# LoveDaisy/ice_halo_sim

Measured on AMD Instinct MI355X. Metric: rays/sec (whole node) at 9 wavelengths, single-scatter hex column, higher is better.
Workload: dtype f32

## Files before the change

### ice_halo_sim_amd/csrc/halo_backend.cpp

```cpp
#include <cstdlib>
#include <dlfcn.h>
#include <hip/hip_runtime.h>

#include <algorithm>
#include <cmath>
#include <cstdio>
#include <cstring>
#include <map>
#include <memory>
#include <mutex>
#include <string>
#include <vector>

#include "halo_device.h"
#include "halo_host.hpp"
#include "halo_launch.h"

#ifndef HALO_XYZ_LOG_MIN_PIX
#define HALO_XYZ_LOG_MIN_PIX (1u << 19)
#endif

using namespace halo;

namespace {

template <typename T>
struct DevBuf {
  T* ptr = nullptr;
  size_t cap = 0;
  hipError_t reserve(size_t n) {
    if (n <= cap) return hipSuccess;
    if (ptr) (void)hipFree(ptr);
    ptr = nullptr;
    cap = 0;
    hipError_t e = hipMalloc(reinterpret_cast<void**>(&ptr), std::max<size_t>(n, 1) * sizeof(T));
    if (e == hipSuccess) cap = n;
    return e;
  }
  void release() {
    if (ptr) (void)hipFree(ptr);
    ptr = nullptr;
    cap = 0;
  }
};
template <typename... B>
void release_all(B&... bufs) { (bufs.release(), ...); }

struct Marker {
  hipEvent_t ev = nullptr;
  bool set = false;
  hipError_t mark(hipStream_t s) { const hipError_t e = hipEventRecord(ev, s); set = set || e == hipSuccess; return e; }
  hipError_t wait_on(hipStream_t s) const { return set ? hipStreamWaitEvent(s, ev, 0) : hipSuccess; }
  void clear() { set = false; }
};

}

struct HaloBackend {
  int device = 0;
  uint32_t seed = 1;
  std::string error;
  hipStream_t own_stream = nullptr;
  hipStream_t stream = nullptr;
  int cu_count = 256;

  int capture = 0;
  uint32_t geom_clock = 32;
  uint64_t chunk = 1ull << 28;
  uint64_t stoch_chunk = 0;
  uint32_t bin_l1 = 128u;
  int aggregate = 1;
  int mono_enabled = 1;
  int bin = -1;
  DevBuf<HitRec> bin_list_s[2], bin_list2_s[2];
  DevBuf<uint32_t> bin_cnt_s[2], bin_cnt2_s[2];
  int log_set = 0;
  Marker set_free[2];
  hipStream_t aux = nullptr;
  hipEvent_t ev_fork = nullptr, ev_join = nullptr;
  bool aux_pending = false;
  hipStream_t cs[2] = {nullptr, nullptr};
  hipEvent_t ev_cs[2] = {nullptr, nullptr}, ev_main = nullptr, ev_aux = nullptr;
  bool cs_pending[2] = {false, false};
  int cs_next = 0;
  uint64_t aux_seq = 0, cs_seen_aux[2] = {0, 0};
  int overlap = 1;
  int defer_fold = 0;
  int twin_set = 0;
  int lambda_planes = -1;
  int mono_copies = 8;
  uint32_t mono_s_log2 = 0;
  int blocks_per_cu = 24;
  int host_shapes = 0;
  int gen_serial = 0;
  int small_blocks_per_cu = 0;
  int blocks_cap = 0;
  int lazy_fold = 1;
  int hit_log = -1;
  uint32_t hit_log_cap = 0;
  int hex_fast = 1;
  int entry_fast = 1;
  int filter_fast = 1;
  int async = 0;
  uint32_t shuffle_chunk_log2 = 5;
  int spec_root = 1;
  int close_direct = -1;
  uint64_t direct_closes = 0;
  Marker close_done;
  int close_ts = 0;
  bool cnt2_clean[2] = {false, false};
  int tile_append = -1;
  uint64_t tile_appends = 0;
  DevBuf<HitRec> tile_chunk_s[2];
  DevBuf<uint32_t> tile_cnt_s[2];
  HaloRouteInfo route{};
  uint32_t route_root = 0;

  uint64_t gen_count = 0, gate_count = 0, transit_count = 0, shape_count = 0;
  double sess_max_w = 1.0;

  bool in_session = false;
  HaloScene scene{};
  HaloRender render{};
  HaloWl wl{};
  ProjDev proj{};
  int layer_idx = 0;
  double carry[HALO_MAX_LAYERS][HALO_MAX_ENTRIES] = {};

  DevBuf<float> acc_own;
  float* acc = nullptr;
  uint64_t acc_floats = 0;
  int acc_w = 0, acc_h = 0;
  int own_w = 0, own_h = 0;
  std::vector<HaloFilter> filters;
  std::vector<HaloColorSet> color_sets;
  std::vector<HaloColorClass> color_classes;
  DevBuf<double> lanes;
  int lanes_w = 0, lanes_h = 0;
  DevBuf<FilterDev> filter_dev;
  std::unique_ptr<FastTables> fast_scratch;
  DevBuf<float> mono;
  DevBuf<double> ovf;
  DevBuf<uint32_t> ovf_flag;
  bool mono_session = false;
  bool mono_by_wl = false;
  bool xyz_log = false;
  bool mono_dirty = false;
  bool mono_two = false;
  int mono_set = 0;
  size_t mono_half = 0;
  Marker set_folded[2];
  uint32_t plane_cnt = 1, plane_copies = 8;
  std::vector<std::array<float, 3>> plane_coef;
  DevBuf<float> cons_sum, cons_comp, cons_xyz_out, cons_stage;
  DevBuf<uint8_t> cons_rgb;
  DevBuf<float> comp_rgb, lanes_stage;
  DevBuf<uint32_t> comp_hist;
  DevBuf<float> aev_vals;
  DevBuf<uint32_t> aev_ws;
  int aev_agg_hist = 0;
  int aev_select = -1;
  int cons_w = 0, cons_h = 0;
  double total_intensity = 0.0;
  DevBuf<double> tally;
  double* tally_host = nullptr;
  double tally_seen[kSumNum] = {};
  bool tally_unread = false;
  double time_trace_ms = 0.0, time_post_ms = 0.0;
  uint64_t time_launches = 0;
  DevBuf<uint32_t> counters;
  static constexpr int kRing = 32;
  DevBuf<DispatchSlot> ring_dev;
  DispatchSlot* ring_host = nullptr;
  hipEvent_t ring_ev0[kRing] = {}, ring_ev1[kRing] = {}, ring_ev2[kRing] = {}, ring_ev3[kRing] = {}, ring_done[kRing] = {};
  bool ring_posts[kRing] = {};
  bool ring_final[kRing] = {};
  bool ring_busy[kRing] = {};
  uint64_t ring_use[kRing] = {};
  int ring_next = 0;
  struct TableCacheEntry {
    bool valid = false;
    int mode = 0;
    bool use_filter = false, use_color = false, entry_fast = false, hex_regular = false, has_fast = false;
    int cur = 0;
    int read_ring[2] = {-1, -1};
    uint64_t read_use[2] = {0, 0};
  };
  TableCacheEntry tcache[HALO_MAX_LAYERS][HALO_MAX_ENTRIES];
  DevBuf<DispatchSlot> tcache_dev;
  HaloScene tcache_scene{};
  HaloWl tcache_wl{};
  std::vector<HaloWl> tcache_spec;
  uint32_t spec_count = 0;
  int table_cache = 1;
  std::map<std::string, int64_t> opt_last;
  HaloLayerStats pending{};
  HaloLayerStats layer_acc{};
  std::vector<WlEntryDev> wl_pool_host;
  uint32_t wl_pool_size = 0;
  struct LutKey { int32_t type; float center, spread; host::LatLut lut; };
  std::vector<LutKey> lut_cache;
  DevBuf<ShapeDev> shapes_s[2];
  Marker shapes_free[2];
  hipEvent_t ev_gen = nullptr;
  int shapes_next = 0;
  hipEvent_t ev_gate = nullptr;
  Marker rmw[2];
  int log_tiles_log2 = 7;
  int alt_log2 = 25;
  int rehit_strategy = 1;
  int pool_entry_fast = 1;
  int gen_ahead = 0;
  int deterministic = 0;
  bool det_session = false;
  bool fix_planes = false;
  DevBuf<unsigned long long> fix;
  uint32_t fix_frac = 32, fix_frac_landed = 32;
  uint64_t fix_hits = 0;
  unsigned long long fix_landed_seen = 0;
  double landed_carry = 0.0;
  uint32_t shard_index = 0, shard_count = 1;
  int64_t rank_opt = 0;
  bool fix_imported = false;
  bool landed_own = false;
  DevBuf<float> cont[2];
  uint32_t cont_stride[2] = {0, 0};
  uint32_t cont_region[2] = {0, 0};
  DevBuf<uint32_t> cont_cnt;
  uint32_t cont_seg[kContShards + 4] = {};
  int cont_out_slot = 0;
  uint64_t cont_in_n = 0;
  int cont_shuffle = 1;
  int cont_order = 0;
  DevBuf<uint32_t> cont_mask;
  DevBuf<uint32_t> cont_err;
  DevBuf<uint32_t> cont_base;
  DevBuf<uint32_t> cont_tiles;
  uint32_t cont_fill_max = 0;
  uint64_t cont_roots = 0;
  DevBuf<HaloExitRecord> exits;
  uint64_t exits_pending = 0;
  DevBuf<float> host_f;
  DevBuf<uint32_t> host_u;
  uint64_t sess_crystal_samples = 0, sess_orient_samples = 0;
  std::vector<hipEvent_t*> untimed_events() {
    return {&ev_cs[0], &ev_cs[1], &ev_main, &ev_aux, &ev_fork, &ev_join, &ev_gen, &ev_gate, &set_free[0].ev, &set_free[1].ev, &shapes_free[0].ev,
            &shapes_free[1].ev, &rmw[0].ev, &rmw[1].ev, &set_folded[0].ev, &set_folded[1].ev, &close_done.ev};
  }
};

namespace {

int fail(HaloBackend* b, int code, const std::string& msg) {
  if (b) b->error = msg;
  return code;
}
int hip_fail(HaloBackend* b, hipError_t e, const char* what) {
  return fail(b, (e == hipErrorNoDevice || e == hipErrorInvalidDevice || e == hipErrorOutOfMemory) ? HALO_UNAVAILABLE : HALO_FATAL,
              std::string(what) + ": " + hipGetErrorString(e));
}
#define HIPCHK(b, call)                                   \
  do {                                                    \
    hipError_t e__ = (call);                              \
    if (e__ != hipSuccess) return hip_fail(b, e__, #call); \
  } while (0)

inline float* planes_of(HaloBackend* b) { return b->mono.ptr + (b->mono_two ? static_cast<size_t>(b->mono_set) * b->mono_half : 0u); }
inline hipStream_t post_stream(HaloBackend* b) { return b->overlap ? b->aux : b->stream; }
int fork_aux(HaloBackend* b) {
  if (!b->overlap) return HALO_OK;
  HIPCHK(b, hipEventRecord(b->ev_fork, b->stream));
  HIPCHK(b, hipStreamWaitEvent(b->aux, b->ev_fork, 0));
  for (int k = 0; k < 2; k++)
    if (b->cs_pending[k]) {
      HIPCHK(b, hipEventRecord(b->ev_cs[k], b->cs[k]));
      HIPCHK(b, hipStreamWaitEvent(b->aux, b->ev_cs[k], 0));
    }
  b->aux_pending = true;
  b->aux_seq++;
  return HALO_OK;
}
int join_aux(HaloBackend* b) {
  if (b->aux_pending) {
    HIPCHK(b, hipEventRecord(b->ev_join, b->aux));
    HIPCHK(b, hipStreamWaitEvent(b->stream, b->ev_join, 0));
    b->aux_pending = false;
  }
  for (int k = 0; k < 2; k++)
    if (b->cs_pending[k]) {
      HIPCHK(b, hipEventRecord(b->ev_cs[k], b->cs[k]));
      HIPCHK(b, hipStreamWaitEvent(b->stream, b->ev_cs[k], 0));
      b->cs_pending[k] = false;
      b->rmw[k].clear();
      if (b->close_ts == k) b->close_done.clear();
    }
  return HALO_OK;
}
int wait_for_aux(HaloBackend* b, int i) {
  if (b->overlap && b->aux_pending && b->cs_seen_aux[i] != b->aux_seq) {
    HIPCHK(b, hipEventRecord(b->ev_aux, b->aux));
    HIPCHK(b, hipStreamWaitEvent(b->cs[i], b->ev_aux, 0));
    b->cs_seen_aux[i] = b->aux_seq;
  }
  return HALO_OK;
}
int next_trace_stream(HaloBackend* b, bool touches_planes, bool alternate, hipStream_t* out, int* which) {
  if (!b->overlap) {
    *out = b->stream;
    *which = 0;
    return HALO_OK;
  }
  const int i = alternate ? b->cs_next : 0;
  if (alternate) b->cs_next ^= 1;
  HIPCHK(b, hipEventRecord(b->ev_main, b->stream));
  HIPCHK(b, hipStreamWaitEvent(b->cs[i], b->ev_main, 0));
  if (touches_planes)
    if (int rc = wait_for_aux(b, i)) return rc;
  b->cs_pending[i] = true;
  *out = b->cs[i];
  *which = i;
  return HALO_OK;
}
inline uint64_t log_min_rays(int visible) { return visible == HALO_VISIBLE_FULL ? (1ull << 19) : (2ull << 20); }
int sync_all(HaloBackend* b) {
  if (int rc = join_aux(b)) return rc;
  HIPCHK(b, hipStreamSynchronize(b->stream));
  return HALO_OK;
}
template <typename T>
int reserve_idle(HaloBackend* b, DevBuf<T>& buf, size_t n, hipError_t* err = nullptr) {
  if (n > buf.cap) {
    if (int rc = sync_all(b)) return rc;
  }
  const hipError_t e = buf.reserve(n);
  if (err) {
    *err = e;
    return HALO_OK;
  }
  HIPCHK(b, e);
  return HALO_OK;
}

int take_landed_delta(HaloBackend* b, double* landed);
int forget_landed(HaloBackend* b) {
  if (!b->tally.ptr) return HALO_OK;
  if (int rc = join_aux(b)) return rc;
  double unused = 0.0;
  return take_landed_delta(b, &unused);
}

int ensure_accumulator(HaloBackend* b, int w, int h) {
  const uint64_t need = static_cast<uint64_t>(w) * h * 3 + 4;
  if (b->acc && b->acc != b->acc_own.ptr) {
    if (b->acc_floats < need) return fail(b, HALO_FATAL, "bound accumulator smaller than width*height*3+4 floats");
    b->acc_w = w;
    b->acc_h = h;
    return HALO_OK;
  }
  if (!b->acc_own.ptr || b->acc_own.cap < need || b->own_w != w || b->own_h != h) {
    if (int rc = reserve_idle(b, b->acc_own, need)) return rc;
    if (int rc = join_aux(b)) return rc;
    if (b->own_w != 0 || b->own_h != 0)
      if (int rc = forget_landed(b)) return rc;
    HIPCHK(b, hipMemsetAsync(b->acc_own.ptr, 0, need * sizeof(float), b->stream));
    b->own_w = w;
    b->own_h = h;
  }
  b->acc_w = w;
  b->acc_h = h;
  b->acc = b->acc_own.ptr;
  b->acc_floats = need;
  return HALO_OK;
}

void harvest_slot(HaloBackend* b, int k) {
  if (!b->ring_busy[k]) return;
  (void)hipEventSynchronize(b->ring_done[k]);
  float ms = 0.0f, ms2 = 0.0f;
  (void)hipEventElapsedTime(&ms, b->ring_ev0[k], b->ring_ev1[k]);
  if (b->ring_posts[k]) (void)hipEventElapsedTime(&ms2, b->ring_ev2[k], b->ring_ev3[k]);
  static const bool debug_timing = std::getenv("HALO_DEBUG_TIMING") != nullptr;
  if (debug_timing) std::fprintf(stderr, "[halo timing] slot %d final %d posts %d trace %.4f ms passes %.4f ms\n", k, int(b->ring_final[k]), int(b->ring_posts[k]), ms, ms2);
  const bool timed = ms >= 0.0f && ms2 >= 0.0f;
  if (timed) b->layer_acc.kernel_ms += ms + ms2;
  if (b->ring_final[k] && timed) {
    b->time_trace_ms += ms;
    b->time_post_ms += ms2;
    b->time_launches += 1;
  }
  b->layer_acc.launches += 1;
  b->ring_busy[k] = false;
}
int read_tally(HaloBackend* b, double out[kSumNum], unsigned long long* fix_landed = nullptr) {
  HIPCHK(b, hipMemcpyAsync(b->tally_host, b->tally.ptr, kTallyLines * kTallyStride * sizeof(double), hipMemcpyDeviceToHost, b->stream));
  HIPCHK(b, hipStreamSynchronize(b->stream));
  if (fix_landed) {
    *fix_landed = 0ull;
    for (uint32_t l = 0; l < kTallyLines; l++) {
      unsigned long long v;
      std::memcpy(&v, &b->tally_host[l * kTallyStride + kSumFixLanded], sizeof(v));
      *fix_landed += v;
    }
  }
  for (int t = 0; t < kSumNum; t++) {
    double v = 0.0;
    for (uint32_t l = 0; l < kTallyLines; l++) v += b->tally_host[l * kTallyStride + static_cast<uint32_t>(t)];
    out[t] = v;
  }
  return HALO_OK;
}
int pull_tally(HaloBackend* b) {
  if (!b->tally_unread) return HALO_OK;
  double now[kSumNum];
  int rc = read_tally(b, now);
  if (rc != HALO_OK) return rc;
  b->layer_acc.exit_w_sum += now[kSumExitW] - b->tally_seen[kSumExitW];
  b->layer_acc.exit_count += static_cast<uint64_t>(now[kSumExitN] - b->tally_seen[kSumExitN] + 0.5);
  b->layer_acc.pixel_hits += static_cast<uint64_t>(now[kSumPixN] - b->tally_seen[kSumPixN] + 0.5);
  for (int t : {kSumExitW, kSumExitN, kSumPixN}) b->tally_seen[t] = now[t];
  b->tally_unread = false;
  return HALO_OK;
}
int take_landed_delta(HaloBackend* b, double* landed) {
  double now[kSumNum];
  unsigned long long fix_now = 0ull;
  int rc = read_tally(b, now, &fix_now);
  if (rc != HALO_OK) return rc;
  *landed = now[kSumLanded] - b->tally_seen[kSumLanded] + std::ldexp(static_cast<double>(fix_now - b->fix_landed_seen), -static_cast<int>(b->fix_frac_landed)) + b->landed_carry;
  b->tally_seen[kSumLanded] = now[kSumLanded];
  b->fix_landed_seen = fix_now;
  b->landed_carry = 0.0;
  return HALO_OK;
}
void harvest_all(HaloBackend* b) {
  for (int k = 0; k < HaloBackend::kRing; k++) harvest_slot(b, k);
}
void add_stats(HaloLayerStats& dst, const HaloLayerStats& src) {
  dst.root_count += src.root_count;
  dst.exit_count += src.exit_count;
  dst.continuation_count += src.continuation_count;
  dst.exit_w_sum += src.exit_w_sum;
  dst.kernel_ms += src.kernel_ms;
  dst.pixel_hits += src.pixel_hits;
  dst.launches += src.launches;
}
void drop_table_cache(HaloBackend* b) {
  for (auto& layer : b->tcache)
    for (auto& e : layer) e.valid = false;
}
const host::LatLut& cached_lut(HaloBackend* b, const HaloDist& d) {
  for (const auto& e : b->lut_cache)
    if (e.type == d.type && e.center == d.center && e.spread == d.spread) return e.lut;
  if (b->lut_cache.size() >= 64) b->lut_cache.clear();
  b->lut_cache.push_back({d.type, d.center, d.spread, host::BuildLatLut(d)});
  return b->lut_cache.back().lut;
}

}

extern "C" {

static int fold_if_dirty(HaloBackend* b);
static int fold_queue(HaloBackend* b);
int halo_abi_version(void) { return HALO_ABI_VERSION; }

int halo_device_count(void) {
  int n = 0;
  if (hipGetDeviceCount(&n) != hipSuccess) return 0;
  return n;
}

int halo_create(int device_ordinal, uint32_t seed, halo_handle_t* out) {
  if (!out) return HALO_FATAL;
  *out = nullptr;
  int n = 0;
  if (hipGetDeviceCount(&n) != hipSuccess || n <= 0 || device_ordinal < 0 || device_ordinal >= n) return HALO_UNAVAILABLE;
  hipDeviceProp_t prop;
  if (hipGetDeviceProperties(&prop, device_ordinal) != hipSuccess) return HALO_UNAVAILABLE;
  if (std::strncmp(prop.gcnArchName, "gfx950", 6) != 0) return HALO_UNAVAILABLE;
  auto* b = new HaloBackend();
  b->device = device_ordinal;
  b->seed = seed ? seed : 1u;
  b->cu_count = prop.multiProcessorCount > 0 ? prop.multiProcessorCount : 256;
  if (hipSetDevice(device_ordinal) != hipSuccess || hipStreamCreateWithFlags(&b->own_stream, hipStreamNonBlocking) != hipSuccess) {
    delete b;
    return HALO_UNAVAILABLE;
  }
  bool aux_ok = hipStreamCreateWithFlags(&b->aux, hipStreamNonBlocking) == hipSuccess && hipStreamCreateWithFlags(&b->cs[0], hipStreamNonBlocking) == hipSuccess &&
                hipStreamCreateWithFlags(&b->cs[1], hipStreamNonBlocking) == hipSuccess;
  for (hipEvent_t* ev : b->untimed_events()) aux_ok = aux_ok && hipEventCreateWithFlags(ev, hipEventDisableTiming) == hipSuccess;
  bool ring_ok = aux_ok && b->ring_dev.reserve(HaloBackend::kRing) == hipSuccess &&
                 hipHostMalloc(reinterpret_cast<void**>(&b->ring_host), HaloBackend::kRing * sizeof(DispatchSlot), hipHostMallocDefault) == hipSuccess &&
                 hipHostMalloc(reinterpret_cast<void**>(&b->tally_host), kTallyLines * kTallyStride * sizeof(double), hipHostMallocDefault) == hipSuccess;
  for (int k = 0; ring_ok && k < HaloBackend::kRing; k++)
    ring_ok = hipEventCreate(&b->ring_ev0[k]) == hipSuccess && hipEventCreate(&b->ring_ev1[k]) == hipSuccess && hipEventCreate(&b->ring_ev2[k]) == hipSuccess && hipEventCreate(&b->ring_ev3[k]) == hipSuccess &&
              hipEventCreateWithFlags(&b->ring_done[k], hipEventDisableTiming) == hipSuccess;
  if (!ring_ok) {
    halo_destroy(b);
    return HALO_UNAVAILABLE;
  }
  b->stream = b->own_stream;
  if (b->tally.reserve(kTallyLines * kTallyStride) != hipSuccess || b->counters.reserve(kCntNum) != hipSuccess) {
    halo_destroy(b);
    return HALO_UNAVAILABLE;
  }
  (void)hipMemsetAsync(b->tally.ptr, 0, kTallyLines * kTallyStride * sizeof(double), b->stream);
  (void)hipMemsetAsync(b->counters.ptr, 0, kCntNum * sizeof(uint32_t), b->stream);
  *out = b;
  return HALO_OK;
}

int halo_destroy(halo_handle_t b) {
  if (!b) return HALO_OK;
  (void)hipSetDevice(b->device);
  (void)hipStreamSynchronize(b->stream);
  if (b->aux) (void)hipStreamSynchronize(b->aux);
  for (int k = 0; k < 2; k++)
    if (b->cs[k]) (void)hipStreamSynchronize(b->cs[k]);
  release_all(b->acc_own, b->tally, b->mono, b->ovf, b->ovf_flag, b->filter_dev, b->cons_sum, b->cons_comp, b->cons_xyz_out, b->cons_stage, b->cons_rgb, b->comp_rgb,
              b->lanes_stage, b->comp_hist, b->aev_vals, b->aev_ws, b->counters, b->ring_dev, b->tcache_dev, b->shapes_s[0], b->shapes_s[1], b->cont_cnt, b->cont_mask, b->cont_err, b->cont_base,
              b->cont_tiles, b->lanes, b->fix, b->cont[0], b->cont[1], b->exits, b->host_f, b->host_u);
  for (int k = 0; k < 2; k++) release_all(b->bin_list_s[k], b->bin_cnt_s[k], b->bin_list2_s[k], b->bin_cnt2_s[k]);
  for (int k = 0; k < 2; k++) release_all(b->tile_chunk_s[k], b->tile_cnt_s[k]);
  if (b->ring_host) (void)hipHostFree(b->ring_host);
  if (b->tally_host) (void)hipHostFree(b->tally_host);
  for (int k = 0; k < HaloBackend::kRing; k++)
    for (hipEvent_t ev : {b->ring_ev0[k], b->ring_ev1[k], b->ring_ev2[k], b->ring_ev3[k], b->ring_done[k]})
      if (ev) (void)hipEventDestroy(ev);
  for (hipEvent_t* ev : b->untimed_events())
    if (*ev) (void)hipEventDestroy(*ev);
  if (b->aux) (void)hipStreamDestroy(b->aux);
  for (int k = 0; k < 2; k++)
    if (b->cs[k]) (void)hipStreamDestroy(b->cs[k]);
  if (b->own_stream) (void)hipStreamDestroy(b->own_stream);
  delete b;
  return HALO_OK;
}

const char* halo_last_error(halo_handle_t b) { return b ? b->error.c_str() : "null handle"; }

int halo_set_option(halo_handle_t b, const char* key, int64_t v) {
  if (!b || !key) return HALO_FATAL;
  const std::string k(key);
  {
    auto it = b->opt_last.find(k);
    const bool same = it != b->opt_last.end() && it->second == v && k != "rank" && k != "ray_base" && k != "seed";
    if (!same) drop_table_cache(b);
    b->opt_last[k] = v;
  }
  if ((k == "capture_exits" || k == "filter_fast") && b->in_session) return fail(b, HALO_FATAL, k + " cannot change inside a session");
  if (k == "capture_exits") b->capture = v ? 1 : 0;
  else if (k == "geom_clock") b->geom_clock = static_cast<uint32_t>(v > 0 ? v : 32);
  else if (k == "chunk") {
    const uint64_t top = (1ull << 32) - (static_cast<uint64_t>(b->cu_count) * 64ull * kBlock) - kBlock;
    b->chunk = std::min<uint64_t>(static_cast<uint64_t>(v > 0 ? v : (1ll << 28)), top);
  }
  else if (k == "bin_l1") {
    if (v < 8 || v > 512 || (v & (v - 1)) != 0) return fail(b, HALO_FATAL, "bin_l1 must be a power of two in [8, 512]");
    b->bin_l1 = static_cast<uint32_t>(v);
  }
  else if (k == "stoch_chunk") b->stoch_chunk = static_cast<uint64_t>(v > 0 ? v : 0);
  else if (k == "aggregate") b->aggregate = static_cast<int>(v);
  else if (k == "mono") b->mono_enabled = v ? 1 : 0;
  else if (k == "async") b->async = v ? 1 : 0;
  else if (k == "lambda_planes") b->lambda_planes = static_cast<int>(v);
  else if (k == "bin") b->bin = static_cast<int>(v);
  else if (k == "host_shapes") b->host_shapes = v ? 1 : 0;
  else if (k == "entry_fast") b->entry_fast = v ? 1 : 0;
  else if (k == "hex_fast") b->hex_fast = v ? 1 : 0;
  else if (k == "filter_fast") b->filter_fast = v ? 1 : 0;
  else if (k == "spec_root") b->spec_root = v ? 1 : 0;
  else if (k == "hit_log") b->hit_log = static_cast<int>(v);
  else if (k == "hit_log_cap") b->hit_log_cap = static_cast<uint32_t>(std::max<int64_t>(v, 0));
  else if (k == "gen_serial") b->gen_serial = v ? 1 : 0;
  else if (k == "shuffle_chunk") {
    if (v < 1 || v > 64 || (v & (v - 1)) != 0) return fail(b, HALO_FATAL, "shuffle_chunk must be a power of two in [1, 64]");
    b->shuffle_chunk_log2 = 0;
    while ((1ll << b->shuffle_chunk_log2) < v) b->shuffle_chunk_log2++;
  }
  else if (k == "lazy_fold") b->lazy_fold = v ? 1 : 0;
  else if (k == "table_cache") b->table_cache = v ? 1 : 0;
  else if (k == "overlap") {
    if (int rc = sync_all(b)) return rc;
    b->overlap = v ? 1 : 0;
  }
  else if (k == "defer_fold") b->defer_fold = v ? 1 : 0;
  else if (k == "auto_ev_hist") b->aev_agg_hist = v ? 1 : 0;
  else if (k == "auto_ev_select") b->aev_select = v < 0 ? -1 : (v ? 1 : 0);
  else if (k == "gen_ahead") b->gen_ahead = v ? 1 : 0;
  else if (k == "close_direct") b->close_direct = v < 0 ? -1 : (v ? 1 : 0);
  else if (k == "tile_append") b->tile_append = v < 0 ? -1 : (v ? 1 : 0);
  else if (k == "pool_entry_fast") b->pool_entry_fast = v ? 1 : 0;
  else if (k == "rehit_strategy") {
    if (b->in_session) return fail(b, HALO_FATAL, "rehit_strategy cannot change inside a session");
    b->rehit_strategy = v ? 1 : 0;
  }
  else if (k == "cont_order") {
    if (b->in_session) return fail(b, HALO_FATAL, "cont_order cannot change inside a session");
    if (v != 0 && v != 1) return fail(b, HALO_FATAL, "cont_order must be 0 (append order) or 1 (canonical order)");
    b->cont_order = static_cast<int>(v);
  }
  else if (k == "deterministic") {
    if (b->in_session) return fail(b, HALO_FATAL, "deterministic cannot change inside a session");
    if (v != 0 && v != 1) return fail(b, HALO_FATAL, "deterministic must be 0 (float accumulation) or 1 (fixed-point accumulation)");
    b->deterministic = static_cast<int>(v);
  }
  else if (k == "log_tiles_log2") b->log_tiles_log2 = static_cast<int>(std::min<int64_t>(std::max<int64_t>(v, 0), 8));
  else if (k == "alt_log2") b->alt_log2 = static_cast<int>(std::min<int64_t>(std::max<int64_t>(v, 10), 28));
  else if (k == "small_blocks_per_cu") b->small_blocks_per_cu = static_cast<int>(std::max<int64_t>(v, 0));
  else if (k == "blocks_cap") b->blocks_cap = static_cast<int>(std::max<int64_t>(v, 0));
  else if (k == "mono_copies") {
    if (b->in_session) return fail(b, HALO_FATAL, "mono_copies cannot change while a session's plane is pending");
    if (int rc = fold_if_dirty(b)) return rc;
    int c = 1;
    while (c < v && c < 64) c <<= 1;
    if (c != b->mono_copies) {
      if (int rc = sync_all(b)) return rc;
      b->mono.release();
    }
    b->mono_copies = c;
  }
  else if (k == "blocks_per_cu") b->blocks_per_cu = static_cast<int>(std::min<int64_t>(std::max<int64_t>(v, 1), 64));
  else if ((k == "rank" || k == "ray_base") && b->in_session) {
    return fail(b, HALO_FATAL, k + " cannot change inside a session");
  }
  else if (k == "rank") {
    if (v != 0 && b->shard_count > 1) return fail(b, HALO_FATAL, "rank: not with halo_set_shard count > 1 (shards trace the one-rank run's rays: they share its counter range)");
    b->rank_opt = v;
    const uint64_t base = static_cast<uint64_t>(v) << 40;
    b->gen_count = b->gate_count = b->transit_count = b->shape_count = base;
  } else if (k == "seed") {
    if (b->in_session) return fail(b, HALO_FATAL, "seed cannot change inside a session");
    b->seed = static_cast<uint32_t>(v) ? static_cast<uint32_t>(v) : 1u;
  } else if (k == "ray_base") {
    const uint64_t base = static_cast<uint64_t>(v);
    b->gen_count = b->gate_count = b->transit_count = b->shape_count = base;
    b->rank_opt = 0;
  } else return fail(b, HALO_FATAL, "unknown option: " + k);
  return HALO_OK;
}

int halo_set_stream(halo_handle_t b, void* s) {
  if (!b) return HALO_FATAL;
  (void)sync_all(b);
  b->stream = s ? static_cast<hipStream_t>(s) : b->own_stream;
  return HALO_OK;
}

int halo_bind_accumulator(halo_handle_t b, void* device_ptr, uint64_t n_floats) {
  if (!b) return HALO_FATAL;
  if (b->in_session) return fail(b, HALO_FATAL, "bind_accumulator inside a session");
  if (int rc = fold_if_dirty(b)) return rc;
  if (!device_ptr) {
    b->acc = b->acc_own.ptr;
    b->acc_floats = b->acc_own.cap;
    return HALO_OK;
  }
  b->acc = static_cast<float*>(device_ptr);
  b->acc_floats = n_floats;
  return HALO_OK;
}

int halo_set_filters(halo_handle_t b, const HaloFilter* filters, int32_t count) {
  if (!b || count < 0 || (count > 0 && !filters)) return HALO_FATAL;
  if (b->in_session) return fail(b, HALO_FATAL, "set_filters inside a session");
  for (int32_t i = 0; i < count; i++) {
    const HaloFilter& f = filters[i];
    int terms = f.is_complex ? 0 : 1;
    if (f.is_complex) {
      if (f.or_count < 0 || f.or_count > HALO_FILTER_MAX_OR) return fail(b, HALO_FATAL, "complex filter: too many OR-clauses");
      for (int o = 0; o < f.or_count; o++) terms += f.and_counts[o];
      if (terms > HALO_FILTER_MAX_TERMS) return fail(b, HALO_FATAL, "complex filter: too many terms");
    }
  }
  const bool same = static_cast<size_t>(count) == b->filters.size() && (count == 0 || std::memcmp(b->filters.data(), filters, sizeof(HaloFilter) * static_cast<size_t>(count)) == 0);
  if (same) return HALO_OK;
  b->filters.assign(filters, filters + count);
  drop_table_cache(b);
  return HALO_OK;
}


static int begin_session(halo_handle_t b, const HaloScene* scene, const HaloRender* render, const HaloWl* wl, const HaloWl* spec, int32_t spec_n, uint64_t ray_num) {
  if (!b || !scene || !render || !wl) return HALO_FATAL;
  if (b->in_session) return fail(b, HALO_FATAL, "BeginSession inside a session");
  if (scene->layer_count < 1 || scene->layer_count > HALO_MAX_LAYERS) return fail(b, HALO_FATAL, "layer_count out of range");
  if (scene->max_hits < 1 || scene->max_hits > HALO_MAX_HITS) return fail(b, HALO_FATAL, "max_hits out of range");
  if (render->width <= 0 || render->height <= 0) return fail(b, HALO_FATAL, "bad resolution");
  bool plain_scene = !b->capture;
  for (int l = 0; l < scene->layer_count; l++) {
    if (scene->layers[l].entry_count < 1 || scene->layers[l].entry_count > HALO_MAX_ENTRIES)
      return fail(b, HALO_FATAL, "entry_count out of range");
    for (int e = 0; e < scene->layers[l].entry_count; e++) {
      const int fid = scene->layers[l].entries[e].filter_id;
      if (fid < 0 || fid > static_cast<int>(b->filters.size())) return fail(b, HALO_FATAL, "entry refers to a filter_id outside the table");
      const int cid = scene->layers[l].entries[e].color_id;
      if (cid < 0 || cid > static_cast<int>(b->color_sets.size())) return fail(b, HALO_FATAL, "entry refers to a color_id outside the table");
      if (fid > 0 || cid > 0) plain_scene = false;
      const int kind = scene->layers[l].entries[e].crystal.kind;
      if (kind != HALO_CRYSTAL_PRISM && kind != HALO_CRYSTAL_PYRAMID) return fail(b, HALO_FATAL, "unknown crystal kind");
    }
  }
  if (b->shard_count > 1 && scene->layer_count > 1)
    return fail(b, HALO_FATAL, "halo_set_shard count > 1: a multi-layer scene is not supported (the next layer's pool order and shuffle are global over all roots; shards do not exchange continuation pools)");
  const bool det = b->deterministic != 0;
  if (det) {
    if (scene->layer_count > 1 && !b->cont_order)
      return fail(b, HALO_FATAL, "deterministic = 1: a multi-layer session needs cont_order = 1 (the continuation pool's append order decides which rays the next layer traces)");
    if (!b->color_classes.empty() || !b->color_sets.empty()) return fail(b, HALO_FATAL, "deterministic = 1: raypath-colour tables are set (the class lanes are fp64 atomics)");
    if (b->capture) return fail(b, HALO_FATAL, "deterministic = 1: capture_exits = 1 is not supported (the capture kernels have no fixed-point route)");
    if (b->rehit_strategy == 0) return fail(b, HALO_FATAL, "deterministic = 1: rehit_strategy = 0 is not supported (the legacy strategy lives in the generic kernels)");
    for (int l = 0; l < scene->layer_count; l++)
      for (int e = 0; e < scene->layers[l].entry_count; e++) {
        const HaloEntry& E = scene->layers[l].entries[e];
        if (E.filter_id <= 0) continue;
        const FilterDev fd = host::BuildFilter(b->filters[static_cast<size_t>(E.filter_id - 1)], E.axis);
        if (!(fd.is_complex || fd.terms[0].type != HALO_FILTER_NONE || fd.action != 0)) continue;
        std::unique_ptr<FastTables> ft(new FastTables());
        std::memset(ft.get(), 0, sizeof(FastTables));
        if (!b->filter_fast || scene->max_hits > 16 ||
            !host::BuildFastTables(&b->filters[static_cast<size_t>(E.filter_id - 1)], nullptr, E.axis, static_cast<uint32_t>(E.crystal_config_id), *ft))
          return fail(b, HALO_FATAL, "deterministic = 1: a filter of this scene needs the generic filter kernels (filter_fast = 0, max_hits > 16, or tables that do not fit the fast form)");
      }
  }
  HIPCHK(b, hipSetDevice(b->device));
  const bool same_spec = b->tcache_spec.size() == static_cast<size_t>(spec_n) &&
                         (spec_n == 0 || std::memcmp(b->tcache_spec.data(), spec, sizeof(HaloWl) * static_cast<size_t>(spec_n)) == 0);
  if (std::memcmp(&b->tcache_scene, scene, sizeof(HaloScene)) != 0 || std::memcmp(&b->tcache_wl, wl, sizeof(HaloWl)) != 0 || !same_spec) {
    drop_table_cache(b);
    b->tcache_scene = *scene;
    b->tcache_wl = *wl;
    b->tcache_spec.assign(spec, spec + spec_n);
  }
  b->scene = *scene;
  b->render = *render;
  b->wl = *wl;
  b->proj = host::BuildProj(*render);
  std::vector<WlEntryDev> pool = host::BuildWlPool(*wl);
  for (int32_t k = 1; k < spec_n; k++) {
    const std::vector<WlEntryDev> one = host::BuildWlPool(spec[k]);
    pool.insert(pool.end(), one.begin(), one.end());
  }
  b->spec_count = static_cast<uint32_t>(spec_n);
  b->wl_pool_size = static_cast<uint32_t>(pool.size());
  if (pool.empty() || pool.size() > HALO_WL_POOL_MAX) return fail(b, HALO_FATAL, "wavelength pool size out of range");
  b->wl_pool_host = pool;
  b->sess_max_w = 0.0;
  for (const WlEntryDev& e : pool) b->sess_max_w = std::max(b->sess_max_w, static_cast<double>(std::fabs(e.spd_weight)));
  const size_t npix = static_cast<size_t>(render->width) * render->height;
  if (npix > (1u << 25)) return fail(b, HALO_UNAVAILABLE, "more than 2^25 pixels");
  const bool discrete = wl->illuminant < 0 && spec_n == 0;
  uint32_t s_log2 = 6;
  while ((static_cast<size_t>(kMonoRows) << s_log2) < npix) s_log2++;
  const bool log_xyz_fits = s_log2 <= 11u, log_mono_fits = s_log2 <= 12u;
  const bool xyz_log_n = !det && b->mono_enabled && !discrete && b->lambda_planes < 0 && b->hit_log != 0 && ray_num >= (2ull << 20) && npix > HALO_XYZ_LOG_MIN_PIX && log_xyz_fits;
  const bool mono_by_wl_n = !det && b->mono_enabled && !discrete && !xyz_log_n && npix <= (1u << 23) && (b->lambda_planes < 0 ? ray_num >= (8ull << 20) : b->lambda_planes != 0);
  const bool mono_session_n = b->mono_enabled && (discrete || mono_by_wl_n);
  const uint32_t plane_cnt_n = mono_by_wl_n ? static_cast<uint32_t>(pool.size()) : (mono_session_n ? 1u : 3u);
  bool one_entry_layers = true;
  for (int l = 0; l < scene->layer_count; l++) one_entry_layers = one_entry_layers && scene->layers[l].entry_count == 1;
  const bool fast_scene = b->rehit_strategy != 0 && (plain_scene || (!b->capture && b->filter_fast && scene->max_hits <= 16));
  const bool all_logged = !det && fast_scene && one_entry_layers && b->hit_log < 0 && b->aggregate == 1 && ray_num >= (discrete ? log_min_rays(render->visible) : (2ull << 20)) &&
                          (discrete ? log_mono_fits : xyz_log_n) && (mono_session_n || xyz_log_n);
  const uint32_t plane_copies_n = (mono_by_wl_n || all_logged || det) ? 1u : static_cast<uint32_t>(b->mono_copies);
  const bool two_sets_n = all_logged && discrete && mono_session_n && !mono_by_wl_n && b->overlap != 0;
  std::vector<std::array<float, 3>> coef_n;
  for (uint32_t m = 0; m < plane_cnt_n; m++) {
    if (mono_session_n) coef_n.push_back({pool[m].cmf_x, pool[m].cmf_y, pool[m].cmf_z});
    else coef_n.push_back({m == 0 ? 1.0f : 0.0f, m == 1 ? 1.0f : 0.0f, m == 2 ? 1.0f : 0.0f});
  }
  {
    const bool same_planes = b->mono_dirty && b->lazy_fold && b->acc != nullptr && b->acc == b->acc_own.ptr && b->acc_w == render->width &&
                             b->acc_h == render->height && b->mono_s_log2 == s_log2 && b->plane_cnt == plane_cnt_n && b->plane_copies == plane_copies_n &&
                             b->mono_two == two_sets_n && b->plane_coef == coef_n && b->fix_planes == det;
    if (!same_planes) {
      int rc = fold_queue(b);
      if (rc != HALO_OK) return rc;
      const bool caller_reads = b->acc != nullptr && b->acc != b->acc_own.ptr && !b->defer_fold;
      const bool layout_changes = b->mono_s_log2 != s_log2 || b->plane_cnt != plane_cnt_n || b->plane_copies != plane_copies_n || b->mono_two != two_sets_n;
      if (caller_reads || layout_changes) {
        rc = join_aux(b);
        if (rc != HALO_OK) return rc;
      }
    }
    int rc = ensure_accumulator(b, render->width, render->height);
    if (rc != HALO_OK) return rc;
  }
  b->xyz_log = xyz_log_n;
  b->mono_by_wl = mono_by_wl_n;
  b->mono_session = mono_session_n;
  b->plane_cnt = plane_cnt_n;
  b->plane_copies = plane_copies_n;
  b->plane_coef = coef_n;
  b->det_session = det;
  if (det) {
    const size_t need = (static_cast<size_t>(kMonoRows) << s_log2) * b->plane_cnt;
    b->mono_two = false;
    b->mono_set = 0;
    if (b->fix.cap < need) {
      if (int rc = reserve_idle(b, b->fix, need)) return rc;
      HIPCHK(b, hipMemsetAsync(b->fix.ptr, 0, b->fix.cap * sizeof(unsigned long long), b->stream));
    }
    b->mono_s_log2 = s_log2;
  } else {
    const size_t one = (static_cast<size_t>(kMonoRows) << s_log2) * b->plane_copies * b->plane_cnt;
    b->mono_two = two_sets_n;
    b->mono_half = one;
    if (!b->mono_two) b->mono_set = 0;
    const size_t need = one * (b->mono_two ? 2u : 1u);
    if (b->mono.cap < need) {
      if (int rc = reserve_idle(b, b->mono, need)) return rc;
      HIPCHK(b, hipMemsetAsync(b->mono.ptr, 0, b->mono.cap * sizeof(float), b->stream));
    }
    b->mono_s_log2 = s_log2;
    const size_t twin_need = (static_cast<size_t>(kMonoRows) << s_log2) * b->plane_cnt;
    if (b->ovf.cap < 2u * twin_need && twin_need <= (512ull << 20)) {
      hipError_t oe = hipSuccess;
      if (int rc = reserve_idle(b, b->ovf, 2u * twin_need, &oe)) return rc;
      bool ok = oe == hipSuccess;
      if (ok && !b->ovf_flag.ptr) ok = b->ovf_flag.reserve(2) == hipSuccess && hipMemsetAsync(b->ovf_flag.ptr, 0, 2 * sizeof(uint32_t), b->stream) == hipSuccess;
      if (ok) {
        HIPCHK(b, hipMemsetAsync(b->ovf.ptr, 0, b->ovf.cap * sizeof(double), b->stream));
      } else {
        (void)hipGetLastError();
        b->ovf.release();
        b->ovf_flag.release();
      }
    }
  }
  if (!b->color_classes.empty()) {
    const size_t need = b->color_classes.size() * npix;
    if (b->lanes.cap < need || b->lanes_w != render->width || b->lanes_h != render->height) {
      if (int rc = reserve_idle(b, b->lanes, need)) return rc;
      if (int rc = join_aux(b)) return rc;
      HIPCHK(b, hipMemsetAsync(b->lanes.ptr, 0, b->lanes.cap * sizeof(double), b->stream));
      b->lanes_w = render->width;
      b->lanes_h = render->height;
    }
  }
  b->sess_crystal_samples = b->sess_orient_samples = 0;
  b->route = HaloRouteInfo{};
  b->route_root = 0u;
  b->route.plane_cnt = b->plane_cnt;
  b->route.plane_copies = b->plane_copies;
  b->route.shuffle_chunk = 1u << b->shuffle_chunk_log2;
  b->in_session = true;
  b->layer_idx = 0;
  b->cont_in_n = 0;
  b->cont_out_slot = 0;
  return HALO_OK;
}

int halo_begin(halo_handle_t b, const HaloScene* scene, const HaloRender* render, const HaloWl* wl, uint64_t ray_num) {
  return begin_session(b, scene, render, wl, nullptr, 0, ray_num);
}

int halo_begin_spectrum(halo_handle_t b, const HaloScene* scene, const HaloRender* render, const HaloWl* entries, int32_t count, uint64_t ray_num) {
  if (!b) return HALO_FATAL;
  if (!scene) return fail(b, HALO_FATAL, "halo_begin_spectrum: scene is NULL");
  if (!render) return fail(b, HALO_FATAL, "halo_begin_spectrum: render is NULL");
  if (!entries) return fail(b, HALO_FATAL, "halo_begin_spectrum: entries is NULL");
  if (count < 1 || count > HALO_WL_POOL_MAX) return fail(b, HALO_FATAL, "halo_begin_spectrum: count " + std::to_string(count) + " outside 1..HALO_WL_POOL_MAX (255)");
  for (int32_t k = 0; k < count; k++)
    if (entries[k].illuminant >= 0)
      return fail(b, HALO_FATAL, "halo_begin_spectrum: entries[" + std::to_string(k) + "] is an illuminant (illuminant >= 0); a spectrum is made of discrete wavelengths");
  if (count == 1) return begin_session(b, scene, render, entries, nullptr, 0, ray_num);
  return begin_session(b, scene, render, entries, entries, count, ray_num);
}

uint32_t halo_host_spectrum_entry(uint64_t m, uint32_t count, uint64_t r) {
  const uint64_t reach = 0xFFFFFFFEull, off_a = r > reach ? r - reach : 0ull, off_b = r - r % 65521ull;
  const SpectrumChunkDev a = SpectrumChunk(m, count, off_a), c = SpectrumChunk(m, count, off_b);
  const uint32_t ka = SpectrumEntry(a.per, a.k0, a.rem, a.last, static_cast<uint32_t>(r - off_a));
  const uint32_t kb = SpectrumEntry(c.per, c.k0, c.rem, c.last, static_cast<uint32_t>(r - off_b));
  return ka == kb ? ka : 0xFFFFFFFFu;
}

static uint32_t fix_frac_bits(double max_w, uint64_t m) {
  const double bound = 4.0 * std::max(max_w, 1e-30) * static_cast<double>(std::max<uint64_t>(m, 1));
  int e = 0;
  (void)std::frexp(bound, &e);
  return static_cast<uint32_t>(std::min(32, std::max(0, 62 - e)));
}

constexpr uint64_t kFixBudgetHits = 1ull << 30, kFixLandedHits = 1ull << 32;
uint32_t halo_host_fixed_frac_bits(double max_w, uint64_t hits) { return fix_frac_bits(max_w, hits); }

static double* twin_of(HaloBackend* b, int set) {
  const size_t half = (static_cast<size_t>(kMonoRows) << b->mono_s_log2) * b->plane_cnt;
  if (!b->ovf.ptr || !b->ovf_flag.ptr || b->ovf.cap < 2u * half) return nullptr;
  return b->ovf.ptr + static_cast<size_t>(set) * half;
}

static int fold_queue(HaloBackend* b) {
  if (!b->mono_dirty) return HALO_OK;
  if (b->fix_planes && b->shard_count > 1 && !b->fix_imported)
    return fail(b, HALO_FATAL, "shard " + std::to_string(b->shard_index) + " of " + std::to_string(b->shard_count) +
                                   ": the pending fixed-point planes hold a part of the image; move them out with halo_export_fixed (and fold what halo_import_fixed brings in)");
  HIPCHK(b, hipSetDevice(b->device));
  if (int rc = fork_aux(b)) return rc;
  hipStream_t ps = post_stream(b);
  const uint32_t npix = static_cast<uint32_t>(b->acc_w) * static_cast<uint32_t>(b->acc_h);
  if (b->fix_planes) {
    FoldCoef coef{};
    for (uint32_t m = 0; m < b->plane_cnt; m++)
      for (int a = 0; a < 3; a++) coef.c[m][a] = b->plane_coef[m][static_cast<size_t>(a)];
    hipError_t e = launch_fold_fixed(b->acc, b->fix.ptr, npix, b->mono_s_log2, b->plane_cnt, coef, b->fix_frac, ps);
    if (e != hipSuccess) return hip_fail(b, e, "halo_fold_fixed_kernel launch");
    b->fix_hits = 0;
    b->fix_planes = false;
    b->fix_imported = false;
    b->mono_dirty = false;
    return HALO_OK;
  }
  const size_t plane = (static_cast<size_t>(kMonoRows) << b->mono_s_log2) * b->plane_copies;
  const size_t twin_plane = static_cast<size_t>(kMonoRows) << b->mono_s_log2;
  double* twin = twin_of(b, b->twin_set);
  uint32_t* flag = twin ? b->ovf_flag.ptr + b->twin_set : nullptr;
// ... 202 lines not shown
  }
  T.ce_dev = T.ce ? b->tcache_dev.ptr + (static_cast<size_t>(c.layer) * HALO_MAX_ENTRIES + static_cast<size_t>(ci)) * 2u : nullptr;
  T.cached = T.ce && T.ce->valid;
  if (T.cached) T.use_filter = T.ce->use_filter;
  else if (E.filter_id > 0) {
    T.fd = host::BuildFilter(b->filters[static_cast<size_t>(E.filter_id - 1)], E.axis);
    T.use_filter = T.fd.is_complex || T.fd.terms[0].type != HALO_FILTER_NONE || T.fd.action != 0;
  }

  ColorDev& cd = T.cd;
  T.use_color = !b->color_classes.empty();
  if (T.use_color && !T.cached) {
    cd.class_cnt = static_cast<uint32_t>(b->color_classes.size());
    for (uint32_t k = 0; k < cd.class_cnt; k++) {
      cd.class_bits[k] = b->color_classes[k].bits;
      cd.class_all[k] = b->color_classes[k].combine_all ? 1 : 0;
    }
    if (E.color_id > 0) {
      const HaloColorSet& cs = b->color_sets[static_cast<size_t>(E.color_id - 1)];
      cd.term_cnt = static_cast<uint32_t>(std::min(cs.term_count, HALO_COLOR_MAX_TERMS));
      for (uint32_t k = 0; k < cd.term_cnt; k++) {
        HaloFilter one{};
        one.symmetry = cs.terms[k].symmetry;
        one.terms[0] = cs.terms[k].predicate;
        const FilterDev f1 = host::BuildFilter(one, E.axis);
        cd.terms[k].t = f1.terms[0];
        cd.terms[k].symmetry = f1.symmetry;
        cd.terms[k].d_applicable = f1.d_applicable;
        cd.terms[k].sigma_a = f1.sigma_a;
        cd.terms[k].bit = static_cast<uint8_t>(cs.terms[k].bit & 0xFF);
      }
    }
  }

  if (T.cached) T.mode = T.ce->mode;
  else if (b->capture) T.mode = 2;
  else if (b->rehit_strategy == 0) T.mode = 3;
  else if (T.use_filter || T.use_color) {
    T.mode = 3;
    if (b->filter_fast && b->scene.max_hits <= 16) {
      b->fast_scratch.reset(new FastTables());
      std::memset(b->fast_scratch.get(), 0, sizeof(FastTables));
      const HaloColorSet* cs = (T.use_color && E.color_id > 0) ? &b->color_sets[static_cast<size_t>(E.color_id - 1)] : nullptr;
      if (host::BuildFastTables(T.use_filter ? &b->filters[static_cast<size_t>(E.filter_id - 1)] : nullptr, cs, E.axis, static_cast<uint32_t>(E.crystal_config_id), *b->fast_scratch)) {
        T.fast_host = b->fast_scratch.get();
        T.fast_host->class_cnt = T.use_color ? cd.class_cnt : 0u;
        for (uint32_t k = 0; k < T.fast_host->class_cnt; k++) {
          T.fast_host->class_bits[k] = cd.class_bits[k];
          T.fast_host->class_all[k] = cd.class_all[k];
        }
        T.mode = T.use_color ? 4 : 1;
      }
    }
  }
  T.fast_mode = T.mode == 0 || T.mode == 1 || T.mode == 4;
  T.has_fast = T.cached ? T.ce->has_fast : T.fast_host != nullptr;
  if (T.cached) T.entry_fast = T.ce->entry_fast, T.hex_regular = T.ce->hex_regular;
}
int upload_tables(HaloBackend* b, const LayerCtx& c, const LaunchPlan& p, const HaloEntry& E, uint32_t lat_path, const ShapeDev* shape, int k, EntryTables& T,
                  DispatchSlot** out) {
  HaloBackend::TableCacheEntry* ce = T.ce;
  DispatchSlot& hs = b->ring_host[k];
  if (ce && !T.cached) ce->cur ^= 1;
  DispatchSlot* ds = *out = ce ? T.ce_dev + ce->cur : b->ring_dev.ptr + k;
  if (T.cached) return HALO_OK;
  if (lat_path == kLatLut) {
    const host::LatLut& lut = cached_lut(b, E.axis.latitude);
    std::copy(lut.theta.begin(), lut.theta.end(), hs.lut);
    std::copy(lut.cdf.begin(), lut.cdf.end(), hs.lut + kLutNodes);
    std::copy(lut.flip.begin(), lut.flip.end(), hs.lut + 2 * kLutNodes);
  }
  std::copy(b->wl_pool_host.begin(), b->wl_pool_host.end(), hs.wl);
  if (p.deterministic) {
    hs.shape = *shape;
    T.entry_fast = b->entry_fast && host::BuildEntryFast(*shape, hs.efast);
    T.hex_regular = T.entry_fast && hs.efast.hex_regular;
  }
  if (T.use_filter) hs.filter = T.fd;
  if (T.use_color) hs.color = T.cd;
  if (T.fast_host) std::memcpy(&hs.fast, T.fast_host, sizeof(FastTables));
  if (c.source == kSrcTransit) std::copy(b->cont_seg, b->cont_seg + kContShards + 1, hs.seg);
  if (ce && ce->read_ring[ce->cur] >= 0) {
    const int rk = ce->read_ring[ce->cur];
    if (b->ring_busy[rk] && b->ring_use[rk] == ce->read_use[ce->cur]) HIPCHK(b, hipStreamWaitEvent(b->stream, b->ring_done[rk], 0));
  }
  HIPCHK(b, hipMemcpyAsync(ds, &hs, T.fast_host ? sizeof(DispatchSlot) : offsetof(DispatchSlot, fast), hipMemcpyHostToDevice, b->stream));
  if (ce) {
    ce->valid = true, ce->mode = T.mode, ce->use_filter = T.use_filter, ce->use_color = T.use_color;
    ce->entry_fast = T.entry_fast, ce->hex_regular = T.hex_regular, ce->has_fast = T.has_fast;
    T.cached = true;
  }
  return HALO_OK;
}
uint32_t root_profile_of(const DispatchParams& P) {
  if (P.lat_path != kLatLut || P.az_type != HALO_DIST_UNIFORM || P.roll_type != HALO_DIST_UNIFORM) return kRootProfileNone;
  return P.source == kSrcGen ? kRootProfileGen : P.source == kSrcTransit ? kRootProfileTransit : kRootProfileNone;
}
DispatchParams fill_params(HaloBackend* b, const LayerCtx& c, int ci) {
  const HaloLayer& L = b->scene.layers[c.layer];
  const HaloEntry& E = L.entries[ci];
  DispatchParams P{};
  P.source = c.source;
  P.layer = static_cast<uint32_t>(c.layer);
  P.final_layer = c.final_layer ? 1u : 0u;
  P.max_hits = static_cast<uint32_t>(b->scene.max_hits);
  P.prob = L.prob;
  P.crystal_id = static_cast<uint32_t>(E.crystal_config_id);
  P.capture = static_cast<uint32_t>(b->capture);
  P.gen_seed = b->seed ^ kNonceGen;
  P.gate_seed = b->seed ^ kNonceGate;
  P.transit_seed = b->seed ^ kNonceTransit;
  P.shuffle = static_cast<uint32_t>(b->cont_shuffle);
  P.shuffle_seed = (b->seed ^ kNonceShuffle) ^ static_cast<uint32_t>(c.layer);
  P.shuffle_chunk_log2 = b->shuffle_chunk_log2;
  P.lat_path = host::SelectLatPath(E.axis);
  P.lat_mean_rad = E.axis.latitude.center * host::kDegToRad;
  P.lat_std_rad = E.axis.latitude.spread * host::kDegToRad;
  P.az_type = static_cast<uint32_t>(E.axis.azimuth.type);
  P.az_mean_rad = E.axis.azimuth.center * host::kDegToRad;
  P.az_std_rad = E.axis.azimuth.spread * host::kDegToRad;
  P.roll_type = static_cast<uint32_t>(E.axis.roll.type);
  P.roll_mean_rad = E.axis.roll.center * host::kDegToRad;
  P.roll_std_rad = E.axis.roll.spread * host::kDegToRad;
  const float sun_lon = (b->scene.sun_azimuth + 180.0f) * host::kDegToRad;
  const float sun_lat = -b->scene.sun_altitude * host::kDegToRad;
  const float half = (b->scene.sun_diameter * 0.5f) * host::kDegToRad;
  P.c_cap = std::cos(half);
  P.c_lon = std::cos(sun_lon);
  P.s_lon = std::sin(sun_lon);
  P.c_lat = std::cos(sun_lat);
  P.s_lat = std::sin(sun_lat);
  P.wl_pool_size = b->wl_pool_size;
  P.proj = b->proj;
  P.proj_pre[0] = static_cast<float>(b->proj.img_w) / 2.0f, P.proj_pre[1] = static_cast<float>(b->proj.img_h) / 2.0f;
  P.proj_pre[2] = static_cast<float>(b->proj.lens_shift_x), P.proj_pre[3] = static_cast<float>(b->proj.lens_shift_y);
  P.cont_in = b->cont[c.out_slot ^ 1].ptr;
  P.cont_in_n = static_cast<uint32_t>(b->cont_in_n);
  P.cont_in_stride = b->cont_stride[c.out_slot ^ 1];
  P.cont_out = b->cont[c.out_slot].ptr;
  P.cont_out_stride = b->cont_stride[c.out_slot];
  P.cont_out_cap = c.out_cap;
  P.cont_in_region = b->cont_region[c.out_slot ^ 1];
  P.cont_cnt = b->cont_cnt.ptr;
  P.cont_mask = (b->cont_order && !c.final_layer) ? b->cont_mask.ptr : nullptr;
  P.cont_err = c.canon_check ? b->cont_err.ptr : nullptr;
  P.counters = b->counters.ptr;
  P.mono = planes_of(b);
  P.mono_s_log2 = b->mono_s_log2;
  P.ovf = twin_of(b, b->twin_set);
  P.ovf_copies_log2 = static_cast<uint32_t>(__builtin_ctz(b->plane_copies));
  P.ovf_flag = P.ovf ? b->ovf_flag.ptr + b->twin_set : nullptr;
  P.pool_entry_fast = b->pool_entry_fast ? 1u : 0u;
  P.rehit_legacy = b->rehit_strategy == 0 ? 1u : 0u;
  P.tally = b->tally.ptr;
  P.exits = b->exits.ptr;
  P.exit_cap = static_cast<uint32_t>(std::min<uint64_t>(b->exits.cap, 0xFFFFFFFFull));
  P.aggregate = static_cast<uint32_t>(b->aggregate);
  P.geom_clock = b->geom_clock;
  P.lanes = b->lanes.ptr;
  P.lane_stride = static_cast<uint32_t>(b->acc_w) * static_cast<uint32_t>(b->acc_h);
  P.root_profile = (b->spec_root && b->spec_count == 0u) ? root_profile_of(P) : kRootProfileNone;
  P.fix = b->det_session ? b->fix.ptr : nullptr;
  return P;
}
int bind_route(HaloBackend* b, LaunchPlan& p, int ls, DispatchParams& P) {
  if (p.use_log)
    if (int rc = reserve_log_buffers(b, p, ls)) return rc;
  DevBuf<HitRec>&bin_list = b->bin_list_s[ls], &bin_list2 = b->bin_list2_s[ls];
  DevBuf<uint32_t>&bin_cnt = b->bin_cnt_s[ls], &bin_cnt2 = b->bin_cnt2_s[ls];
  if (p.use_bin)
    if (int rc = join_aux(b)) return rc;
  if (p.use_log) {
    if (int rc = reserve_idle(b, bin_cnt, std::max<size_t>(static_cast<size_t>(p.blocks), static_cast<size_t>(512) * 16u))) return rc;
    if (int rc = reserve_idle(b, bin_cnt2, static_cast<size_t>(512) * 16u)) return rc;
    HIPCHK(b, b->set_free[ls].wait_on(b->stream));
  } else if (p.use_bin) {
    if (int rc = reserve_idle(b, bin_cnt, static_cast<size_t>(512) * 16u)) return rc;
    HIPCHK(b, hipMemsetAsync(bin_cnt.ptr, 0, static_cast<size_t>(p.two_level ? 512u : p.bin_tiles) * 16u * sizeof(uint32_t), b->stream));
    if (int rc = reserve_idle(b, bin_list, p.cap1 * p.lists1)) return rc;
    if (p.two_level) {
      if (int rc = reserve_idle(b, bin_cnt2, static_cast<size_t>(p.bin_tiles) * 16u)) return rc;
      HIPCHK(b, hipMemsetAsync(bin_cnt2.ptr, 0, static_cast<size_t>(p.bin_tiles) * 16u * sizeof(uint32_t), b->stream));
      b->cnt2_clean[ls] = false;
      if (int rc = reserve_idle(b, bin_list2, p.cap2 * p.bin_tiles)) return rc;
    }
  }
  const bool lists = p.use_log || p.use_bin;
  P.bin_list = lists ? bin_list.ptr : nullptr;
  P.bin_log = p.use_log ? 1u : 0u;
  P.log_xyz = p.use_log_xyz ? 1u : 0u;
  P.mono_by_wl = b->mono_by_wl ? 1u : 0u;
  P.mono_copy_mask = lists ? 0u : b->plane_copies - 1u;
  if (lists) {
    P.bin_cap = static_cast<uint32_t>(p.cap1);
    P.bin_tiles = p.use_log ? p.log_tiles : p.two_level ? b->bin_l1 : p.bin_tiles;
    P.bin_shift = (p.use_bin && p.two_level) ? 14u + p.fan_log2 : 0u;
    P.bin_cnt = bin_cnt.ptr;
  }
  if (p.use_log) P.log_plane_stride = static_cast<uint32_t>((static_cast<uint64_t>(kMonoRows) << b->mono_s_log2) * b->plane_copies);
  P.no_land = p.no_land ? 1u : 0u;
  return HALO_OK;
}
bool close_direct_ok(const HaloBackend& b, const LaunchPlan& p, const DispatchParams& P) {
  if (b.close_direct == 0 || !p.only || p.fixed || !p.use_log || p.use_log_xyz || p.log_planes != 1u || b.mono_by_wl) return false;
  if (b.plane_cnt != 1u || b.plane_copies != 1u || b.render.visible == HALO_VISIBLE_FULL) return false;
  if ((1u << p.log_t_log2) > 256u || b.mono_s_log2 + 10u - p.log_t_log2 > kBinTileLog2) return false;
  if (P.ovf == nullptr || P.ovf_flag == nullptr || b.mono_dirty || b.acc == nullptr) return false;
  return b.close_direct > 0 || !p.alternate;
}
int bind_tile_append(HaloBackend* b, LaunchPlan& p, const EntryTables& T, int ls, DispatchParams& P) {
  P.tile_chunk = nullptr, P.tile_cnt = nullptr, P.tile_cap = P.tile_log2 = P.tile_tiles = 0u;
  p.tile = false;
  if (!p.close || b->tile_append == 0 || (b->tile_append < 0 && (p.alternate || P.source != kSrcGen))) return HALO_OK;
  const int lens = P.proj.proj_type;
  const bool lens_known = lens == HALO_LENS_LINEAR || lens == HALO_LENS_FISHEYE_EQUAL_AREA || lens == HALO_LENS_DUAL_FISHEYE_EQUAL_AREA || lens == HALO_LENS_RECTANGULAR;
  const bool hex = p.geom == 0 && T.entry_fast && b->hex_fast && T.hex_regular;
  if (T.mode != 0 || !hex || !b->mono_session || P.final_layer == 0u || P.prob > 0.0f || P.cont_mask != nullptr || P.no_land != 0u || P.fix != nullptr ||
      P.mono_by_wl != 0u || P.proj.visible_range != HALO_VISIBLE_UPPER || !lens_known)
    return HALO_OK;
  const uint32_t t_log2 = std::min<uint32_t>(p.log_t_log2, static_cast<uint32_t>(__builtin_ctz(kTileAppendMax)));
  if (b->mono_s_log2 + 10u < t_log2 || b->mono_s_log2 + 10u - t_log2 > kBinTileLog2) return HALO_OK;
  const uint64_t tiles = 1ull << t_log2, blocks = static_cast<uint64_t>(p.blocks), chunks = tiles * blocks;
  const uint64_t per_wg = (p.m + blocks - 1u) / blocks;
  uint64_t cap = std::max<uint64_t>(8ull * 4ull * per_wg / tiles, 16ull);
  cap = std::min<uint64_t>(cap, (1ull << 30) / chunks);
  if (b->hit_log_cap) cap = std::max<uint64_t>(b->hit_log_cap / tiles, 2ull);
  size_t free_b = 0, total_b = 0;
  const uint64_t have = b->tile_chunk_s[ls].cap * sizeof(HitRec), need = cap * chunks * sizeof(HitRec);
  if (need > have && hipMemGetInfo(&free_b, &total_b) == hipSuccess && need - have > free_b / 2u)
    cap = (have + free_b / 2u) / (chunks * sizeof(HitRec));
  cap &= ~1ull;
  if (cap < 2u) return HALO_OK;
  hipError_t e1 = hipSuccess, e2 = hipSuccess;
  if (int rc = reserve_idle(b, b->tile_chunk_s[ls], cap * chunks, &e1)) return rc;
  if (e1 == hipSuccess)
    if (int rc = reserve_idle(b, b->tile_cnt_s[ls], chunks, &e2)) return rc;
  if (e1 != hipSuccess || e2 != hipSuccess) {
    (void)hipGetLastError();
    return HALO_OK;
  }
  if (b->overlap && p.alternate) {
    hipError_t e3 = hipSuccess, e4 = hipSuccess;
    if (int rc = reserve_idle(b, b->tile_chunk_s[ls ^ 1], cap * chunks, &e3)) return rc;
    if (e3 == hipSuccess)
      if (int rc = reserve_idle(b, b->tile_cnt_s[ls ^ 1], chunks, &e4)) return rc;
    if (e3 != hipSuccess || e4 != hipSuccess) (void)hipGetLastError();
  }
  p.tile = true;
  P.tile_chunk = b->tile_chunk_s[ls].ptr, P.tile_cnt = b->tile_cnt_s[ls].ptr;
  P.tile_cap = static_cast<uint32_t>(cap), P.tile_tiles = static_cast<uint32_t>(tiles), P.tile_log2 = b->mono_s_log2 + 10u - t_log2;
  return HALO_OK;
}
void record_route(HaloBackend* b, const LaunchPlan& p, const DispatchParams& P, int mode, bool fast_mode, int launch_geom) {
  b->route.launches++;
  b->route.mode_mask |= 1u << mode;
  const bool ran_hex = launch_geom == 3 && fast_mode && (P.bin_list == nullptr || P.bin_log != 0u || P.no_land != 0u);
  const bool ran_none = P.no_land != 0u && p.geom == 0;
  b->route.geom_mask |= 1u << (launch_geom == 3 && !ran_hex ? 0 : launch_geom);
  b->route.accum_mask |= ran_none ? 64u : p.fixed ? (128u | (p.use_log ? (p.use_log_xyz ? 32u : 16u) : 0u)) : p.use_log ? (p.use_log_xyz ? 32u : 16u) : (p.use_bin ? (p.two_level ? 8u : 4u) : (b->mono_session ? 2u : 1u));
  const bool one = p.geom == 0, lens_known = P.proj.proj_type == HALO_LENS_LINEAR || P.proj.proj_type == HALO_LENS_FISHEYE_EQUAL_AREA ||
                                             P.proj.proj_type == HALO_LENS_DUAL_FISHEYE_EQUAL_AREA || P.proj.proj_type == HALO_LENS_RECTANGULAR;
  const bool vis_known = P.proj.visible_range == HALO_VISIBLE_UPPER || P.proj.visible_range == HALO_VISIBLE_FULL;
  uint32_t spec = 0u;
  const bool logged = p.use_log && !p.fixed;
  if (fast_mode && logged && one && !ran_none && b->mono_session && P.final_layer) {
    spec |= 1u;
    if ((mode == 0 || mode == 1) && P.prob <= 0.0f && lens_known && vis_known) spec |= 2u | 4u | 8u;
  }
  if (fast_mode && logged && one && !ran_none && b->mono_session && !P.final_layer && (mode == 0 || mode == 1) && lens_known && vis_known)
    spec |= 2u | 4u;
  if (mode == 0 && logged && !one && !b->mono_session && P.prob <= 0.0f && P.proj.visible_range == HALO_VISIBLE_FULL) spec |= 4u | 8u;
  if (mode == 0 && logged && !one && P.prob <= 0.0f && P.proj.visible_range == HALO_VISIBLE_FULL && P.proj.proj_type == HALO_LENS_RECTANGULAR)
    spec |= 2u | 4u | 8u;
  b->route.spec_mask |= spec;
  if (spec == 0u) b->route.generic_launches++;
  const bool no_transit = P.proj.proj_type == HALO_LENS_LINEAR && P.proj.visible_range == HALO_VISIBLE_FULL;
  if (mode == 0 && ran_hex && P.final_layer && (spec & (2u | 4u | 8u)) == (2u | 4u | 8u) && P.root_profile != kRootProfileNone && P.root_profile == root_profile_of(P) &&
      !(no_transit && P.root_profile == kRootProfileTransit))
    b->route_root |= 1u << (P.root_profile - 1u);
  b->route.source_mask |= 1u << P.source;
}
int queue_passes(HaloBackend* b, const LaunchPlan& p, const DispatchParams& P, const LaunchSlots& S, hipStream_t ts, int ts_i, hipEvent_t before_sums) {
  const int k = S.k;
  DevBuf<HitRec>&bin_list = b->bin_list_s[S.ls], &bin_list2 = b->bin_list2_s[S.ls];
  DevBuf<uint32_t>&bin_cnt = b->bin_cnt_s[S.ls], &bin_cnt2 = b->bin_cnt2_s[S.ls];
  const uint32_t frac_bits = fix_frac_bits(b->sess_max_w, p.m);
  const uint32_t cap2 = static_cast<uint32_t>(p.cap2 & ~15ull);
  if (!p.use_log) {
    if (p.use_bin) {
      hipError_t be = p.two_level ? launch_bin_two_level(P.mono, bin_list.ptr, P.bin_cap, bin_cnt.ptr, p.lists1, bin_list2.ptr, cap2, bin_cnt2.ptr,
                                                         p.bin_tiles, p.fan_log2, frac_bits, P.ovf, P.ovf_flag, ts, before_sums)
                                  : launch_bin_accumulate(P.mono, bin_list.ptr, P.bin_cap, bin_cnt.ptr, p.bin_tiles, frac_bits, ts);
      if (be != hipSuccess) return hip_fail(b, be, "halo_bin_accumulate_kernel launch");
      if (b->overlap && p.two_level) HIPCHK(b, b->rmw[ts_i].mark(ts));
    }
    HIPCHK(b, hipEventRecord(b->ring_ev1[k], ts));
    b->ring_posts[k] = false;
    HIPCHK(b, hipEventRecord(b->ring_done[k], ts));
    return HALO_OK;
  }
  HIPCHK(b, hipEventRecord(b->ring_ev1[k], ts));
  hipStream_t ps = ts;
  if (p.under_fold()) {
    if (b->mono_two) {
      HIPCHK(b, b->set_folded[b->mono_set].wait_on(ps));
    } else if (int rc = wait_for_aux(b, ts_i)) return rc;
  }
  HIPCHK(b, hipEventRecord(b->ring_ev2[k], ps));
  if (p.close && p.tile) {
    const float coef[3] = {b->plane_coef[0][0], b->plane_coef[0][1], b->plane_coef[0][2]};
    hipError_t ce = launch_tile_route_close(b->acc, static_cast<uint32_t>(b->acc_w) * static_cast<uint32_t>(b->acc_h), coef, P.tile_chunk, P.tile_cap, P.tile_cnt,
                                            static_cast<uint32_t>(p.blocks), P.tile_tiles, b->mono_s_log2, frac_bits, P.ovf, P.ovf_flag, ps, before_sums);
    if (ce != hipSuccess) return hip_fail(b, ce, "halo_tile_close_kernel launch");
    b->direct_closes++;
    b->tile_appends++;
    HIPCHK(b, b->close_done.mark(ps));
    b->close_ts = ts_i;
    HIPCHK(b, hipEventRecord(b->ring_ev3[k], ps));
    HIPCHK(b, b->set_free[S.ls].mark(ps));
    if (b->overlap && p.alternate) b->log_set ^= 1;
    b->ring_posts[k] = true;
    HIPCHK(b, hipEventRecord(b->ring_done[k], ps));
    return HALO_OK;
  }
  if (p.close) {
    if (!b->cnt2_clean[S.ls]) HIPCHK(b, hipMemsetAsync(bin_cnt2.ptr, 0, static_cast<size_t>(p.log_tiles) * 16u * sizeof(uint32_t), ps));
    const float coef[3] = {b->plane_coef[0][0], b->plane_coef[0][1], b->plane_coef[0][2]};
    hipError_t ce = launch_log_route_close(b->acc, static_cast<uint32_t>(b->acc_w) * static_cast<uint32_t>(b->acc_h), coef, bin_list.ptr, P.bin_cap, bin_cnt.ptr,
                                           static_cast<uint32_t>(p.blocks), bin_list2.ptr, cap2, bin_cnt2.ptr, 1u << p.log_t_log2, b->mono_s_log2, frac_bits, P.ovf, P.ovf_flag,
                                           ps, before_sums);
    if (ce != hipSuccess) return hip_fail(b, ce, "halo_split_kernel launch (direct close)");
    b->cnt2_clean[S.ls] = true;
    b->direct_closes++;
    HIPCHK(b, b->close_done.mark(ps));
    b->close_ts = ts_i;
    HIPCHK(b, hipEventRecord(b->ring_ev3[k], ps));
    HIPCHK(b, b->set_free[S.ls].mark(ps));
    if (b->overlap && p.alternate) b->log_set ^= 1;
    b->ring_posts[k] = true;
    HIPCHK(b, hipEventRecord(b->ring_done[k], ps));
    return HALO_OK;
  }
  HIPCHK(b, hipMemsetAsync(bin_cnt2.ptr, 0, static_cast<size_t>(p.log_tiles) * 16u * sizeof(uint32_t), ps));
  b->cnt2_clean[S.ls] = false;
  hipError_t be = p.fixed ? (p.use_log_xyz ? launch_log_route_xyz_fixed(P.fix, P.log_plane_stride, bin_list.ptr, P.bin_cap, bin_cnt.ptr, static_cast<uint32_t>(p.blocks), bin_list2.ptr, cap2,
                                                                        bin_cnt2.ptr, p.log_tiles, b->mono_s_log2, P.wl_pool, P.wl_pool_size, b->fix_frac, ps)
                                           : launch_log_route_fixed(P.fix, bin_list.ptr, P.bin_cap, bin_cnt.ptr, static_cast<uint32_t>(p.blocks), bin_list2.ptr, cap2, bin_cnt2.ptr,
                                                                    1u << p.log_t_log2, b->mono_s_log2, b->render.visible == HALO_VISIBLE_FULL, b->fix_frac, ps))
                  : p.use_log_xyz ? launch_log_route_xyz(P.mono, P.log_plane_stride, bin_list.ptr, P.bin_cap, bin_cnt.ptr, static_cast<uint32_t>(p.blocks),
                                                       bin_list2.ptr, cap2, bin_cnt2.ptr, p.log_tiles, b->mono_s_log2, P.wl_pool, P.wl_pool_size, frac_bits, P.ovf, P.ovf_flag, P.ovf_copies_log2, ps, before_sums)
                                : launch_log_route(P.mono, bin_list.ptr, P.bin_cap, bin_cnt.ptr, static_cast<uint32_t>(p.blocks), bin_list2.ptr, cap2,
                                                   bin_cnt2.ptr, 1u << p.log_t_log2, p.log_planes, b->mono_s_log2, b->render.visible == HALO_VISIBLE_FULL, frac_bits,
                                                   P.ovf, P.ovf_flag, P.ovf_copies_log2, ps, before_sums);
  if (be != hipSuccess) return hip_fail(b, be, "halo_split_kernel launch");
  if (b->overlap && !p.fixed) HIPCHK(b, b->rmw[ts_i].mark(ps));
  HIPCHK(b, hipEventRecord(b->ring_ev3[k], ps));
  HIPCHK(b, b->set_free[S.ls].mark(ps));
  if (b->overlap && p.alternate) b->log_set ^= 1;
  b->ring_posts[k] = true;
  HIPCHK(b, hipEventRecord(b->ring_done[k], ps));
  return HALO_OK;
}
int queue_launch(HaloBackend* b, const LaunchPlan& p, const HaloEntry& E, EntryTables& T, const DispatchParams& P, const LaunchSlots& S) {
  const int k = S.k;
  hipStream_t ts = nullptr;
  int ts_i = 0;
  if (int rc = next_trace_stream(b, !p.under_fold(), p.alternate, &ts, &ts_i)) return rc;
  if (b->close_done.set && b->close_ts != ts_i)
    HIPCHK(b, b->close_done.wait_on(ts));
  hipEvent_t before_sums = nullptr;
#ifndef HALO_NO_PLANE_GATES
  if (b->overlap && !p.use_log)
    HIPCHK(b, b->rmw[ts_i ^ 1].wait_on(ts));
  if (b->overlap && ((p.use_log && !p.fixed) || (p.use_bin && p.two_level)) && b->cs_pending[ts_i ^ 1]) {
    HIPCHK(b, hipEventRecord(b->ev_gate, b->cs[ts_i ^ 1]));
    before_sums = b->ev_gate;
  }
#endif
  if (!p.deterministic && !p.host_pool) {
    const bool ahead = b->overlap && b->gen_ahead && !p.alternate;
    hipStream_t gs = ahead ? b->cs[1] : ts;
    HIPCHK(b, b->shapes_free[S.shape_set].wait_on(gs));
    hipError_t ge = launch_shapegen(const_cast<ShapeDev*>(P.shapes), p.geom == 2, p.shape_cnt, b->seed, host::MakeRecipe(E.crystal), S.first_shape, gs, b->gen_serial != 0);
    if (ge != hipSuccess) return hip_fail(b, ge, "halo_shapegen_kernel launch");
    if (ahead) {
      HIPCHK(b, hipEventRecord(b->ev_gen, gs));
      HIPCHK(b, hipStreamWaitEvent(ts, b->ev_gen, 0));
      b->cs_pending[1] = true;
    }
  }
  HIPCHK(b, hipEventRecord(b->ring_ev0[k], ts));
  b->ring_final[k] = P.final_layer != 0u;
  const int launch_geom = (p.geom == 0 && T.entry_fast && b->hex_fast && T.hex_regular) ? 3 : p.geom;
  hipError_t le = launch_trace(P, p.blocks, ts, T.mode, launch_geom, b->mono_session);
  if (T.ce) {
    T.ce->read_ring[T.ce->cur] = k;
    T.ce->read_use[T.ce->cur] = b->ring_use[k];
  }
  if (!p.close && !(p.no_land && p.geom == 0)) b->mono_dirty = true;
  b->fix_planes = b->det_session;
  record_route(b, p, P, T.mode, T.fast_mode, launch_geom);
  if (le != hipSuccess) return hip_fail(b, le, "halo_trace_kernel launch");
  if (!p.deterministic) HIPCHK(b, b->shapes_free[S.shape_set].mark(ts));
  if (int rc = queue_passes(b, p, P, S, ts, ts_i, before_sums)) return rc;
  b->tally_unread = true;
  b->ring_busy[k] = true;
  return HALO_OK;
}
int fix_prepare(HaloBackend* b, uint64_t m) {
  const uint32_t f = fix_frac_bits(b->sess_max_w, kFixBudgetHits), fl = fix_frac_bits(b->sess_max_w, kFixLandedHits);
  if (b->mono_dirty && b->fix_planes && (f != b->fix_frac || b->fix_hits + m > kFixBudgetHits))
    if (int rc = fold_queue(b)) return rc;
  if (!(b->mono_dirty && b->fix_planes)) {
    b->fix_frac = f;
    b->fix_hits = 0;
  }
  b->fix_hits += m;
  if (fl != b->fix_frac_landed) {
    if (b->shard_count > 1 && b->landed_own)
      return fail(b, HALO_FATAL, "shard " + std::to_string(b->shard_index) + " of " + std::to_string(b->shard_count) +
                                     ": this session's weights change the scale of the landed integer (F_landed) while the shard still holds landed weight of its own; move it out with halo_export_fixed first");
    if (int rc = join_aux(b)) return rc;
    double now[kSumNum];
    unsigned long long fix_now = 0ull;
    if (int rc = read_tally(b, now, &fix_now)) return rc;
    b->landed_carry += std::ldexp(static_cast<double>(fix_now - b->fix_landed_seen), -static_cast<int>(b->fix_frac_landed));
    b->fix_landed_seen = fix_now;
    b->fix_frac_landed = fl;
  }
  return HALO_OK;
}
int trace_launch(HaloBackend* b, const LayerCtx& c, LaunchPlan& p, EntryTables& T, DispatchParams& P) {
  const HaloEntry& E = b->scene.layers[c.layer].entries[p.ci];
  const uint64_t m = p.m;
  LaunchSlots S;
  std::vector<ShapeDev> pool((p.deterministic && !T.cached) || p.host_pool ? p.shape_cnt : 0u);
  for (uint32_t k = 0; k < static_cast<uint32_t>(pool.size()); k++) {
    if (c.host_crystal) host::ToShapeDev(*c.rays->crystal, pool[k]);
    else host::MakeShapeDev(b->seed, E.crystal, p.deterministic ? 0 : (b->shape_count + k), pool[k]);
  }
  S.first_shape = b->shape_count;
  if (!p.deterministic) {
    b->shape_count += p.shape_cnt;
    b->sess_crystal_samples += p.shape_cnt;
  }
  if (c.rays == nullptr && (E.axis.azimuth.type != HALO_DIST_NONE || E.axis.latitude.type != HALO_DIST_NONE || E.axis.roll.type != HALO_DIST_NONE))
    b->sess_orient_samples += m;
  S.k = b->ring_next;
  b->ring_next = (S.k + 1) % HaloBackend::kRing;
  harvest_slot(b, S.k);
  b->ring_use[S.k]++;
  DispatchSlot* ds = nullptr;
  if (int rc = upload_tables(b, c, p, E, P.lat_path, pool.empty() ? nullptr : pool.data(), S.k, T, &ds)) return rc;
  P.lut = ds->lut;
  P.wl_pool = ds->wl;
  P.filter = T.use_filter ? &ds->filter : nullptr;
  P.color = T.use_color ? &ds->color : nullptr;
  P.fast = T.has_fast ? &ds->fast : nullptr;
  P.cont_in_seg = ds->seg;
  P.entry_fast = T.entry_fast ? &ds->efast : nullptr;
  if (p.deterministic) {
    P.shapes = &ds->shape;
  } else {
    const bool turn = b->overlap && (p.alternate || b->gen_ahead);
    S.shape_set = turn ? b->shapes_next : 0;
    if (turn) b->shapes_next ^= 1;
    DevBuf<ShapeDev>& shapes = b->shapes_s[S.shape_set];
    if (int rc = reserve_idle(b, shapes, p.shape_cnt)) return rc;
    if (turn)
      if (int rc = reserve_idle(b, b->shapes_s[S.shape_set ^ 1], p.shape_cnt)) return rc;
    if (p.host_pool) {
      HIPCHK(b, b->shapes_free[S.shape_set].wait_on(b->stream));
      HIPCHK(b, hipMemcpyAsync(shapes.ptr, pool.data(), pool.size() * sizeof(ShapeDev), hipMemcpyHostToDevice, b->stream));
    }
    P.shapes = shapes.ptr;
  }
  P.shape_cnt = p.shape_cnt;
  P.n_rays = static_cast<uint32_t>(m);
  P.ci_start = static_cast<uint32_t>(p.first);
  P.spec_per = P.spec_k0 = P.spec_rem = P.spec_last = 0u;
  if (b->spec_count != 0u && c.layer == 0) {
    const SpectrumChunkDev sc = SpectrumChunk(p.share, b->spec_count, p.off);
    P.spec_per = sc.per, P.spec_k0 = sc.k0, P.spec_rem = sc.rem, P.spec_last = sc.last;
  }
  auto split = [](uint64_t v, uint32_t& lo, uint32_t& hi) { lo = static_cast<uint32_t>(v & 0xFFFFFFFFull), hi = static_cast<uint32_t>(v >> 32); };
  split(b->gen_count, P.gen_lo, P.gen_hi);
  split(b->gate_count, P.gate_lo, P.gate_hi);
  split(b->transit_count, P.transit_lo, P.transit_hi);
  if (c.rays) {
    P.host_d = b->host_f.ptr + p.off * 3;
    P.host_p = b->host_f.ptr + c.n * 3 + p.off * 3;
    P.host_w = b->host_f.ptr + c.n * 6 + p.off;
    P.host_tf = b->host_u.ptr + p.off;
  }
  plan_route(*b, c, T.fast_mode, p);
  if (p.fixed) {
    if (T.mode != 0 && T.mode != 1) return fail(b, HALO_FATAL, "deterministic = 1: this entry needs kernels without a fixed-point route");
    if (int rc = fix_prepare(b, m)) return rc;
    P.fix_frac = b->fix_frac;
    P.fix_frac_landed = b->fix_frac_landed;
  }
  S.ls = (b->overlap && p.alternate) ? b->log_set : 0;
  if (int rc = bind_route(b, p, S.ls, P)) return rc;
  p.close = close_direct_ok(*b, p, P);
  if (int rc = bind_tile_append(b, p, T, S.ls, P)) return rc;
  if (int rc = queue_launch(b, p, E, T, P, S)) return rc;
  if (p.host_pool) HIPCHK(b, hipStreamSynchronize(b->stream));
  if (P.source == kSrcGen) b->gen_count += m;
  if (P.source == kSrcTransit) b->transit_count += m;
  b->gate_count += m;
  return HALO_OK;
}
int trace_shard(HaloBackend* b, LayerCtx& c, std::vector<LaunchPlan>& plans, const std::vector<uint64_t>& per_ci) {
  for (const LaunchPlan& p : plans)
    if (!p.deterministic && p.off % b->geom_clock != 0u)
      return fail(b, HALO_FATAL, "halo_set_shard count > 1: a sampled crystal entry is cut into launches (chunk, stoch_chunk) that are not multiples of geom_clock; a shard cannot start inside a sampled shape");
  if (b->det_session && b->landed_own && fix_frac_bits(b->sess_max_w, kFixLandedHits) != b->fix_frac_landed)
    return fail(b, HALO_FATAL, "shard " + std::to_string(b->shard_index) + " of " + std::to_string(b->shard_count) +
                                   ": this session's weights change the scale of the landed integer (F_landed) while the shard still holds landed weight of its own; move it out with halo_export_fixed first");
  EntryTables T;
  DispatchParams P{};
  int cur = -1;
  c.traced = 0;
  for (const LaunchPlan& whole : plans) {
    uint64_t s0 = 0, sn = 0;
    shard_slice(per_ci[static_cast<size_t>(whole.ci)], whole.deterministic ? 1u : b->geom_clock, b->shard_index, b->shard_count, &s0, &sn);
    const uint64_t lo = std::max(whole.off, s0), hi = std::min(whole.off + whole.m, s0 + sn);
    const uint64_t gen0 = b->gen_count, gate0 = b->gate_count, shape0 = b->shape_count;
    if (lo < hi) {
      LaunchPlan p = plan_launch(*b, c, whole.ci, whole.first - whole.off, lo, hi - lo);
      p.share = whole.share;
      b->gen_count = gen0 + (lo - whole.off);
      b->gate_count = gate0 + (lo - whole.off);
      if (!whole.deterministic) b->shape_count = shape0 + (lo - whole.off) / b->geom_clock;
      if (p.ci != cur) {
        cur = p.ci;
        prepare_entry_tables(b, c, cur, T);
        P = fill_params(b, c, cur);
      }
      if (int rc = trace_launch(b, c, p, T, P)) return rc;
      b->fix_imported = false;
      b->landed_own = b->det_session;
      c.traced += p.m;
    }
    b->gen_count = gen0 + whole.m;
    b->gate_count = gate0 + whole.m;
    if (!whole.deterministic) b->shape_count = shape0 + whole.shape_cnt;
  }
  if (b->det_session && !(b->mono_dirty && b->fix_planes)) {
    if (int rc = fix_prepare(b, 0)) return rc;
    b->mono_dirty = true;
    b->fix_planes = true;
    b->fix_imported = false;
  }
  return HALO_OK;
}
int close_layer(HaloBackend* b, const LayerCtx& c, bool defer, HaloLayerStats* stats) {
  const uint64_t n = c.n;
  if (defer) {
    b->layer_acc.root_count += c.traced;
    if (stats) {
      std::memset(stats, 0, sizeof(*stats));
      stats->root_count = c.traced;
    }
    b->cont_in_n = 0;
    return HALO_OK;
  }
  if (int rc = join_aux(b)) return rc;
  uint32_t cnt[kCntNum] = {0, 0, 0, 0};
  std::vector<uint32_t> fill(c.final_layer ? 0 : kContShards * kContCntStride);
  HIPCHK(b, hipMemcpyAsync(cnt, b->counters.ptr, sizeof(cnt), hipMemcpyDeviceToHost, b->stream));
  if (!c.final_layer) HIPCHK(b, hipMemcpyAsync(fill.data(), b->cont_cnt.ptr, fill.size() * sizeof(uint32_t), hipMemcpyDeviceToHost, b->stream));
  uint32_t cont_err = 0;
  if (c.canon_check) HIPCHK(b, hipMemcpyAsync(&cont_err, b->cont_err.ptr, sizeof(uint32_t), hipMemcpyDeviceToHost, b->stream));
  if (b->tally_unread) {
    if (int rc = pull_tally(b)) return rc;
  } else {
    HIPCHK(b, hipStreamSynchronize(b->stream));
  }
  harvest_all(b);
  if (cont_err != 0u)
    return cont_order_fail(b, cont_err);
  uint64_t n_cont = 0;
  if (!c.final_layer) {
    b->cont_fill_max = 0;
    for (int sI = 0; sI < kContShards; sI++) {
      const uint32_t cs = fill[static_cast<size_t>(sI) * kContCntStride];
      if (cs > c.out_cap) return fail(b, HALO_FATAL, b->cont_order ? "continuation pool overflow (cont_order = 1: the canonical pool would be incomplete)" : "continuation pool overflow");
      b->cont_seg[sI] = static_cast<uint32_t>(n_cont);
      n_cont += cs;
      b->cont_fill_max = std::max(b->cont_fill_max, cs);
    }
    b->cont_seg[kContShards] = static_cast<uint32_t>(n_cont);
    b->cont_roots = n;
  }
  b->exits_pending = std::min<uint64_t>(cnt[kCntExit], b->exits.cap);
  b->layer_acc.root_count = c.traced;
  b->layer_acc.continuation_count = n_cont;
  if (stats) *stats = b->layer_acc;
  add_stats(b->pending, b->layer_acc);
  b->layer_acc = HaloLayerStats{};
  b->cont_in_n = n_cont;
  return HALO_OK;
}
}

extern "C" {
int halo_trace_layer(halo_handle_t b, uint64_t count, const HaloHostRays* rays, HaloLayerStats* stats) {
  if (!b) return HALO_FATAL;
  if (!b->in_session) return fail(b, HALO_FATAL, "TraceLayer outside a session");
  LayerCtx c;
  const int layer = c.layer = b->layer_idx;
  if (layer >= b->scene.layer_count) return fail(b, HALO_FATAL, "TraceLayer past the last layer");
  HIPCHK(b, hipSetDevice(b->device));
  const HaloLayer& L = b->scene.layers[layer];
  const uint64_t n = c.n = c.traced = (layer == 0) ? count : b->cont_in_n;
  c.final_layer = (layer == b->scene.layer_count - 1);
  if (n > 0xFFFFFFF0ull) return fail(b, HALO_FATAL, "more than 2^32 rays in one layer dispatch; split the batch");
  if (layer > 0 && rays) return fail(b, HALO_FATAL, "host rays are first-layer only");
  if (rays && b->shard_count > 1) return fail(b, HALO_FATAL, "halo_set_shard count > 1: host-injected rays are not supported (a shard generates its slice of the session's roots)");
  if (rays && rays->crystal) {
    const HaloGeomTables& g = *rays->crystal;
    if (g.face_cnt < 0 || g.face_cnt > HALO_MAX_FACES || g.tri_cnt < 0 || g.tri_cnt > HALO_MAX_TRIS)
      return fail(b, HALO_FATAL, "host crystal: face_cnt / tri_cnt outside 0..HALO_MAX_FACES / 0..HALO_MAX_TRIS");
    for (int t = 0; t < g.tri_cnt; t++)
      if (g.tri_face[t] < 0 || g.tri_face[t] >= g.face_cnt) return fail(b, HALO_FATAL, "host crystal: tri_face refers to a face outside the table");
  }
  c.rays = rays;
  c.source = rays ? kSrcHost : (layer == 0 ? kSrcGen : kSrcTransit);
  c.host_crystal = rays != nullptr && rays->crystal != nullptr && layer == 0;
  c.out_slot = b->cont_out_slot;
  c.canon_check = b->cont_order && b->scene.layer_count > 1;
  float props[HALO_MAX_ENTRIES];
  for (int ci = 0; ci < L.entry_count; ci++) props[ci] = L.entries[ci].proportion;
  std::vector<uint64_t> per_ci = host::Partition(props, L.entry_count, n, b->carry[layer]);
  if (rays && layer == 0) {
    std::fill(per_ci.begin(), per_ci.end(), 0);
    per_ci[0] = n;
  }
  std::vector<LaunchPlan> plans;
  uint64_t ci_start = 0;
  for (int ci = 0; ci < L.entry_count; ci_start += per_ci[ci], ci++)
    for (uint64_t off = 0; off < per_ci[ci]; off += plans.back().m) plans.push_back(plan_launch(*b, c, ci, ci_start, off, per_ci[ci] - off));
  if (!c.final_layer) {
    uint64_t region = 0;
    for (const LaunchPlan& p : plans) {
      const uint64_t nb = static_cast<uint64_t>(p.blocks);
      const uint64_t per_block = (p.m + nb * kBlock - 1) / (nb * kBlock) * kBlock;
      region += (nb + kContShards - 1) / kContShards * per_block * static_cast<uint64_t>(b->scene.max_hits);
    }
    region = (region + 63) & ~63ull;
    const uint64_t stride = region * kContShards;
    if (stride > 0xFFFFFFF0ull) return fail(b, HALO_FATAL, "continuation pool would exceed 2^32 rays; split the batch");
    const uint64_t planes = b->cont_order ? kContPlanesCanonical : (b->color_classes.empty() ? 5 : 7);
    if (b->cont_order && stride * planes > 0xFFFFFFFFull) return fail(b, HALO_FATAL, "canonical continuation pool planes would exceed 2^32 floats; split the batch");
    if (int rc = reserve_idle(b, b->cont[c.out_slot], stride * planes)) return rc;
    b->cont_stride[c.out_slot] = static_cast<uint32_t>(stride);
    b->cont_region[c.out_slot] = static_cast<uint32_t>(region);
    c.out_cap = static_cast<uint32_t>(region);
    HIPCHK(b, b->cont_cnt.reserve(kContShards * kContCntStride));
    HIPCHK(b, hipMemsetAsync(b->cont_cnt.ptr, 0, kContShards * kContCntStride * sizeof(uint32_t), b->stream));
    if (b->cont_order) {
      if (b->rehit_strategy == 0) return fail(b, HALO_FATAL, "cont_order = 1 needs rehit_strategy = 1 (the legacy strategy can emit twice at one interaction)");
      if (int rc = reserve_idle(b, b->cont_mask, kContMaskWords * std::max<uint64_t>(c.n, 1))) return rc;
      HIPCHK(b, hipMemsetAsync(b->cont_mask.ptr, 0, kContMaskWords * c.n * sizeof(uint32_t), b->stream));
      if (c.layer == 0) {
        if (int rc = reserve_idle(b, b->cont_err, 16)) return rc;
        HIPCHK(b, hipMemsetAsync(b->cont_err.ptr, 0, sizeof(uint32_t), b->stream));
      }
    }
  }
  const bool defer = b->async && c.final_layer && !b->capture && !c.canon_check;
  if (!defer) {
    harvest_all(b);
    if (int rc = pull_tally(b)) return rc;
    add_stats(b->pending, b->layer_acc);
    b->layer_acc = HaloLayerStats{};
  }
  if (b->capture) {
    const uint64_t need = b->exits_pending + n * static_cast<uint64_t>(b->scene.max_hits + 1);
    if (need > b->exits.cap) {
      DevBuf<HaloExitRecord> bigger;
      HIPCHK(b, bigger.reserve(need));
      if (b->exits_pending)
        HIPCHK(b, hipMemcpyAsync(bigger.ptr, b->exits.ptr, b->exits_pending * sizeof(HaloExitRecord), hipMemcpyDeviceToDevice, b->stream));
      if (int rc = sync_all(b)) return rc;
      b->exits.release();
      b->exits = bigger;
    }
  }
  if (rays && layer == 0) {
    for (uint64_t i = 0; i < n; i++) b->sess_max_w = std::max(b->sess_max_w, static_cast<double>(std::fabs(rays->w[i])));
    if (int rc = join_aux(b)) return rc;
    if (int rc = reserve_idle(b, b->host_f, n * 7)) return rc;
    if (int rc = reserve_idle(b, b->host_u, n)) return rc;
    HIPCHK(b, hipMemcpyAsync(b->host_f.ptr, rays->d, n * 3 * sizeof(float), hipMemcpyHostToDevice, b->stream));
    HIPCHK(b, hipMemcpyAsync(b->host_f.ptr + n * 3, rays->p, n * 3 * sizeof(float), hipMemcpyHostToDevice, b->stream));
    HIPCHK(b, hipMemcpyAsync(b->host_f.ptr + n * 6, rays->w, n * sizeof(float), hipMemcpyHostToDevice, b->stream));
    HIPCHK(b, hipMemcpyAsync(b->host_u.ptr, rays->tf, n * sizeof(uint32_t), hipMemcpyHostToDevice, b->stream));
    HIPCHK(b, hipStreamSynchronize(b->stream));
  }
  EntryTables T;
  DispatchParams P{};
  int cur = -1;
  if (plans.size() == 1u) plans[0].only = c.final_layer;
  if (b->shard_count > 1) {
    if (int rc = trace_shard(b, c, plans, per_ci)) return rc;
    return close_layer(b, c, defer, stats);
  }
  for (LaunchPlan& p : plans) {
    if (p.ci != cur) {
      cur = p.ci;
      prepare_entry_tables(b, c, cur, T);
      P = fill_params(b, c, cur);
    }
    if (int rc = trace_launch(b, c, p, T, P)) return rc;
  }
  return close_layer(b, c, defer, stats);
}

int halo_generate_shapes(halo_handle_t b, const HaloCrystal* crystal, uint64_t first_index, uint32_t n, int on_device, HaloGeomTables* out) {
  if (!b || !crystal || (!out && n)) return HALO_FATAL;
  if (crystal->kind != HALO_CRYSTAL_PRISM && crystal->kind != HALO_CRYSTAL_PYRAMID) return fail(b, HALO_FATAL, "unknown crystal kind");
  std::vector<ShapeDev> pool(n);
  if (on_device == 2 && crystal->kind == HALO_CRYSTAL_PRISM) {
    HIPCHK(b, hipSetDevice(b->device));
    DevBuf<ShapePrism> dev;
    HIPCHK(b, dev.reserve(n));
    std::vector<ShapePrism> recs(n);
    hipError_t ge = launch_shapegen(dev.ptr, true, n, b->seed, host::MakeRecipe(*crystal), first_index, b->stream, b->gen_serial != 0);
    if (ge == hipSuccess) ge = hipMemcpyAsync(recs.data(), dev.ptr, static_cast<size_t>(n) * sizeof(ShapePrism), hipMemcpyDeviceToHost, b->stream);
    if (ge == hipSuccess) ge = hipStreamSynchronize(b->stream);
    dev.release();
    if (ge != hipSuccess) return hip_fail(b, ge, "halo_prismgen_team_kernel");
    for (uint32_t k = 0; k < n; k++) {
      const ShapePrism& r = recs[k];
      ShapeDev& d = pool[k];
      std::memset(&d, 0, sizeof(d));
      d.face_cnt = r.face_cnt, d.tri_cnt = r.tri_cnt, d.slab_cnt = r.slab_cnt, d.single_cnt = r.single_cnt;
      std::memcpy(d.face, r.face, sizeof(r.face));
      std::memcpy(d.slab, r.slab, sizeof(r.slab));
      std::memcpy(d.tri_v, r.tri_v, sizeof(r.tri_v));
      std::memcpy(d.tri_na, r.tri_na, sizeof(r.tri_na));
      std::memcpy(d.tri_face, r.tri_face, sizeof(r.tri_face));
      std::memcpy(d.face_number, r.face_number, sizeof(r.face_number));
      std::memcpy(d.single, r.single, sizeof(r.single));
    }
  } else if (on_device) {
    HIPCHK(b, hipSetDevice(b->device));
    DevBuf<ShapeDev> dev;
    HIPCHK(b, dev.reserve(n));
    hipError_t ge = launch_shapegen(dev.ptr, false, n, b->seed, host::MakeRecipe(*crystal), first_index, b->stream, b->gen_serial != 0);
    if (ge == hipSuccess) ge = hipMemcpyAsync(pool.data(), dev.ptr, static_cast<size_t>(n) * sizeof(ShapeDev), hipMemcpyDeviceToHost, b->stream);
    if (ge == hipSuccess) ge = hipStreamSynchronize(b->stream);
    dev.release();
    if (ge != hipSuccess) return hip_fail(b, ge, "halo_shapegen_kernel");
  } else {
    for (uint32_t k = 0; k < n; k++) host::MakeShapeDev(b->seed, *crystal, first_index + k, pool[k]);
  }
  for (uint32_t k = 0; k < n; k++) host::FromShapeDev(pool[k], out[k]);
  return HALO_OK;
}

int halo_set_color(halo_handle_t b, const HaloColorSet* sets, int n_sets, const HaloColorClass* classes, int n_classes) {
  if (!b || n_sets < 0 || n_classes < 0 || (n_sets && !sets) || (n_classes && !classes)) return HALO_FATAL;
  if (b->in_session) return fail(b, HALO_FATAL, "halo_set_color inside a session");
  if (n_classes > HALO_COLOR_MAX_CLASSES) return fail(b, HALO_FATAL, "more than HALO_COLOR_MAX_CLASSES colour classes");
  for (int i = 0; i < n_sets; i++) {
    if (sets[i].term_count < 0 || sets[i].term_count > HALO_COLOR_MAX_TERMS) return fail(b, HALO_FATAL, "colour set term_count out of range");
    for (int k = 0; k < sets[i].term_count; k++)
      if (sets[i].terms[k].bit < 0 || sets[i].terms[k].bit > 63) return fail(b, HALO_FATAL, "colour bit outside 0..63");
  }
  const bool same = static_cast<size_t>(n_sets) == b->color_sets.size() && static_cast<size_t>(n_classes) == b->color_classes.size() &&
                    (n_sets == 0 || std::memcmp(b->color_sets.data(), sets, sizeof(HaloColorSet) * static_cast<size_t>(n_sets)) == 0) &&
                    (n_classes == 0 || std::memcmp(b->color_classes.data(), classes, sizeof(HaloColorClass) * static_cast<size_t>(n_classes)) == 0);
  if (same) return HALO_OK;
  b->color_sets.assign(sets, sets + n_sets);
  b->color_classes.assign(classes, classes + n_classes);
  drop_table_cache(b);
  return HALO_OK;
}

int halo_readback_class_lanes(halo_handle_t b, float* lanes, int width, int height, int class_count) {
  if (!b || !lanes) return HALO_FATAL;
  if (class_count != static_cast<int>(b->color_classes.size()) || width != b->lanes_w || height != b->lanes_h || !b->lanes.ptr)
    return fail(b, HALO_FATAL, "class lanes: size does not match the session (classes x width x height)");
  HIPCHK(b, hipSetDevice(b->device));
  if (int rc = join_aux(b)) return rc;
  const size_t n = static_cast<size_t>(class_count) * width * height;
  HIPCHK(b, b->lanes_stage.reserve(n));
  hipError_t e = launch_lanes_drain(b->lanes.ptr, b->lanes_stage.ptr, n, b->cu_count * 8, b->stream);
  if (e != hipSuccess) return hip_fail(b, e, "halo_lanes_drain_kernel launch");
  HIPCHK(b, hipMemcpyAsync(lanes, b->lanes_stage.ptr, n * sizeof(float), hipMemcpyDeviceToHost, b->stream));
  HIPCHK(b, hipStreamSynchronize(b->stream));
  return HALO_OK;
}

int halo_last_sample_counts(halo_handle_t b, uint64_t* crystal_samples, uint64_t* orientation_samples) {
  if (!b) return HALO_FATAL;
  if (crystal_samples) *crystal_samples = b->sess_crystal_samples;
  if (orientation_samples) *orientation_samples = b->sess_orient_samples;
  return HALO_OK;
}

int halo_last_route(halo_handle_t b, HaloRouteInfo* out) {
  if (!b || !out) return HALO_FATAL;
  *out = b->route;
  return HALO_OK;
}

int halo_direct_closes(halo_handle_t b, uint64_t* out) {
  if (!b || !out) return HALO_FATAL;
  *out = b->direct_closes;
  return HALO_OK;
}

int halo_tile_appends(halo_handle_t b, uint64_t* out) {
  if (!b || !out) return HALO_FATAL;
  *out = b->tile_appends;
  return HALO_OK;
}

int halo_last_root_profile(halo_handle_t b, uint32_t* out) {
  if (!b || !out) return HALO_FATAL;
  *out = b->route_root;
  return HALO_OK;
}

int halo_reduce_accumulator(halo_handle_t b, void* nccl_comm, int root, int this_rank) {
  if (!b || !nccl_comm) return HALO_FATAL;
  if (!b->acc || b->acc_w <= 0) return fail(b, HALO_FATAL, "reduce_accumulator before any session");
  typedef int (*nccl_reduce_fn)(const void*, void*, size_t, int, int, int, void*, hipStream_t);
  static nccl_reduce_fn reduce = nullptr;
  static std::once_flag reduce_once;
  std::call_once(reduce_once, [] {
    void* lib = dlopen("librccl.so", RTLD_NOW | RTLD_GLOBAL);
    if (!lib) lib = dlopen("librccl.so.1", RTLD_NOW | RTLD_GLOBAL);
    if (!lib) lib = dlopen("/opt/rocm/lib/librccl.so", RTLD_NOW | RTLD_GLOBAL);
    if (lib) reduce = reinterpret_cast<nccl_reduce_fn>(dlsym(lib, "ncclReduce"));
  });
  if (!reduce) return fail(b, HALO_UNAVAILABLE, "RCCL (librccl.so: ncclReduce) cannot be loaded");
  HIPCHK(b, hipSetDevice(b->device));
  int rc = fold_if_dirty(b);
  if (rc != HALO_OK) return rc;
  const size_t n = static_cast<size_t>(b->acc_w) * static_cast<size_t>(b->acc_h) * 3 + 4;
  if (n > b->acc_floats) return fail(b, HALO_FATAL, "reduce_accumulator: the bound accumulator is smaller than width*height*3+4 floats");
  const int nr = reduce(b->acc, b->acc, n, 7 , 0 , root, nccl_comm, b->stream);
  if (nr != 0) return fail(b, HALO_FATAL, "ncclReduce failed with code " + std::to_string(nr));
  if (this_rank != root) HIPCHK(b, hipMemsetAsync(b->acc, 0, n * sizeof(float), b->stream));
  return HALO_OK;
}

int halo_collect_stats(halo_handle_t b, HaloLayerStats* out) {
  if (!b || !out) return HALO_FATAL;
  HIPCHK(b, hipSetDevice(b->device));
  if (int rc = join_aux(b)) return rc;
  HIPCHK(b, hipStreamSynchronize(b->stream));
  harvest_all(b);
  if (int rc = pull_tally(b)) return rc;
  add_stats(b->pending, b->layer_acc);
  b->layer_acc = HaloLayerStats{};
  *out = b->pending;
  b->pending = HaloLayerStats{};
  return HALO_OK;
}

int halo_collect_timing(halo_handle_t b, double* trace_ms, double* post_ms, uint64_t* launches) {
  if (!b) return HALO_FATAL;
  HIPCHK(b, hipSetDevice(b->device));
  if (int rc = sync_all(b)) return rc;
  harvest_all(b);
  if (trace_ms) *trace_ms = b->time_trace_ms;
  if (post_ms) *post_ms = b->time_post_ms;
  if (launches) *launches = b->time_launches;
  b->time_trace_ms = b->time_post_ms = 0.0;
  b->time_launches = 0;
  return HALO_OK;
}

int halo_recombine(halo_handle_t b, int shuffle, uint64_t* continuation_count) {
  if (!b) return HALO_FATAL;
  if (!b->in_session) return fail(b, HALO_FATAL, "Recombine outside a session");
  if (b->cont_order) {
    const int src = b->cont_out_slot, dst = src ^ 1;
    const uint64_t n_cont = b->cont_in_n;
    const uint64_t planes = b->color_classes.empty() ? 5 : 7;
    const uint64_t stride = std::max<uint64_t>((n_cont + 63) & ~63ull, 64);
    HIPCHK(b, hipSetDevice(b->device));
    if (int rc = reserve_idle(b, b->cont[dst], stride * planes)) return rc;
    if (n_cont > 0) {
      const uint64_t tiles = (b->cont_roots + 2047) / 2048;
      if (int rc = reserve_idle(b, b->cont_base, std::max<uint64_t>(b->cont_roots, 1))) return rc;
      if (int rc = reserve_idle(b, b->cont_tiles, std::max<uint64_t>(tiles, 1))) return rc;
      const hipError_t e = launch_cont_reorder(b->cont[src].ptr, b->cont_stride[src], b->cont_region[src], b->cont_cnt.ptr, b->cont_fill_max, b->cont_mask.ptr,
                                               static_cast<uint32_t>(b->cont_roots), b->cont_tiles.ptr, b->cont_base.ptr, b->cont[dst].ptr, static_cast<uint32_t>(stride),
                                               static_cast<uint32_t>(n_cont), static_cast<uint32_t>(planes), b->cont_err.ptr, b->stream);
      if (e != hipSuccess) return hip_fail(b, e, "halo_cont_scatter_kernel launch");
      uint32_t err = 0;
      HIPCHK(b, hipMemcpyAsync(&err, b->cont_err.ptr, sizeof(uint32_t), hipMemcpyDeviceToHost, b->stream));
      HIPCHK(b, hipStreamSynchronize(b->stream));
      if (err != 0u) return cont_order_fail(b, err);
    }
    b->cont_stride[dst] = static_cast<uint32_t>(stride);
    b->cont_region[dst] = static_cast<uint32_t>(stride);
    b->cont_seg[0] = 0;
    for (int sI = 1; sI <= kContShards; sI++) b->cont_seg[sI] = static_cast<uint32_t>(n_cont);
    b->cont_shuffle = shuffle ? 1 : 0;
    b->layer_idx++;
    if (continuation_count) *continuation_count = b->cont_in_n;
    return HALO_OK;
  }
  b->cont_out_slot ^= 1;
  b->cont_shuffle = shuffle ? 1 : 0;
  b->layer_idx++;
  if (continuation_count) *continuation_count = b->cont_in_n;
  return HALO_OK;
}

int halo_drain_exits(halo_handle_t b, HaloExitRecord* out, uint64_t cap, uint64_t* count) {
  if (!b) return HALO_FATAL;
  HIPCHK(b, hipSetDevice(b->device));
  if (int rc = join_aux(b)) return rc;
  HIPCHK(b, hipStreamSynchronize(b->stream));
  const uint64_t n = b->exits_pending;
  if (!out) {
    if (count) *count = n;
    return HALO_OK;
  }
  const uint64_t take = std::min(n, cap);
  if (count) *count = take;
  if (take) HIPCHK(b, hipMemcpy(out, b->exits.ptr, take * sizeof(HaloExitRecord), hipMemcpyDeviceToHost));
  const uint64_t left = n - take;
  if (left && take) {
    DevBuf<HaloExitRecord> tmp;
    HIPCHK(b, tmp.reserve(left));
    HIPCHK(b, hipMemcpy(tmp.ptr, b->exits.ptr + take, left * sizeof(HaloExitRecord), hipMemcpyDeviceToDevice));
    HIPCHK(b, hipMemcpy(b->exits.ptr, tmp.ptr, left * sizeof(HaloExitRecord), hipMemcpyDeviceToDevice));
    tmp.release();
  }
  b->exits_pending = left;
  const uint32_t left32 = static_cast<uint32_t>(left);
  HIPCHK(b, hipMemcpyAsync(b->counters.ptr + kCntExit, &left32, sizeof(uint32_t), hipMemcpyHostToDevice, b->stream));
  HIPCHK(b, hipStreamSynchronize(b->stream));
  return HALO_OK;
}

int halo_flush(halo_handle_t b) {
  if (!b) return HALO_FATAL;
  if (b->in_session) return fail(b, HALO_FATAL, "halo_flush inside a session");
  HIPCHK(b, hipSetDevice(b->device));
  return fold_if_dirty(b);
}

int halo_sync(halo_handle_t b) {
  if (!b) return HALO_FATAL;
  HIPCHK(b, hipSetDevice(b->device));
  if (b->defer_fold && !b->in_session)
    if (int rc = fold_if_dirty(b)) return rc;
  return sync_all(b);
}

int halo_take_landed(halo_handle_t b, double* landed) {
  if (!b || !landed) return HALO_FATAL;
  HIPCHK(b, hipSetDevice(b->device));
  {
    int rc = fold_if_dirty(b);
    if (rc != HALO_OK) return rc;
  }
  return take_landed_delta(b, landed);
}

int halo_peek_fixed(halo_handle_t b, int32_t plane, uint64_t* sums, uint64_t n_pix, uint32_t* frac_bits, uint64_t* landed, uint32_t* landed_frac_bits) {
  if (!b) return HALO_FATAL;
  if (b->in_session) return fail(b, HALO_FATAL, "halo_peek_fixed inside a session");
  if (!b->mono_dirty || !b->fix_planes || b->acc != b->acc_own.ptr)
    return fail(b, HALO_FATAL, "halo_peek_fixed: no fixed-point planes are pending (needs deterministic = 1, lazy_fold = 1 and the backend's own accumulator, after halo_end and before any reader)");
  if (plane < 0 || static_cast<uint32_t>(plane) >= b->plane_cnt) return fail(b, HALO_FATAL, "halo_peek_fixed: plane outside the session's planes");
  if (sums && n_pix != static_cast<uint64_t>(b->acc_w) * static_cast<uint64_t>(b->acc_h)) return fail(b, HALO_FATAL, "halo_peek_fixed: n_pix is not the session's width * height");
  HIPCHK(b, hipSetDevice(b->device));
  if (int rc = sync_all(b)) return rc;
  if (sums) {
    const size_t slots = static_cast<size_t>(kMonoRows) << b->mono_s_log2;
    std::vector<unsigned long long> host(slots);
    HIPCHK(b, hipMemcpy(host.data(), b->fix.ptr + static_cast<size_t>(plane) * slots, slots * sizeof(unsigned long long), hipMemcpyDeviceToHost));
    for (uint64_t pix = 0; pix < n_pix; pix++) sums[pix] = host[MonoSlot(static_cast<uint32_t>(pix), b->mono_s_log2)];
  }
  if (frac_bits) *frac_bits = b->fix_frac;
  if (landed) {
    double now[kSumNum];
    unsigned long long fix_now = 0ull;
    if (int rc = read_tally(b, now, &fix_now)) return rc;
    *landed = fix_now - b->fix_landed_seen;
  }
  if (landed_frac_bits) *landed_frac_bits = b->fix_frac_landed;
  return HALO_OK;
}

int halo_set_shard(halo_handle_t b, uint32_t index, uint32_t count) {
  if (!b) return HALO_FATAL;
  if (b->in_session) return fail(b, HALO_FATAL, "halo_set_shard inside a session");
  if (count == 0u || index >= count) return fail(b, HALO_FATAL, "halo_set_shard: index " + std::to_string(index) + " outside count " + std::to_string(count) + " (needs count >= 1 and index < count)");
  if (count > 1u && b->rank_opt != 0) return fail(b, HALO_FATAL, "halo_set_shard count > 1: option rank is set (shards trace the one-rank run's rays: they share its counter range)");
  b->shard_index = index;
  b->shard_count = count;
  return HALO_OK;
}

int halo_host_shard_slice(uint64_t share, uint32_t clock, uint32_t index, uint32_t count, uint64_t* first, uint64_t* n) {
  if (!first || !n || clock == 0u || count == 0u || index >= count) return HALO_FATAL;
  shard_slice(share, clock, index, count, first, n);
  return HALO_OK;
}

static int fixed_layout_check(HaloBackend* b, const char* who, uint64_t n_words) {
  if (b->in_session) return fail(b, HALO_FATAL, std::string(who) + " inside a session");
  if (!b->det_session || !b->fix.ptr || !b->acc || b->acc != b->acc_own.ptr)
    return fail(b, HALO_FATAL, std::string(who) + ": the handle's last session was not a deterministic one on the backend's own accumulator");
  const uint64_t want = static_cast<uint64_t>(b->plane_cnt) * static_cast<uint64_t>(b->acc_w) * static_cast<uint64_t>(b->acc_h) + 1u;
  if (n_words != want)
    return fail(b, HALO_FATAL, std::string(who) + ": n_words " + std::to_string(n_words) + " is not plane_cnt * width * height + 1 = " + std::to_string(want) + " of the handle's last session (image size or plane count differ)");
  return HALO_OK;
}

int halo_export_fixed(halo_handle_t b, void* dev_words, uint64_t n_words, uint32_t* plane_cnt, uint32_t* frac_bits, uint32_t* landed_frac_bits) {
  if (!b) return HALO_FATAL;
  if (!dev_words) return fail(b, HALO_FATAL, "halo_export_fixed: dev_words is NULL");
  if (b->in_session) return fail(b, HALO_FATAL, "halo_export_fixed inside a session");
  if (!b->mono_dirty || !b->fix_planes || b->acc != b->acc_own.ptr)
    return fail(b, HALO_FATAL, "halo_export_fixed: no fixed-point planes are pending (needs deterministic = 1, lazy_fold = 1 and the backend's own accumulator, after halo_end and before any reader)");
  if (int rc = fixed_layout_check(b, "halo_export_fixed", n_words)) return rc;
  HIPCHK(b, hipSetDevice(b->device));
  if (int rc = join_aux(b)) return rc;
  double now[kSumNum];
  unsigned long long fix_now = 0ull;
  if (int rc = read_tally(b, now, &fix_now)) return rc;
  const uint32_t npix = static_cast<uint32_t>(b->acc_w) * static_cast<uint32_t>(b->acc_h);
  hipError_t e = launch_export_fixed(b->fix.ptr, static_cast<unsigned long long*>(dev_words), npix, b->mono_s_log2, b->plane_cnt, fix_now - b->fix_landed_seen, b->stream);
  if (e != hipSuccess) return hip_fail(b, e, "halo_export_fixed_kernel launch");
  HIPCHK(b, hipStreamSynchronize(b->stream));
  b->fix_landed_seen = fix_now;
  b->landed_own = false;
  if (plane_cnt) *plane_cnt = b->plane_cnt;
  if (frac_bits) *frac_bits = b->fix_frac;
  if (landed_frac_bits) *landed_frac_bits = b->fix_frac_landed;
  b->fix_hits = 0;
  b->fix_planes = false;
  b->fix_imported = false;
  b->mono_dirty = false;
  return HALO_OK;
}

int halo_import_fixed(halo_handle_t b, const void* dev_words, uint64_t n_words, uint32_t plane_cnt, uint32_t frac_bits, uint32_t landed_frac_bits, uint64_t rays) {
  if (!b) return HALO_FATAL;
  if (!dev_words) return fail(b, HALO_FATAL, "halo_import_fixed: dev_words is NULL");
  if (b->mono_dirty && !b->fix_planes) return fail(b, HALO_FATAL, "halo_import_fixed: float planes are pending (fold them first: halo_flush)");
  if (b->det_session && plane_cnt != b->plane_cnt)
    return fail(b, HALO_FATAL, "halo_import_fixed: plane count " + std::to_string(plane_cnt) + " is not the " + std::to_string(b->plane_cnt) + " of the handle's last session");
  if (int rc = fixed_layout_check(b, "halo_import_fixed", n_words)) return rc;
  if (frac_bits != b->fix_frac) return fail(b, HALO_FATAL, "halo_import_fixed: frac_bits (F) " + std::to_string(frac_bits) + " is not the handle's " + std::to_string(b->fix_frac));
  if (landed_frac_bits != b->fix_frac_landed)
    return fail(b, HALO_FATAL, "halo_import_fixed: landed_frac_bits (F_landed) " + std::to_string(landed_frac_bits) + " is not the handle's " + std::to_string(b->fix_frac_landed));
  const uint64_t held = b->mono_dirty ? b->fix_hits : 0u;
  if (rays > kFixBudgetHits || held + rays > kFixBudgetHits)
    return fail(b, HALO_FATAL, "halo_import_fixed: " + std::to_string(held) + " + " + std::to_string(rays) + " rays would pass the budget of 2^30 rays of one unfolded plane set");
  HIPCHK(b, hipSetDevice(b->device));
  if (int rc = join_aux(b)) return rc;
  const uint32_t npix = static_cast<uint32_t>(b->acc_w) * static_cast<uint32_t>(b->acc_h);
  hipError_t e = launch_import_fixed(b->fix.ptr, static_cast<const unsigned long long*>(dev_words), npix, b->mono_s_log2, b->plane_cnt, b->stream);
  if (e != hipSuccess) return hip_fail(b, e, "halo_import_fixed_kernel launch");
  unsigned long long landed = 0ull;
  HIPCHK(b, hipMemcpyAsync(&landed, static_cast<const unsigned long long*>(dev_words) + (n_words - 1u), sizeof(landed), hipMemcpyDeviceToHost, b->stream));
  HIPCHK(b, hipStreamSynchronize(b->stream));
  b->fix_landed_seen -= landed;
  b->fix_imported = !b->mono_dirty || b->fix_imported;
  b->fix_hits = held + rays;
  b->fix_planes = true;
  b->mono_dirty = true;
  return HALO_OK;
}

int halo_readback_xyz64(halo_handle_t b, float* xyz, int width, int height, double* landed) {
  if (!b || !xyz) return HALO_FATAL;
  if (!b->acc || width != b->acc_w || height != b->acc_h) return fail(b, HALO_FATAL, "readback size does not match the session render");
  HIPCHK(b, hipSetDevice(b->device));
  {
    int rc = fold_if_dirty(b);
    if (rc != HALO_OK) return rc;
  }
  const size_t n = static_cast<size_t>(width) * height * 3;
  HIPCHK(b, hipMemcpyAsync(xyz, b->acc, n * sizeof(float), hipMemcpyDeviceToHost, b->stream));
  HIPCHK(b, hipMemsetAsync(b->acc, 0, (n + 4) * sizeof(float), b->stream));
  double l = 0.0;
  if (int rc = take_landed_delta(b, &l)) return rc;
  if (landed) *landed = l;
  return HALO_OK;
}

int halo_readback_xyz(halo_handle_t b, float* xyz, int width, int height, float* landed_weight) {
  double l = 0.0;
  int rc = halo_readback_xyz64(b, xyz, width, height, &l);
  if (rc == HALO_OK && landed_weight) *landed_weight += static_cast<float>(l);
  return rc;
}

int halo_consumer_reset(halo_handle_t b) {
  if (!b) return HALO_FATAL;
  HIPCHK(b, hipSetDevice(b->device));
  if (int rc = join_aux(b)) return rc;
  if (b->cons_sum.ptr) {
    const size_t n = static_cast<size_t>(b->cons_w) * b->cons_h * 3;
    HIPCHK(b, hipMemsetAsync(b->cons_sum.ptr, 0, n * sizeof(float), b->stream));
    HIPCHK(b, hipMemsetAsync(b->cons_comp.ptr, 0, n * sizeof(float), b->stream));
  }
  if (b->lanes.ptr) HIPCHK(b, hipMemsetAsync(b->lanes.ptr, 0, b->lanes.cap * sizeof(double), b->stream));
  b->total_intensity = 0.0;
  return HALO_OK;
}

int halo_consumer_fold(halo_handle_t b) {
  if (!b) return HALO_FATAL;
  if (!b->acc || b->acc_w <= 0) return fail(b, HALO_FATAL, "consumer_fold before any session");
  HIPCHK(b, hipSetDevice(b->device));
  int rc = fold_if_dirty(b);
  if (rc != HALO_OK) return rc;
  const size_t n = static_cast<size_t>(b->acc_w) * b->acc_h * 3;
  if (b->cons_w != b->acc_w || b->cons_h != b->acc_h || !b->cons_sum.ptr) {
    HIPCHK(b, b->cons_sum.reserve(n));
    HIPCHK(b, b->cons_comp.reserve(n));
    b->cons_w = b->acc_w;
    b->cons_h = b->acc_h;
    HIPCHK(b, hipMemsetAsync(b->cons_sum.ptr, 0, n * sizeof(float), b->stream));
    HIPCHK(b, hipMemsetAsync(b->cons_comp.ptr, 0, n * sizeof(float), b->stream));
    b->total_intensity = 0.0;
  }
  hipError_t e = launch_consumer_fold(b->acc, b->cons_sum.ptr, b->cons_comp.ptr, static_cast<uint32_t>(n), b->cu_count * 8, b->stream);
  if (e != hipSuccess) return hip_fail(b, e, "halo_consumer_fold_kernel launch");
  double landed = 0.0;
  if (int rc = take_landed_delta(b, &landed)) return rc;
  b->total_intensity += landed;
  return HALO_OK;
}

int halo_consumer_consume(halo_handle_t b, const float* xyz, int width, int height, float landed, const float* lanes, int class_count) {
  if (!b || !xyz) return HALO_FATAL;
  if (b->in_session) return fail(b, HALO_FATAL, "consumer_consume inside a session");
  if (width <= 0 || height <= 0) return fail(b, HALO_FATAL, "consumer_consume: empty image");
  if (static_cast<uint64_t>(width) * static_cast<uint64_t>(height) > (1ull << 25)) return fail(b, HALO_UNAVAILABLE, "more than 2^25 pixels");
  if (b->cons_sum.ptr && (b->cons_w != width || b->cons_h != height)) return fail(b, HALO_FATAL, "consumer_consume: image size differs from the consumer's (halo_consumer_reset first)");
  HIPCHK(b, hipSetDevice(b->device));
  if (int rc = join_aux(b)) return rc;
  const size_t n = static_cast<size_t>(width) * height * 3;
  if (!b->cons_sum.ptr) {
    HIPCHK(b, b->cons_sum.reserve(n));
    HIPCHK(b, b->cons_comp.reserve(n));
    b->cons_w = width;
    b->cons_h = height;
    HIPCHK(b, hipMemsetAsync(b->cons_sum.ptr, 0, n * sizeof(float), b->stream));
    HIPCHK(b, hipMemsetAsync(b->cons_comp.ptr, 0, n * sizeof(float), b->stream));
    b->total_intensity = 0.0;
  }
  HIPCHK(b, b->cons_stage.reserve(n));
  HIPCHK(b, hipMemcpyAsync(b->cons_stage.ptr, xyz, n * sizeof(float), hipMemcpyHostToDevice, b->stream));
  hipError_t e = launch_consumer_fold(b->cons_stage.ptr, b->cons_sum.ptr, b->cons_comp.ptr, static_cast<uint32_t>(n), b->cu_count * 8, b->stream);
  if (e != hipSuccess) return hip_fail(b, e, "halo_consumer_fold_kernel launch");
  if (lanes != nullptr && class_count > 0) {
    if (class_count != static_cast<int>(b->color_classes.size())) return fail(b, HALO_FATAL, "consumer_consume: class count must equal halo_set_color's");
    const size_t nl = static_cast<size_t>(class_count) * width * height;
    if (!b->lanes.ptr || b->lanes_w != width || b->lanes_h != height) {
      HIPCHK(b, b->lanes.reserve(nl));
      HIPCHK(b, hipMemsetAsync(b->lanes.ptr, 0, b->lanes.cap * sizeof(double), b->stream));
      b->lanes_w = width;
      b->lanes_h = height;
    }
    HIPCHK(b, b->lanes_stage.reserve(nl));
    HIPCHK(b, hipMemcpyAsync(b->lanes_stage.ptr, lanes, nl * sizeof(float), hipMemcpyHostToDevice, b->stream));
    e = launch_lanes_add(b->lanes_stage.ptr, b->lanes.ptr, nl, b->cu_count * 8, b->stream);
    if (e != hipSuccess) return hip_fail(b, e, "halo_lanes_add_kernel launch");
  }
  HIPCHK(b, hipStreamSynchronize(b->stream));
  b->total_intensity += static_cast<double>(landed);
  return HALO_OK;
}

int halo_consumer_snapshot(halo_handle_t b, const HaloDisplay* dsp, uint8_t* rgb_out, float* xyz_out, double* total_intensity) {
  if (!b || !dsp) return HALO_FATAL;
  if (!b->cons_sum.ptr) return fail(b, HALO_FATAL, "consumer_snapshot before consumer_fold");
  HIPCHK(b, hipSetDevice(b->device));
  const uint32_t npix = static_cast<uint32_t>(b->cons_w) * static_cast<uint32_t>(b->cons_h);
  const size_t n = static_cast<size_t>(npix) * 3;
  const float snapshot_intensity = static_cast<float>(b->total_intensity);
  const float scale = (npix == 0 || snapshot_intensity <= 0.0f) ? 0.0f : dsp->intensity_factor * 0.08f * static_cast<float>(npix) / snapshot_intensity;
  if (rgb_out) HIPCHK(b, b->cons_rgb.reserve(n));
  if (xyz_out) HIPCHK(b, b->cons_xyz_out.reserve(n));
  hipError_t e = launch_post_snapshot(b->cons_sum.ptr, b->cons_comp.ptr, rgb_out ? b->cons_rgb.ptr : nullptr,
                                      xyz_out ? b->cons_xyz_out.ptr : nullptr, npix, scale, dsp->ray_color, dsp->background,
                                      b->cu_count * 8, b->stream);
  if (e != hipSuccess) return hip_fail(b, e, "halo_post_snapshot_kernel launch");
  if (rgb_out) HIPCHK(b, hipMemcpyAsync(rgb_out, b->cons_rgb.ptr, n, hipMemcpyDeviceToHost, b->stream));
  if (xyz_out) HIPCHK(b, hipMemcpyAsync(xyz_out, b->cons_xyz_out.ptr, n * sizeof(float), hipMemcpyDeviceToHost, b->stream));
  HIPCHK(b, hipStreamSynchronize(b->stream));
  if (rgb_out && scale == 0.0f) std::memset(rgb_out, 0, n);
  if (total_intensity) *total_intensity = b->total_intensity;
  return HALO_OK;
}

float halo_host_ev_auto(float p99_y, float per_pixel_intensity, float target_white) {
  if (per_pixel_intensity <= 0.0f || p99_y <= 0.0f) return 0.0f;
  const float p99_norm = p99_y / per_pixel_intensity;
  const float t = target_white / 255.0f;
  const float target_linear = t <= 0.04045f ? t / 12.92f : std::pow((t + 0.055f) / 1.055f, 2.4f);
  if (target_linear <= 0.0f || p99_norm <= 0.0f) return 0.0f;
  const float ev = std::log2f(target_linear / p99_norm);
  return std::min(std::max(ev, -6.0f), 6.0f);
}

int halo_consumer_auto_ev(halo_handle_t b, int32_t downsample_factor, float target_white, HaloAutoEv* out) {
  if (!b) return HALO_FATAL;
  if (!out) return fail(b, HALO_FATAL, "consumer_auto_ev: out is NULL");
  if (!b->cons_sum.ptr) return fail(b, HALO_FATAL, "consumer_auto_ev before consumer_fold");
  if (!(target_white > 0.0f && target_white <= 255.0f)) return fail(b, HALO_FATAL, "consumer_auto_ev: target_white must lie in (0, 255]");
  HIPCHK(b, hipSetDevice(b->device));
  const uint32_t w = static_cast<uint32_t>(b->cons_w), h = static_cast<uint32_t>(b->cons_h), npix = w * h;
  const uint32_t f = downsample_factor > 1 ? static_cast<uint32_t>(downsample_factor) : 1u;
  const bool coarse = f > 1u && w / f > 0u && h / f > 0u;
  const uint32_t wc = coarse ? w / f : 0u, hc = coarse ? h / f : 0u;
  const uint32_t n_vals = coarse ? wc * hc : npix;
  HIPCHK(b, b->aev_vals.reserve(n_vals));
  constexpr size_t kRecWords = sizeof(AevRecord) / sizeof(uint32_t);
  HIPCHK(b, b->aev_ws.reserve(kRecWords + kAevHistWords));
  AevRecord* rec_dev = reinterpret_cast<AevRecord*>(b->aev_ws.ptr);
  hipError_t e = launch_aev_values(b->cons_sum.ptr, b->cons_comp.ptr, w, h, f, wc, hc, b->aev_vals.ptr, b->cu_count * 8, b->stream);
  if (e != hipSuccess) return hip_fail(b, e, "halo_aev value kernel launch");
  const bool one_wg = b->aev_select < 0 ? n_vals <= kAevSmallMax : b->aev_select == 1;
  e = launch_aev_select(b->aev_vals.ptr, n_vals, rec_dev, b->aev_ws.ptr + kRecWords, one_wg, b->aev_agg_hist != 0, b->cu_count, b->stream);
  if (e != hipSuccess) return hip_fail(b, e, "halo_aev select kernel launch");
  AevRecord rec{};
  HIPCHK(b, hipMemcpyAsync(&rec, rec_dev, sizeof(rec), hipMemcpyDeviceToHost, b->stream));
  HIPCHK(b, hipStreamSynchronize(b->stream));
  float p99 = 0.0f;
  if (rec.count) std::memcpy(&p99, &rec.p99_bits, sizeof(float));
  if (coarse) p99 = p99 / (static_cast<float>(f) * static_cast<float>(f));
  const float snapshot_intensity = static_cast<float>(b->total_intensity);
  const int total_pix = b->cons_w * b->cons_h;
  const float per_pixel = total_pix > 0 ? snapshot_intensity / (0.08f * total_pix) : 0.0f;
  out->p99_y = p99;
  out->per_pixel_intensity = per_pixel;
  out->ev_auto = halo_host_ev_auto(p99, per_pixel, target_white);
  out->produced = (p99 > 0.0f && per_pixel > 0.0f) ? 1 : 0;
  out->value_count = rec.count;
  out->coarse_w = static_cast<int32_t>(wc);
  out->coarse_h = static_cast<int32_t>(hc);
  return HALO_OK;
}

int halo_host_parse_composite_mode(const char* mode) {
  if (mode && std::strcmp(mode, "dominant") == 0) return HALO_COMPOSITE_DOMINANT;
  if (mode && std::strcmp(mode, "additive") == 0) return HALO_COMPOSITE_ADDITIVE;
  return HALO_COMPOSITE_PAINTER;
}

int halo_consumer_load_lanes(halo_handle_t b, const float* lanes, int width, int height, int class_count, double total_intensity) {
  if (!b || !lanes) return HALO_FATAL;
  if (b->in_session) return fail(b, HALO_FATAL, "consumer_load_lanes inside a session");
  if (width <= 0 || height <= 0 || class_count <= 0 || class_count != static_cast<int>(b->color_classes.size()))
    return fail(b, HALO_FATAL, "consumer_load_lanes: class count must equal halo_set_color's, image must not be empty");
  if (static_cast<uint64_t>(width) * static_cast<uint64_t>(height) > (1ull << 25)) return fail(b, HALO_UNAVAILABLE, "more than 2^25 pixels");
  HIPCHK(b, hipSetDevice(b->device));
  if (int rc = join_aux(b)) return rc;
  const size_t n = static_cast<size_t>(class_count) * width * height;
  HIPCHK(b, b->lanes.reserve(n));
  b->lanes_w = width;
  b->lanes_h = height;
  HIPCHK(b, b->lanes_stage.reserve(n));
  HIPCHK(b, hipMemcpyAsync(b->lanes_stage.ptr, lanes, n * sizeof(float), hipMemcpyHostToDevice, b->stream));
  hipError_t e = launch_lanes_load(b->lanes_stage.ptr, b->lanes.ptr, n, b->cu_count * 8, b->stream);
  if (e != hipSuccess) return hip_fail(b, e, "halo_lanes_load_kernel launch");
  HIPCHK(b, hipStreamSynchronize(b->stream));
  if (total_intensity >= 0.0) b->total_intensity = total_intensity;
  return HALO_OK;
}

int halo_consumer_composite(halo_handle_t b, const HaloComposite* spec, float* linear_rgb_out, uint8_t* srgb_out, float* participating_p99_y, int32_t* produced) {
  if (!b || !spec || !produced) return HALO_FATAL;
  *produced = 0;
  if (spec->mode < HALO_COMPOSITE_DOMINANT || spec->mode > HALO_COMPOSITE_PAINTER) return fail(b, HALO_FATAL, "consumer_composite: unknown mode");
  uint64_t referenced = 0;
  for (const HaloColorClass& c : b->color_classes) referenced |= c.bits;
  if (referenced == 0) return HALO_OK;
  if (spec->class_count != static_cast<int>(b->color_classes.size())) return fail(b, HALO_FATAL, "consumer_composite: class_count differs from halo_set_color's");
  if (!b->lanes.ptr || b->lanes_w <= 0 || b->lanes_h <= 0) return fail(b, HALO_FATAL, "consumer_composite before any colour session (no lanes)");
  HIPCHK(b, hipSetDevice(b->device));
  if (int rc = join_aux(b)) return rc;
  const uint32_t npix = static_cast<uint32_t>(b->lanes_w) * static_cast<uint32_t>(b->lanes_h);
  const size_t n3 = static_cast<size_t>(npix) * 3u;
  bool any_solo = false;
  for (int c = 0; c < spec->class_count; c++) any_solo = any_solo || spec->classes[c].solo != 0;
  std::vector<int> order(static_cast<size_t>(spec->class_count));
  for (int c = 0; c < spec->class_count; c++) order[static_cast<size_t>(c)] = c;
  std::stable_sort(order.begin(), order.end(), [spec](int x, int y) { return spec->classes[x].z_order < spec->classes[y].z_order; });
  CompositeDev cd{};
  cd.mode = static_cast<uint32_t>(spec->mode);
  for (int c : order) {
    const HaloCompositeClass& k = spec->classes[c];
    if (!(any_solo ? k.solo != 0 : k.visible != 0)) continue;
    cd.lane[cd.n_active] = static_cast<uint32_t>(c);
    for (int j = 0; j < 3; j++) cd.color[cd.n_active][j] = k.color[j];
    cd.n_active++;
  }
  auto deliver_black = [&]() -> int {
    if (linear_rgb_out) std::memset(linear_rgb_out, 0, n3 * sizeof(float));
    if (srgb_out) std::memset(srgb_out, 0, n3);
    if (participating_p99_y) *participating_p99_y = 0.0f;
    *produced = 1;
    return HALO_OK;
  };
  if (cd.n_active == 0) return deliver_black();
  HIPCHK(b, b->comp_hist.reserve(2048));
  std::vector<uint32_t> hist(2048);
  const int blocks = b->cu_count * 8;
  float p99 = 0.0f;
  {
    uint32_t prefix = 0u;
    uint64_t rank = 0;
    const uint32_t shifts[3] = {21u, 10u, 0u}, widths[3] = {11u, 11u, 10u};
    bool empty = false;
    for (int pass = 0; pass < 3 && !empty; pass++) {
      const uint32_t nb = 1u << widths[pass];
      HIPCHK(b, hipMemsetAsync(b->comp_hist.ptr, 0, nb * sizeof(uint32_t), b->stream));
      hipError_t e = launch_lane_hist(b->lanes.ptr, npix, cd, shifts[pass], widths[pass], prefix, b->comp_hist.ptr, blocks, b->stream);
      if (e != hipSuccess) return hip_fail(b, e, "halo_lane_hist_kernel launch");
      HIPCHK(b, hipMemcpyAsync(hist.data(), b->comp_hist.ptr, nb * sizeof(uint32_t), hipMemcpyDeviceToHost, b->stream));
      HIPCHK(b, hipStreamSynchronize(b->stream));
      if (pass == 0) {
        uint64_t count = 0;
        for (uint32_t i = 0; i < nb; i++) count += hist[i];
        if (count == 0) {
          empty = true;
          break;
        }
        uint64_t idx = static_cast<uint64_t>(static_cast<float>(count) * 0.99f);
        if (idx >= count) idx = count - 1;
        rank = idx;
      }
      uint32_t bin = 0;
      for (; bin < nb; bin++) {
        if (rank < hist[bin]) break;
        rank -= hist[bin];
      }
      if (bin >= nb) return fail(b, HALO_FATAL, "consumer_composite: lanes changed under the P99 select");
      prefix = (prefix << widths[pass]) | bin;
    }
    if (!empty) std::memcpy(&p99, &prefix, sizeof(float));
  }
  const float snapshot_intensity = static_cast<float>(b->total_intensity);
  float A = 0.0f;
  if (p99 > 0.0f && snapshot_intensity > 0.0f) {
    const float target_srgb = 135.0f / 255.0f;
    const float target_linear = target_srgb <= 0.04045f ? target_srgb / 12.92f : std::pow((target_srgb + 0.055f) / 1.055f, 2.4f);
    A = spec->intensity_factor * target_linear / p99;
  }
  if (participating_p99_y) *participating_p99_y = p99;
  if (!(A > 0.0f)) {
    if (linear_rgb_out) std::memset(linear_rgb_out, 0, n3 * sizeof(float));
    return HALO_OK;
  }
  cd.a = A;
  cd.s = A * spec->display_exposure_scale;
  cd.display = spec->display_exposure_scale;
  if (linear_rgb_out) HIPCHK(b, b->comp_rgb.reserve(n3));
  if (srgb_out) HIPCHK(b, b->cons_rgb.reserve(n3));
  if (linear_rgb_out || srgb_out) {
    hipError_t e = launch_composite(b->lanes.ptr, npix, cd, linear_rgb_out ? b->comp_rgb.ptr : nullptr, srgb_out ? b->cons_rgb.ptr : nullptr, blocks, b->stream);
    if (e != hipSuccess) return hip_fail(b, e, "halo_composite_kernel launch");
    if (linear_rgb_out) HIPCHK(b, hipMemcpyAsync(linear_rgb_out, b->comp_rgb.ptr, n3 * sizeof(float), hipMemcpyDeviceToHost, b->stream));
    if (srgb_out) HIPCHK(b, hipMemcpyAsync(srgb_out, b->cons_rgb.ptr, n3, hipMemcpyDeviceToHost, b->stream));
    HIPCHK(b, hipStreamSynchronize(b->stream));
  }
  *produced = 1;
  return HALO_OK;
}

int halo_host_prism_geometry(float h, const float dist[6], HaloGeomTables* out) {
  if (!out || !dist) return HALO_FATAL;
  host::BuildPrism(h, dist, *out);
  return HALO_OK;
}
int halo_host_pyramid_geometry(float wu, float wl, float h1, float h2, float h3, const float dist[6], HaloGeomTables* out) {
  if (!out || !dist) return HALO_FATAL;
  return host::BuildPyramid(wu, wl, h1, h2, h3, dist, *out) ? HALO_OK : HALO_UNAVAILABLE;
}
int halo_host_shape_scalars(const HaloCrystal* crystal, uint32_t seed, uint64_t shape_index, int via_plan, float out9[9]) {
  if (!crystal || !out9) return HALO_FATAL;
  const geom::CrystalRecipe rc = host::MakeRecipe(*crystal);
  if (via_plan) {
    for (int q = 0; q < 9; q++) out9[q] = geom::DrawShapeScalarOne(seed, rc, shape_index, q);
  } else {
    geom::DrawShapeScalars(seed, rc, shape_index, out9);
  }
  return HALO_OK;
}
int halo_host_build_lat_lut(const HaloDist* lat, float* theta, float* cdf, float* flip) {
  if (!lat || !theta || !cdf || !flip) return HALO_FATAL;
  host::LatLut l = host::BuildLatLut(*lat);
  std::copy(l.theta.begin(), l.theta.end(), theta);
  std::copy(l.cdf.begin(), l.cdf.end(), cdf);
  std::copy(l.flip.begin(), l.flip.end(), flip);
  return HALO_OK;
}
int halo_host_build_proj_params(const HaloRender* render, void* out76) {
  if (!render || !out76) return HALO_FATAL;
  ProjDev p = host::BuildProj(*render);
  static_assert(sizeof(ProjDev) == 76, "ProjDev mirrors lm_proj::ProjParams");
  std::memcpy(out76, &p, sizeof(p));
  return HALO_OK;
}
int halo_host_partition(const float* prop, int n, uint64_t ray_num, double* carry, uint64_t* out) {
  if (!prop || !carry || !out || n < 0) return HALO_FATAL;
  std::vector<uint64_t> v = host::Partition(prop, n, ray_num, carry);
  std::copy(v.begin(), v.end(), out);
  return HALO_OK;
}
int halo_host_reduce_raypath(const uint8_t* rp, int32_t n, int32_t symmetry, int32_t sigma_a, int32_t d_applicable, uint8_t* out) {
  if (!rp || !out || n < 0 || n > HALO_MAX_HITS) return HALO_FATAL;
  std::vector<uint8_t> v = host::ReduceRaypath(std::vector<uint8_t>(rp, rp + n), static_cast<uint8_t>(symmetry), sigma_a, d_applicable != 0);
  std::copy(v.begin(), v.end(), out);
  return HALO_OK;
}
int halo_host_filter_fast_check(const HaloFilter* f, const HaloAxis* axis, const uint8_t* path, int32_t n, const float dir[3], int32_t crystal_id, int32_t* pass) {
  if (!f || !axis || !pass || n < 0 || n > 16 || (n && !path) || !dir) return HALO_FATAL;
  struct Cache {
    HaloFilter f;
    HaloAxis axis;
    int32_t crystal_id = 0;
    bool valid = false, fits = false;
    FastTables tables;
  };
  static thread_local std::unique_ptr<Cache> cache;
  if (!cache) cache.reset(new Cache());
  if (!cache->valid || std::memcmp(&cache->f, f, sizeof(HaloFilter)) != 0 || std::memcmp(&cache->axis, axis, sizeof(HaloAxis)) != 0 || cache->crystal_id != crystal_id) {
    std::memset(&cache->tables, 0, sizeof(FastTables));
    cache->f = *f;
    cache->axis = *axis;
    cache->crystal_id = crystal_id;
    cache->fits = host::BuildFastTables(f, nullptr, *axis, static_cast<uint32_t>(crystal_id), cache->tables);
    cache->valid = true;
  }
  if (!cache->fits) return HALO_FATAL;
  *pass = host::FastFilterCheck(cache->tables, path, static_cast<uint32_t>(n), dir, static_cast<uint32_t>(crystal_id)) ? 1 : 0;
  return HALO_OK;
}
int halo_host_color_fast_mask(const HaloColorSet* colors, const HaloAxis* axis, const uint8_t* path, int32_t n, const float dir[3], int32_t crystal_id, uint64_t carried,
                              uint64_t* mask) {
  if (!colors || !axis || !mask || n < 0 || n > 16 || (n && !path) || !dir) return HALO_FATAL;
  std::unique_ptr<FastTables> tables(new FastTables());
  std::memset(tables.get(), 0, sizeof(FastTables));
  if (!host::BuildFastTables(nullptr, colors, *axis, static_cast<uint32_t>(crystal_id), *tables)) return HALO_FATAL;
  *mask = host::FastColorMask(*tables, carried, path, static_cast<uint32_t>(n), dir, static_cast<uint32_t>(crystal_id));
  return HALO_OK;
}
// ... 37 lines not shown
```

### ice_halo_sim_amd/csrc/halo_kernels.hip

```cpp
#include "halo_trace.inl"
#include "halo_launch.h"

namespace halo {

constexpr uint32_t kListOnceMin = 1u << 16;
template <bool ONCE>
__device__ __forceinline__ uint4 load_list_u4(const uint4* p) {
  if constexpr (!ONCE) return *p;
  const uint32_t* q = reinterpret_cast<const uint32_t*>(p);
  return make_uint4(__builtin_nontemporal_load(q), __builtin_nontemporal_load(q + 1), __builtin_nontemporal_load(q + 2), __builtin_nontemporal_load(q + 3));
}


constexpr int kBinBlock = 1024;
constexpr uint32_t kBinSplit = 2u;
__global__ void __launch_bounds__(kBinBlock) halo_bin_accumulate_kernel(float* __restrict__ plane, const uint2* __restrict__ list, uint32_t cap,
                                                                         const uint32_t* __restrict__ cnt, uint32_t tiles_log2, uint32_t frac_bits) {
  const FixQ fq(frac_bits);
  __shared__ unsigned long long acc[1u << kBinTileLog2];
  const uint32_t tile = blockIdx.x / kBinSplit, part = blockIdx.x % kBinSplit;
  const uint32_t n = min(cnt[tile * kBinCntStride], cap);
  const uint32_t lo = static_cast<uint32_t>(static_cast<uint64_t>(n) * part / kBinSplit);
  const uint32_t hi = static_cast<uint32_t>(static_cast<uint64_t>(n) * (part + 1u) / kBinSplit);
  if (hi <= lo) return;
// ... 418 lines not shown
      for (uint32_t u = 0; u < kU; ++u) {
        const float w = __uint_as_float(h[u].y);
        if (c4[u].x != 0.0f) atomicAdd(&acc[0][sl[u]], fq.fix(c4[u].x * w));
        if (c4[u].y != 0.0f) atomicAdd(&acc[1][sl[u]], fq.fix(c4[u].y * w));
        if (c4[u].z != 0.0f) atomicAdd(&acc[2][sl[u]], fq.fix(c4[u].z * w));
      }
    } else {
#pragma unroll
      for (uint32_t u = 0; u < kU; ++u) add(h[u]);
    }
  }
  };
  if (n >= kListOnceMin) stream(std::true_type{});
  else stream(std::false_type{});
  for (uint32_t r = 2u * i; r < n; r += 2u * kBinBlock) {
    add(src[r]);
    if (r + 1u < n) add(src[r + 1u]);
  }
  __syncthreads();
  for (uint32_t c = 0; c < CH; ++c) {
    PlaneOf<kFix>* dst = planes + static_cast<size_t>(c) * plane_stride + (static_cast<size_t>(plane_of_tile) << (s_log2 + 10u));
    for (uint32_t j = threadIdx.x; j < slots; j += kBinBlock) {
      if constexpr (kFix) {
        const unsigned long long v = acc[c][j];
        if (v != 0ull) atomicAdd(&dst[map.slot_of(tile_in, j)], v);
      } else {
      const float v = fq.unfix(acc[c][j]);
      if (v != 0.0f) dst[map.slot_of(tile_in, j)] += v;
      }
    }
  }
}

hipError_t launch_log_route(float* plane, const HitRec* log, uint32_t cap1, const uint32_t* cnt1, uint32_t regions, HitRec* list2, uint32_t cap2, uint32_t* cnt2,
                            uint32_t tiles, uint32_t planes, uint32_t s_log2, bool interleaved, uint32_t frac_bits, double* ovf, uint32_t* ovf_flag, uint32_t copies_log2, hipStream_t stream,
                            hipEvent_t before_sums) {
  const uint32_t tiles_log2 = static_cast<uint32_t>(__builtin_ctz(tiles)), tile_log2 = s_log2 + 10u - tiles_log2;
  if (planes > 1u || tiles > 256u) {
    hipLaunchKernelGGL((halo_split_kernel<kLogSplitThreads, kLogSplitPer, 512u, false, true>), dim3(regions), dim3(kLogSplitThreads), 0, stream, plane, reinterpret_cast<const uint2*>(log), cap1, cnt1, 1u,
                       1u, reinterpret_cast<uint2*>(list2), cap2, cnt2, tiles_log2, 0u, 0xFFFFFFFFu, 0u, s_log2, SplitXyz{nullptr, 0u, 0u, ovf, ovf_flag, s_log2 + 10u, copies_log2});
    hipError_t e = hipGetLastError();
    if (e != hipSuccess) return e;
    if (before_sums && (e = hipStreamWaitEvent(stream, before_sums, 0)) != hipSuccess) return e;
    hipLaunchKernelGGL((halo_log_accumulate_kernel<1u>), dim3(tiles * planes), dim3(kBinBlock), 0, stream, plane, 0u, reinterpret_cast<const uint2*>(list2), cap2, cnt2,
                       static_cast<const WlEntryDev*>(nullptr), 0u, tiles_log2, s_log2, frac_bits);
    return hipGetLastError();
  }
  if (interleaved)
    hipLaunchKernelGGL((halo_split_kernel<kLogSplitThreads, kLogSplitPer, 256u, false, true>), dim3(regions), dim3(kLogSplitThreads), 0, stream, plane, reinterpret_cast<const uint2*>(log), cap1, cnt1, 1u,
                       1u, reinterpret_cast<uint2*>(list2), cap2, cnt2, tiles_log2, 0u, 0xFFFFFFFFu, 0u, s_log2, SplitXyz{nullptr, 0u, 0u, ovf, ovf_flag, s_log2 + 10u, copies_log2});
  else
    hipLaunchKernelGGL((halo_split_kernel<kLogSplitThreads, kLogSplitPer, 256u, false, false>), dim3(regions), dim3(kLogSplitThreads), 0, stream, plane, reinterpret_cast<const uint2*>(log), cap1, cnt1, 1u,
                       1u, reinterpret_cast<uint2*>(list2), cap2, cnt2, tiles_log2, 0u, 0xFFFFFFFFu, tile_log2, 0u, SplitXyz{nullptr, 0u, 0u, ovf, ovf_flag, s_log2 + 10u, copies_log2});
  hipError_t e = hipGetLastError();
  if (e != hipSuccess) return e;
  if (before_sums && (e = hipStreamWaitEvent(stream, before_sums, 0)) != hipSuccess) return e;
  if (interleaved)
    hipLaunchKernelGGL((halo_log_accumulate_kernel<1u>), dim3(tiles), dim3(kBinBlock), 0, stream, plane, 0u, reinterpret_cast<const uint2*>(list2), cap2, cnt2,
                       static_cast<const WlEntryDev*>(nullptr), 0u, tiles_log2, s_log2, frac_bits);
  else hipLaunchKernelGGL((halo_bin_accumulate_range_kernel<false>), dim3(tiles), dim3(kBinBlock), 0, stream, plane, reinterpret_cast<const uint2*>(list2), cap2, cnt2, tile_log2, frac_bits, CloseArgsOf<false>{});
  return hipGetLastError();
}

hipError_t launch_log_route_close(float* xyz, uint32_t n_pix, const float* coef, const HitRec* log, uint32_t cap1, const uint32_t* cnt1, uint32_t regions, HitRec* list2,
                                  uint32_t cap2, uint32_t* cnt2, uint32_t tiles, uint32_t s_log2, uint32_t frac_bits, double* ovf, uint32_t* ovf_flag,
                                  hipStream_t stream, hipEvent_t before_sums) {
  if (tiles == 0u || (tiles & (tiles - 1u)) != 0u || tiles > 256u || xyz == nullptr || coef == nullptr || ovf == nullptr || ovf_flag == nullptr) return hipErrorInvalidValue;
  const uint32_t tiles_log2 = static_cast<uint32_t>(__builtin_ctz(tiles));
  if (s_log2 + 10u < tiles_log2 || s_log2 + 10u - tiles_log2 > kBinTileLog2) return hipErrorInvalidValue;
  const uint32_t tile_log2 = s_log2 + 10u - tiles_log2;
  hipLaunchKernelGGL((halo_split_kernel<kLogSplitThreads, kLogSplitPer, 256u, false, false>), dim3(regions), dim3(kLogSplitThreads), 0, stream, static_cast<float*>(nullptr),
                     reinterpret_cast<const uint2*>(log), cap1, cnt1, 1u, 1u, reinterpret_cast<uint2*>(list2), cap2, cnt2, tiles_log2, 0u, 0xFFFFFFFFu, tile_log2, 0u,
                     SplitXyz{nullptr, 0u, 0u, ovf, ovf_flag, s_log2 + 10u, 0u});
  hipError_t e = hipGetLastError();
  if (e != hipSuccess) return e;
  if (before_sums && (e = hipStreamWaitEvent(stream, before_sums, 0)) != hipSuccess) return e;
  const CloseArgsOf<true> cl{xyz, n_pix, s_log2, {coef[0], coef[1], coef[2]}, cnt2, ovf, ovf_flag};
  hipLaunchKernelGGL((halo_bin_accumulate_range_kernel<false, true>), dim3(tiles), dim3(kBinBlock), 0, stream, static_cast<float*>(nullptr), reinterpret_cast<const uint2*>(list2), cap2,
                     static_cast<const uint32_t*>(nullptr), tile_log2, frac_bits, cl);
  if ((e = hipGetLastError()) != hipSuccess) return e;
  return hipMemsetAsync(ovf_flag, 0, sizeof(uint32_t), stream);
}

constexpr uint32_t kChunksInFlight = 16u, kLoads = 1u;
__global__ void __launch_bounds__(kBinBlock) halo_tile_close_kernel(const uint2* __restrict__ chunk, uint32_t cap, const uint32_t* __restrict__ cnt, uint32_t wgs,
                                                                    uint32_t tile_log2, uint32_t frac_bits, const CloseArgsOf<true> cl) {
  __shared__ __attribute__((aligned(16))) unsigned long long acc[1u << kBinTileLog2];
  const FixQ fq(frac_bits);
  const uint32_t tile = blockIdx.x;
  const uint32_t* tcnt = cnt + static_cast<size_t>(tile) * wgs;
  const bool take_twin = *cl.flag != 0u;
  uint32_t any = 0u;
  for (uint32_t c = threadIdx.x; c < wgs; c += kBinBlock) any |= tcnt[c];
  if (!__syncthreads_or(static_cast<int>(any != 0u)) && !take_twin) return;
  const uint32_t slots = 1u << tile_log2, mask = slots - 1u;
  for (uint32_t j = threadIdx.x; j < slots; j += kBinBlock) acc[j] = 0ull;
  __syncthreads();
  const uint32_t lane = threadIdx.x & 63u, wave = threadIdx.x >> 6, waves = kBinBlock / 64u;
  const uint2* tsrc = chunk + static_cast<size_t>(tile) * wgs * cap;
  auto add = [&](uint32_t slot, uint32_t w_bits) { atomicAdd(&acc[slot & mask], fq.fix(__uint_as_float(w_bits))); };
  for (uint32_t c0 = wave * 64u; c0 < wgs; c0 += waves * 64u) {
    const uint32_t mine = c0 + lane < wgs ? min(tcnt[c0 + lane], cap) : 0u;
    if (__ballot(mine != 0u) == 0ull) continue;
    for (uint32_t g = 0; g < 64u; g += kChunksInFlight) {
      uint32_t n[kChunksInFlight], most = 0u;
#pragma unroll
      for (uint32_t k = 0; k < kChunksInFlight; ++k) {
        n[k] = static_cast<uint32_t>(__builtin_amdgcn_readlane(static_cast<int>(mine), static_cast<int>(g + k)));
        most = max(most, n[k]);
      }
      if (most == 0u) continue;
      uint4 h[kChunksInFlight][kLoads];
#pragma unroll
      for (uint32_t k = 0; k < kChunksInFlight; ++k) {
        const uint4* src4 = reinterpret_cast<const uint4*>(tsrc + static_cast<size_t>(c0 + g + k) * cap);
#pragma unroll
        for (uint32_t u = 0; u < kLoads; ++u) {
          const uint32_t i = lane + 64u * u;
          h[k][u] = i < n[k] / 2u ? load_list_u4<true>(&src4[i]) : make_uint4(0u, 0u, 0u, 0u);
        }
      }
#pragma unroll
      for (uint32_t k = 0; k < kChunksInFlight; ++k) {
#pragma unroll
        for (uint32_t u = 0; u < kLoads; ++u) {
          if (lane + 64u * u < n[k] / 2u) {
            add(h[k][u].x, h[k][u].y);
            add(h[k][u].z, h[k][u].w);
          }
        }
      }
#pragma unroll
      for (uint32_t k = 0; k < kChunksInFlight; ++k) {
        const uint2* src = tsrc + static_cast<size_t>(c0 + g + k) * cap;
        const uint4* src4 = reinterpret_cast<const uint4*>(src);
        for (uint32_t i = lane + 64u * kLoads; i < n[k] / 2u; i += 64u) {
          const uint4 q = load_list_u4<true>(&src4[i]);
          add(q.x, q.y);
          add(q.z, q.w);
        }
        if ((n[k] & 1u) != 0u && lane == 0u) {
          const uint2 q = src[n[k] - 1u];
          add(q.x, q.y);
        }
      }
    }
  }
  __syncthreads();
  close_write_out(acc, fq, tile, tile_log2, slots, take_twin, cl);
}

hipError_t launch_tile_route_close(float* xyz, uint32_t n_pix, const float* coef, const HitRec* chunk, uint32_t cap, const uint32_t* cnt, uint32_t wgs, uint32_t tiles,
                                   uint32_t s_log2, uint32_t frac_bits, double* ovf, uint32_t* ovf_flag, hipStream_t stream, hipEvent_t before_sums) {
  if (tiles == 0u || (tiles & (tiles - 1u)) != 0u || tiles > kTileAppendMax || wgs == 0u || cap == 0u || (cap & 1u) != 0u) return hipErrorInvalidValue;
  if (xyz == nullptr || coef == nullptr || chunk == nullptr || cnt == nullptr || ovf == nullptr || ovf_flag == nullptr) return hipErrorInvalidValue;
  const uint32_t tiles_log2 = static_cast<uint32_t>(__builtin_ctz(tiles));
  if (s_log2 + 10u < tiles_log2 || s_log2 + 10u - tiles_log2 > kBinTileLog2) return hipErrorInvalidValue;
  if (static_cast<uint64_t>(tiles) * wgs * cap > (1ull << 30)) return hipErrorInvalidValue;
  hipError_t e = hipSuccess;
  if (before_sums && (e = hipStreamWaitEvent(stream, before_sums, 0)) != hipSuccess) return e;
  const CloseArgsOf<true> cl{xyz, n_pix, s_log2, {coef[0], coef[1], coef[2]}, nullptr, ovf, ovf_flag};
  hipLaunchKernelGGL(halo_tile_close_kernel, dim3(tiles), dim3(kBinBlock), 0, stream, reinterpret_cast<const uint2*>(chunk), cap, cnt, wgs, s_log2 + 10u - tiles_log2, frac_bits, cl);
  if ((e = hipGetLastError()) != hipSuccess) return e;
  return hipMemsetAsync(ovf_flag, 0, sizeof(uint32_t), stream);
}

hipError_t launch_log_route_xyz(float* planes, uint32_t plane_stride, const HitRec* log, uint32_t cap1, const uint32_t* cnt1, uint32_t regions, HitRec* list2,
                                uint32_t cap2, uint32_t* cnt2, uint32_t tiles, uint32_t s_log2, const WlEntryDev* pool, uint32_t pool_size, uint32_t frac_bits,
                                double* ovf, uint32_t* ovf_flag, uint32_t copies_log2, hipStream_t stream, hipEvent_t before_sums) {
  const uint32_t tiles_log2 = static_cast<uint32_t>(__builtin_ctz(tiles));
  hipLaunchKernelGGL((halo_split_kernel<kLogSplitThreads, kLogSplitPer, 512u, true, true>), dim3(regions), dim3(kLogSplitThreads), 0, stream, planes, reinterpret_cast<const uint2*>(log), cap1, cnt1, 1u, 1u,
                     reinterpret_cast<uint2*>(list2), cap2, cnt2, tiles_log2, 0u, (1u << kLogWlShift) - 1u, 0u, s_log2, SplitXyz{pool, pool_size, plane_stride, ovf, ovf_flag, s_log2 + 10u, copies_log2});
  hipError_t e = hipGetLastError();
  if (e != hipSuccess) return e;
  if (before_sums && (e = hipStreamWaitEvent(stream, before_sums, 0)) != hipSuccess) return e;
  hipLaunchKernelGGL((halo_log_accumulate_kernel<3u>), dim3(tiles), dim3(kBinBlock), 0, stream, planes, plane_stride, reinterpret_cast<const uint2*>(list2), cap2, cnt2,
                     pool, pool_size, tiles_log2, s_log2, frac_bits);
  return hipGetLastError();
}

hipError_t launch_log_route_fixed(unsigned long long* fix, const HitRec* log, uint32_t cap1, const uint32_t* cnt1, uint32_t regions, HitRec* list2, uint32_t cap2,
                                  uint32_t* cnt2, uint32_t tiles, uint32_t s_log2, bool interleaved, uint32_t frac_bits, hipStream_t stream) {
  const uint32_t tiles_log2 = static_cast<uint32_t>(__builtin_ctz(tiles)), tile_log2 = s_log2 + 10u - tiles_log2;
  if (tiles > 512u || tile_log2 > kBinTileLog2) return hipErrorInvalidValue;
  const uint2* l1 = reinterpret_cast<const uint2*>(log);
  uint2* l2 = reinterpret_cast<uint2*>(list2);
  const SplitXyz none{nullptr, 0u, 0u, nullptr, nullptr, 0u, 0u};
  const SplitFix sf{fix, frac_bits};
  const bool mix = interleaved || tiles > 256u;
  if (tiles > 256u)
    hipLaunchKernelGGL((halo_split_fixed_kernel<kLogSplitThreads, kLogSplitPer, 512u, false, true>), dim3(regions), dim3(kLogSplitThreads), 0, stream, l1, cap1, cnt1, l2, cap2, cnt2,
                       tiles_log2, 0xFFFFFFFFu, 0u, s_log2, none, sf);
  else if (mix)
    hipLaunchKernelGGL((halo_split_fixed_kernel<kLogSplitThreads, kLogSplitPer, 256u, false, true>), dim3(regions), dim3(kLogSplitThreads), 0, stream, l1, cap1, cnt1, l2, cap2, cnt2,
                       tiles_log2, 0xFFFFFFFFu, 0u, s_log2, none, sf);
  else
    hipLaunchKernelGGL((halo_split_fixed_kernel<kLogSplitThreads, kLogSplitPer, 256u, false, false>), dim3(regions), dim3(kLogSplitThreads), 0, stream, l1, cap1, cnt1, l2, cap2, cnt2,
                       tiles_log2, 0xFFFFFFFFu, tile_log2, 0u, none, sf);
  hipError_t e = hipGetLastError();
  if (e != hipSuccess) return e;
  if (mix)
    hipLaunchKernelGGL((halo_log_accumulate_kernel<1u, true>), dim3(tiles), dim3(kBinBlock), 0, stream, fix, 0u, reinterpret_cast<const uint2*>(list2), cap2, cnt2,
                       static_cast<const WlEntryDev*>(nullptr), 0u, tiles_log2, s_log2, frac_bits);
  else hipLaunchKernelGGL((halo_bin_accumulate_range_kernel<true>), dim3(tiles), dim3(kBinBlock), 0, stream, fix, reinterpret_cast<const uint2*>(list2), cap2, cnt2, tile_log2, frac_bits, CloseArgsOf<false>{});
  return hipGetLastError();
}

hipError_t launch_log_route_xyz_fixed(unsigned long long* fix, uint32_t plane_stride, const HitRec* log, uint32_t cap1, const uint32_t* cnt1, uint32_t regions, HitRec* list2,
                                      uint32_t cap2, uint32_t* cnt2, uint32_t tiles, uint32_t s_log2, const WlEntryDev* pool, uint32_t pool_size, uint32_t frac_bits,
                                      hipStream_t stream) {
  const uint32_t tiles_log2 = static_cast<uint32_t>(__builtin_ctz(tiles));
  if (tiles > 512u || s_log2 + 10u - tiles_log2 > 12u || pool_size > HALO_WL_POOL_MAX) return hipErrorInvalidValue;
  hipLaunchKernelGGL((halo_split_fixed_kernel<kLogSplitThreads, kLogSplitPer, 512u, true, true>), dim3(regions), dim3(kLogSplitThreads), 0, stream, reinterpret_cast<const uint2*>(log), cap1, cnt1,
                     reinterpret_cast<uint2*>(list2), cap2, cnt2, tiles_log2, (1u << kLogWlShift) - 1u, 0u, s_log2, SplitXyz{pool, pool_size, plane_stride, nullptr, nullptr, 0u, 0u},
                     SplitFix{fix, frac_bits});
  hipError_t e = hipGetLastError();
  if (e != hipSuccess) return e;
  hipLaunchKernelGGL((halo_log_accumulate_kernel<3u, true>), dim3(tiles), dim3(kBinBlock), 0, stream, fix, plane_stride, reinterpret_cast<const uint2*>(list2), cap2, cnt2,
                     pool, pool_size, tiles_log2, s_log2, frac_bits);
  return hipGetLastError();
}

hipError_t launch_bin_two_level(float* plane, const HitRec* list1, uint32_t cap1, uint32_t* cnt1, uint32_t lists1, HitRec* list2, uint32_t cap2,
                                uint32_t* cnt2, uint32_t tiles, uint32_t fan_log2, uint32_t frac_bits, double* ovf, uint32_t* ovf_flag, hipStream_t stream, hipEvent_t before_sums) {
  hipLaunchKernelGGL((halo_split_kernel<256u, 16u, 256u, false, false>), dim3(lists1 * kSplitParts), dim3(256u), 0, stream, plane, reinterpret_cast<const uint2*>(list1), cap1,
                     cnt1, static_cast<uint32_t>(kBinCntStride), kSplitParts, reinterpret_cast<uint2*>(list2), cap2, cnt2, fan_log2, 1u, 0xFFFFFFFFu,
                     static_cast<uint32_t>(kBinTileLog2), 0u, SplitXyz{nullptr, 0u, 0u, ovf, ovf_flag, 0u, 0u});
  hipError_t e = hipGetLastError();
  if (e != hipSuccess) return e;
  if (before_sums && (e = hipStreamWaitEvent(stream, before_sums, 0)) != hipSuccess) return e;
// ... 586 lines not shown
```

Before: 27.72 billion.

## Double-buffer tile close loads and trim redundant cross-stream event records

The tile close kernel now walks chunk lists in batches, prefetching the next group of loads into a second register buffer while accumulating the current one. It also keeps the first per-tile counts in registers so the emptiness check reuses them. On the host, main-stream-to-compute-stream event waits are skipped when nothing new was enqueued on the main stream, and the close, set-free and ring-finish markers share one recorded event instead of several. This is meant to hide global-load latency in the close and cut per-launch API overhead. In exchange it adds register pressure and new dirty-tracking logic that has to cover every main-stream enqueue.

```diff
diff --git a/ice_halo_sim_amd/csrc/halo_backend.cpp b/ice_halo_sim_amd/csrc/halo_backend.cpp
--- a/ice_halo_sim_amd/csrc/halo_backend.cpp
+++ b/ice_halo_sim_amd/csrc/halo_backend.cpp
@@ -48,9 +48,18 @@
 
 struct Marker {
   hipEvent_t ev = nullptr;
+  hipEvent_t at = nullptr;
   bool set = false;
-  hipError_t mark(hipStream_t s) { const hipError_t e = hipEventRecord(ev, s); set = set || e == hipSuccess; return e; }
-  hipError_t wait_on(hipStream_t s) const { return set ? hipStreamWaitEvent(s, ev, 0) : hipSuccess; }
+  hipError_t mark(hipStream_t s) {
+    const hipError_t e = hipEventRecord(ev, s);
+    if (e == hipSuccess) at = ev, set = true;
+    return e;
+  }
+  hipError_t mark_at(hipEvent_t shared) {
+    at = shared, set = true;
+    return hipSuccess;
+  }
+  hipError_t wait_on(hipStream_t s) const { return set ? hipStreamWaitEvent(s, at, 0) : hipSuccess; }
   void clear() { set = false; }
 };
 
@@ -83,6 +92,8 @@
   hipEvent_t ev_cs[2] = {nullptr, nullptr}, ev_main = nullptr, ev_aux = nullptr;
   bool cs_pending[2] = {false, false};
   int cs_next = 0;
+  bool main_dirty[2] = {true, true};
+  int lean_events = 1;
   uint64_t aux_seq = 0, cs_seen_aux[2] = {0, 0};
   int overlap = 1;
   int defer_fold = 0;
@@ -173,6 +184,7 @@
   DevBuf<DispatchSlot> ring_dev;
   DispatchSlot* ring_host = nullptr;
   hipEvent_t ring_ev0[kRing] = {}, ring_ev1[kRing] = {}, ring_ev2[kRing] = {}, ring_ev3[kRing] = {}, ring_done[kRing] = {};
+  hipEvent_t ring_t2[kRing] = {}, ring_fin[kRing] = {};
   bool ring_posts[kRing] = {};
   bool ring_final[kRing] = {};
   bool ring_busy[kRing] = {};
@@ -265,11 +277,15 @@
     if (e__ != hipSuccess) return hip_fail(b, e__, #call); \
   } while (0)
 
+inline hipStream_t main_q(HaloBackend* b) {
+  b->main_dirty[0] = b->main_dirty[1] = true;
+  return b->stream;
+}
 inline float* planes_of(HaloBackend* b) { return b->mono.ptr + (b->mono_two ? static_cast<size_t>(b->mono_set) * b->mono_half : 0u); }
 inline hipStream_t post_stream(HaloBackend* b) { return b->overlap ? b->aux : b->stream; }
 int fork_aux(HaloBackend* b) {
   if (!b->overlap) return HALO_OK;
-  HIPCHK(b, hipEventRecord(b->ev_fork, b->stream));
+  HIPCHK(b, hipEventRecord(b->ev_fork, main_q(b)));
   HIPCHK(b, hipStreamWaitEvent(b->aux, b->ev_fork, 0));
   for (int k = 0; k < 2; k++)
     if (b->cs_pending[k]) {
@@ -283,13 +299,13 @@
 int join_aux(HaloBackend* b) {
   if (b->aux_pending) {
     HIPCHK(b, hipEventRecord(b->ev_join, b->aux));
-    HIPCHK(b, hipStreamWaitEvent(b->stream, b->ev_join, 0));
+    HIPCHK(b, hipStreamWaitEvent(main_q(b), b->ev_join, 0));
     b->aux_pending = false;
   }
   for (int k = 0; k < 2; k++)
     if (b->cs_pending[k]) {
       HIPCHK(b, hipEventRecord(b->ev_cs[k], b->cs[k]));
-      HIPCHK(b, hipStreamWaitEvent(b->stream, b->ev_cs[k], 0));
+      HIPCHK(b, hipStreamWaitEvent(main_q(b), b->ev_cs[k], 0));
       b->cs_pending[k] = false;
       b->rmw[k].clear();
       if (b->close_ts == k) b->close_done.clear();
@@ -312,8 +328,11 @@
   }
   const int i = alternate ? b->cs_next : 0;
   if (alternate) b->cs_next ^= 1;
-  HIPCHK(b, hipEventRecord(b->ev_main, b->stream));
-  HIPCHK(b, hipStreamWaitEvent(b->cs[i], b->ev_main, 0));
+  if (!b->lean_events || b->main_dirty[i] || b->stream != b->own_stream) {
+    HIPCHK(b, hipEventRecord(b->ev_main, b->stream));
+    HIPCHK(b, hipStreamWaitEvent(b->cs[i], b->ev_main, 0));
+    b->main_dirty[i] = false;
+  }
   if (touches_planes)
     if (int rc = wait_for_aux(b, i)) return rc;
   b->cs_pending[i] = true;
@@ -324,7 +343,7 @@
 inline uint64_t log_min_rays(int visible) { return visible == HALO_VISIBLE_FULL ? (1ull << 19) : (2ull << 20); }
 int sync_all(HaloBackend* b) {
   if (int rc = join_aux(b)) return rc;
-  HIPCHK(b, hipStreamSynchronize(b->stream));
+  HIPCHK(b, hipStreamSynchronize(main_q(b)));
   return HALO_OK;
 }
 template <typename T>
@@ -362,7 +381,7 @@
     if (int rc = join_aux(b)) return rc;
     if (b->own_w != 0 || b->own_h != 0)
       if (int rc = forget_landed(b)) return rc;
-    HIPCHK(b, hipMemsetAsync(b->acc_own.ptr, 0, need * sizeof(float), b->stream));
+    HIPCHK(b, hipMemsetAsync(b->acc_own.ptr, 0, need * sizeof(float), main_q(b)));
     b->own_w = w;
     b->own_h = h;
   }
@@ -375,10 +394,10 @@
 
 void harvest_slot(HaloBackend* b, int k) {
   if (!b->ring_busy[k]) return;
-  (void)hipEventSynchronize(b->ring_done[k]);
+  (void)hipEventSynchronize(b->ring_fin[k]);
   float ms = 0.0f, ms2 = 0.0f;
   (void)hipEventElapsedTime(&ms, b->ring_ev0[k], b->ring_ev1[k]);
-  if (b->ring_posts[k]) (void)hipEventElapsedTime(&ms2, b->ring_ev2[k], b->ring_ev3[k]);
+  if (b->ring_posts[k]) (void)hipEventElapsedTime(&ms2, b->ring_t2[k], b->ring_ev3[k]);
   static const bool debug_timing = std::getenv("HALO_DEBUG_TIMING") != nullptr;
   if (debug_timing) std::fprintf(stderr, "[halo timing] slot %d final %d posts %d trace %.4f ms passes %.4f ms\n", k, int(b->ring_final[k]), int(b->ring_posts[k]), ms, ms2);
   const bool timed = ms >= 0.0f && ms2 >= 0.0f;
@@ -392,8 +411,8 @@
   b->ring_busy[k] = false;
 }
 int read_tally(HaloBackend* b, double out[kSumNum], unsigned long long* fix_landed = nullptr) {
-  HIPCHK(b, hipMemcpyAsync(b->tally_host, b->tally.ptr, kTallyLines * kTallyStride * sizeof(double), hipMemcpyDeviceToHost, b->stream));
-  HIPCHK(b, hipStreamSynchronize(b->stream));
+  HIPCHK(b, hipMemcpyAsync(b->tally_host, b->tally.ptr, kTallyLines * kTallyStride * sizeof(double), hipMemcpyDeviceToHost, main_q(b)));
+  HIPCHK(b, hipStreamSynchronize(main_q(b)));
   if (fix_landed) {
     *fix_landed = 0ull;
     for (uint32_t l = 0; l < kTallyLines; l++) {
@@ -504,8 +523,8 @@
     halo_destroy(b);
     return HALO_UNAVAILABLE;
   }
-  (void)hipMemsetAsync(b->tally.ptr, 0, kTallyLines * kTallyStride * sizeof(double), b->stream);
-  (void)hipMemsetAsync(b->counters.ptr, 0, kCntNum * sizeof(uint32_t), b->stream);
+  (void)hipMemsetAsync(b->tally.ptr, 0, kTallyLines * kTallyStride * sizeof(double), main_q(b));
+  (void)hipMemsetAsync(b->counters.ptr, 0, kCntNum * sizeof(uint32_t), main_q(b));
   *out = b;
   return HALO_OK;
 }
@@ -513,7 +532,7 @@
 int halo_destroy(halo_handle_t b) {
   if (!b) return HALO_OK;
   (void)hipSetDevice(b->device);
-  (void)hipStreamSynchronize(b->stream);
+  (void)hipStreamSynchronize(main_q(b));
   if (b->aux) (void)hipStreamSynchronize(b->aux);
   for (int k = 0; k < 2; k++)
     if (b->cs[k]) (void)hipStreamSynchronize(b->cs[k]);
@@ -589,6 +608,7 @@
   else if (k == "auto_ev_select") b->aev_select = v < 0 ? -1 : (v ? 1 : 0);
   else if (k == "gen_ahead") b->gen_ahead = v ? 1 : 0;
   else if (k == "close_direct") b->close_direct = v < 0 ? -1 : (v ? 1 : 0);
+  else if (k == "lean_events") b->lean_events = v ? 1 : 0;
   else if (k == "tile_append") b->tile_append = v < 0 ? -1 : (v ? 1 : 0);
   else if (k == "pool_entry_fast") b->pool_entry_fast = v ? 1 : 0;
   else if (k == "rehit_strategy") {
@@ -644,6 +664,7 @@
   if (!b) return HALO_FATAL;
   (void)sync_all(b);
   b->stream = s ? static_cast<hipStream_t>(s) : b->own_stream;
+  b->main_dirty[0] = b->main_dirty[1] = true;
   return HALO_OK;
 }
 
@@ -799,7 +820,7 @@
     b->mono_set = 0;
     if (b->fix.cap < need) {
       if (int rc = reserve_idle(b, b->fix, need)) return rc;
-      HIPCHK(b, hipMemsetAsync(b->fix.ptr, 0, b->fix.cap * sizeof(unsigned long long), b->stream));
+      HIPCHK(b, hipMemsetAsync(b->fix.ptr, 0, b->fix.cap * sizeof(unsigned long long), main_q(b)));
     }
     b->mono_s_log2 = s_log2;
   } else {
@@ -810,7 +831,7 @@
     const size_t need = one * (b->mono_two ? 2u : 1u);
     if (b->mono.cap < need) {
       if (int rc = reserve_idle(b, b->mono, need)) return rc;
-      HIPCHK(b, hipMemsetAsync(b->mono.ptr, 0, b->mono.cap * sizeof(float), b->stream));
+      HIPCHK(b, hipMemsetAsync(b->mono.ptr, 0, b->mono.cap * sizeof(float), main_q(b)));
     }
     b->mono_s_log2 = s_log2;
     const size_t twin_need = (static_cast<size_t>(kMonoRows) << s_log2) * b->plane_cnt;
@@ -818,9 +839,9 @@
       hipError_t oe = hipSuccess;
       if (int rc = reserve_idle(b, b->ovf, 2u * twin_need, &oe)) return rc;
       bool ok = oe == hipSuccess;
-      if (ok && !b->ovf_flag.ptr) ok = b->ovf_flag.reserve(2) == hipSuccess && hipMemsetAsync(b->ovf_flag.ptr, 0, 2 * sizeof(uint32_t), b->stream) == hipSuccess;
+      if (ok && !b->ovf_flag.ptr) ok = b->ovf_flag.reserve(2) == hipSuccess && hipMemsetAsync(b->ovf_flag.ptr, 0, 2 * sizeof(uint32_t), main_q(b)) == hipSuccess;
       if (ok) {
-        HIPCHK(b, hipMemsetAsync(b->ovf.ptr, 0, b->ovf.cap * sizeof(double), b->stream));
+        HIPCHK(b, hipMemsetAsync(b->ovf.ptr, 0, b->ovf.cap * sizeof(double), main_q(b)));
       } else {
         (void)hipGetLastError();
         b->ovf.release();
@@ -833,7 +854,7 @@
     if (b->lanes.cap < need || b->lanes_w != render->width || b->lanes_h != render->height) {
       if (int rc = reserve_idle(b, b->lanes, need)) return rc;
       if (int rc = join_aux(b)) return rc;
-      HIPCHK(b, hipMemsetAsync(b->lanes.ptr, 0, b->lanes.cap * sizeof(double), b->stream));
+      HIPCHK(b, hipMemsetAsync(b->lanes.ptr, 0, b->lanes.cap * sizeof(double), main_q(b)));
       b->lanes_w = render->width;
       b->lanes_h = render->height;
     }
@@ -1202,9 +1223,12 @@
   if (c.source == kSrcTransit) std::copy(b->cont_seg, b->cont_seg + kContShards + 1, hs.seg);
   if (ce && ce->read_ring[ce->cur] >= 0) {
     const int rk = ce->read_ring[ce->cur];
-    if (b->ring_busy[rk] && b->ring_use[rk] == ce->read_use[ce->cur]) HIPCHK(b, hipStreamWaitEvent(b->stream, b->ring_done[rk], 0));
-  }
-  HIPCHK(b, hipMemcpyAsync(ds, &hs, T.fast_host ? sizeof(DispatchSlot) : offsetof(DispatchSlot, fast), hipMemcpyHostToDevice, b->stream));
+    if (b->ring_busy[rk] && b->ring_use[rk] == ce->read_use[ce->cur]) {
+      HIPCHK(b, hipStreamWaitEvent(b->stream, b->ring_fin[rk], 0));
+      b->main_dirty[0] = b->main_dirty[1] = true;
+    }
+  }
+  HIPCHK(b, hipMemcpyAsync(ds, &hs, T.fast_host ? sizeof(DispatchSlot) : offsetof(DispatchSlot, fast), hipMemcpyHostToDevice, main_q(b)));
   if (ce) {
     ce->valid = true, ce->mode = T.mode, ce->use_filter = T.use_filter, ce->use_color = T.use_color;
     ce->entry_fast = T.entry_fast, ce->hex_regular = T.hex_regular, ce->has_fast = T.has_fast;
@@ -1293,14 +1317,14 @@
   if (p.use_log) {
     if (int rc = reserve_idle(b, bin_cnt, std::max<size_t>(static_cast<size_t>(p.blocks), static_cast<size_t>(512) * 16u))) return rc;
     if (int rc = reserve_idle(b, bin_cnt2, static_cast<size_t>(512) * 16u)) return rc;
-    HIPCHK(b, b->set_free[ls].wait_on(b->stream));
+    HIPCHK(b, b->set_free[ls].wait_on(main_q(b)));
   } else if (p.use_bin) {
     if (int rc = reserve_idle(b, bin_cnt, static_cast<size_t>(512) * 16u)) return rc;
-    HIPCHK(b, hipMemsetAsync(bin_cnt.ptr, 0, static_cast<size_t>(p.two_level ? 512u : p.bin_tiles) * 16u * sizeof(uint32_t), b->stream));
+    HIPCHK(b, hipMemsetAsync(bin_cnt.ptr, 0, static_cast<size_t>(p.two_level ? 512u : p.bin_tiles) * 16u * sizeof(uint32_t), main_q(b)));
     if (int rc = reserve_idle(b, bin_list, p.cap1 * p.lists1)) return rc;
     if (p.two_level) {
       if (int rc = reserve_idle(b, bin_cnt2, static_cast<size_t>(p.bin_tiles) * 16u)) return rc;
-      HIPCHK(b, hipMemsetAsync(bin_cnt2.ptr, 0, static_cast<size_t>(p.bin_tiles) * 16u * sizeof(uint32_t), b->stream));
+      HIPCHK(b, hipMemsetAsync(bin_cnt2.ptr, 0, static_cast<size_t>(p.bin_tiles) * 16u * sizeof(uint32_t), main_q(b)));
       b->cnt2_clean[ls] = false;
       if (int rc = reserve_idle(b, bin_list2, p.cap2 * p.bin_tiles)) return rc;
     }
@@ -1417,6 +1441,7 @@
     HIPCHK(b, hipEventRecord(b->ring_ev1[k], ts));
     b->ring_posts[k] = false;
     HIPCHK(b, hipEventRecord(b->ring_done[k], ts));
+    b->ring_fin[k] = b->ring_done[k];
     return HALO_OK;
   }
   HIPCHK(b, hipEventRecord(b->ring_ev1[k], ts));
@@ -1426,7 +1451,25 @@
       HIPCHK(b, b->set_folded[b->mono_set].wait_on(ps));
     } else if (int rc = wait_for_aux(b, ts_i)) return rc;
   }
-  HIPCHK(b, hipEventRecord(b->ring_ev2[k], ps));
+  if (b->lean_events && !p.under_fold()) b->ring_t2[k] = b->ring_ev1[k];
+  else {
+    HIPCHK(b, hipEventRecord(b->ring_ev2[k], ps));
+    b->ring_t2[k] = b->ring_ev2[k];
+  }
+  auto close_marks = [&]() -> hipError_t {
+    hipError_t e = hipEventRecord(b->ring_ev3[k], ps);
+    if (e != hipSuccess) return e;
+    if (b->lean_events) {
+      (void)b->close_done.mark_at(b->ring_ev3[k]);
+      (void)b->set_free[S.ls].mark_at(b->ring_ev3[k]);
+      b->ring_fin[k] = b->ring_ev3[k];
+      return hipSuccess;
+    }
+    if ((e = b->close_done.mark(ps)) != hipSuccess) return e;
+    if ((e = b->set_free[S.ls].mark(ps)) != hipSuccess) return e;
+    b->ring_fin[k] = b->ring_done[k];
+    return hipEventRecord(b->ring_done[k], ps);
+  };
   if (p.close && p.tile) {
     const float coef[3] = {b->plane_coef[0][0], b->plane_coef[0][1], b->plane_coef[0][2]};
     hipError_t ce = launch_tile_route_close(b->acc, static_cast<uint32_t>(b->acc_w) * static_cast<uint32_t>(b->acc_h), coef, P.tile_chunk, P.tile_cap, P.tile_cnt,
@@ -1434,13 +1477,21 @@
     if (ce != hipSuccess) return hip_fail(b, ce, "halo_tile_close_kernel launch");
     b->direct_closes++;
     b->tile_appends++;
-    HIPCHK(b, b->close_done.mark(ps));
+    static const bool debug_counts = std::getenv("HALO_DEBUG_TILE_COUNTS") != nullptr;
+    if (debug_counts) {
+      std::vector<uint32_t> cnt(static_cast<size_t>(P.tile_tiles) * static_cast<size_t>(p.blocks));
+      HIPCHK(b, hipStreamSynchronize(ps));
+      HIPCHK(b, hipMemcpy(cnt.data(), P.tile_cnt, cnt.size() * sizeof(uint32_t), hipMemcpyDeviceToHost));
+      uint64_t met = 0, over = 0, most = 0, empty = 0;
+      for (uint32_t c : cnt) met += c, over += c > P.tile_cap ? 1u : 0u, most = std::max<uint64_t>(most, c), empty += c == 0u ? 1u : 0u;
+      std::fprintf(stderr, "[halo tile counts] workgroups %d tiles %u cap %u chunks %zu records %llu per chunk %.1f longest %llu empty %llu over cap %llu\n", p.blocks, P.tile_tiles,
+                   P.tile_cap, cnt.size(), static_cast<unsigned long long>(met), static_cast<double>(met) / static_cast<double>(cnt.size()), static_cast<unsigned long long>(most),
+                   static_cast<unsigned long long>(empty), static_cast<unsigned long long>(over));
+    }
+    HIPCHK(b, close_marks());
     b->close_ts = ts_i;
-    HIPCHK(b, hipEventRecord(b->ring_ev3[k], ps));
-    HIPCHK(b, b->set_free[S.ls].mark(ps));
     if (b->overlap && p.alternate) b->log_set ^= 1;
     b->ring_posts[k] = true;
-    HIPCHK(b, hipEventRecord(b->ring_done[k], ps));
     return HALO_OK;
   }
   if (p.close) {
@@ -1452,13 +1503,10 @@
     if (ce != hipSuccess) return hip_fail(b, ce, "halo_split_kernel launch (direct close)");
     b->cnt2_clean[S.ls] = true;
     b->direct_closes++;
-    HIPCHK(b, b->close_done.mark(ps));
+    HIPCHK(b, close_marks());
     b->close_ts = ts_i;
-    HIPCHK(b, hipEventRecord(b->ring_ev3[k], ps));
-    HIPCHK(b, b->set_free[S.ls].mark(ps));
     if (b->overlap && p.alternate) b->log_set ^= 1;
     b->ring_posts[k] = true;
-    HIPCHK(b, hipEventRecord(b->ring_done[k], ps));
     return HALO_OK;
   }
   HIPCHK(b, hipMemsetAsync(bin_cnt2.ptr, 0, static_cast<size_t>(p.log_tiles) * 16u * sizeof(uint32_t), ps));
@@ -1479,6 +1527,7 @@
   if (b->overlap && p.alternate) b->log_set ^= 1;
   b->ring_posts[k] = true;
   HIPCHK(b, hipEventRecord(b->ring_done[k], ps));
+  b->ring_fin[k] = b->ring_done[k];
   return HALO_OK;
 }
 int queue_launch(HaloBackend* b, const LaunchPlan& p, const HaloEntry& E, EntryTables& T, const DispatchParams& P, const LaunchSlots& S) {
@@ -1590,8 +1639,8 @@
     if (turn)
       if (int rc = reserve_idle(b, b->shapes_s[S.shape_set ^ 1], p.shape_cnt)) return rc;
     if (p.host_pool) {
-      HIPCHK(b, b->shapes_free[S.shape_set].wait_on(b->stream));
-      HIPCHK(b, hipMemcpyAsync(shapes.ptr, pool.data(), pool.size() * sizeof(ShapeDev), hipMemcpyHostToDevice, b->stream));
+      HIPCHK(b, b->shapes_free[S.shape_set].wait_on(main_q(b)));
+      HIPCHK(b, hipMemcpyAsync(shapes.ptr, pool.data(), pool.size() * sizeof(ShapeDev), hipMemcpyHostToDevice, main_q(b)));
     }
     P.shapes = shapes.ptr;
   }
@@ -1625,7 +1674,7 @@
   p.close = close_direct_ok(*b, p, P);
   if (int rc = bind_tile_append(b, p, T, S.ls, P)) return rc;
   if (int rc = queue_launch(b, p, E, T, P, S)) return rc;
-  if (p.host_pool) HIPCHK(b, hipStreamSynchronize(b->stream));
+  if (p.host_pool) HIPCHK(b, hipStreamSynchronize(main_q(b)));
   if (P.source == kSrcGen) b->gen_count += m;
   if (P.source == kSrcTransit) b->transit_count += m;
   b->gate_count += m;
@@ -1689,14 +1738,14 @@
   if (int rc = join_aux(b)) return rc;
   uint32_t cnt[kCntNum] = {0, 0, 0, 0};
   std::vector<uint32_t> fill(c.final_layer ? 0 : kContShards * kContCntStride);
-  HIPCHK(b, hipMemcpyAsync(cnt, b->counters.ptr, sizeof(cnt), hipMemcpyDeviceToHost, b->stream));
-  if (!c.final_layer) HIPCHK(b, hipMemcpyAsync(fill.data(), b->cont_cnt.ptr, fill.size() * sizeof(uint32_t), hipMemcpyDeviceToHost, b->stream));
+  HIPCHK(b, hipMemcpyAsync(cnt, b->counters.ptr, sizeof(cnt), hipMemcpyDeviceToHost, main_q(b)));
+  if (!c.final_layer) HIPCHK(b, hipMemcpyAsync(fill.data(), b->cont_cnt.ptr, fill.size() * sizeof(uint32_t), hipMemcpyDeviceToHost, main_q(b)));
   uint32_t cont_err = 0;
-  if (c.canon_check) HIPCHK(b, hipMemcpyAsync(&cont_err, b->cont_err.ptr, sizeof(uint32_t), hipMemcpyDeviceToHost, b->stream));
+  if (c.canon_check) HIPCHK(b, hipMemcpyAsync(&cont_err, b->cont_err.ptr, sizeof(uint32_t), hipMemcpyDeviceToHost, main_q(b)));
   if (b->tally_unread) {
     if (int rc = pull_tally(b)) return rc;
   } else {
-    HIPCHK(b, hipStreamSynchronize(b->stream));
+    HIPCHK(b, hipStreamSynchronize(main_q(b)));
   }
   harvest_all(b);
   if (cont_err != 0u)
@@ -1779,14 +1828,14 @@
     b->cont_region[c.out_slot] = static_cast<uint32_t>(region);
     c.out_cap = static_cast<uint32_t>(region);
     HIPCHK(b, b->cont_cnt.reserve(kContShards * kContCntStride));
-    HIPCHK(b, hipMemsetAsync(b->cont_cnt.ptr, 0, kContShards * kContCntStride * sizeof(uint32_t), b->stream));
+    HIPCHK(b, hipMemsetAsync(b->cont_cnt.ptr, 0, kContShards * kContCntStride * sizeof(uint32_t), main_q(b)));
     if (b->cont_order) {
       if (b->rehit_strategy == 0) return fail(b, HALO_FATAL, "cont_order = 1 needs rehit_strategy = 1 (the legacy strategy can emit twice at one interaction)");
       if (int rc = reserve_idle(b, b->cont_mask, kContMaskWords * std::max<uint64_t>(c.n, 1))) return rc;
-      HIPCHK(b, hipMemsetAsync(b->cont_mask.ptr, 0, kContMaskWords * c.n * sizeof(uint32_t), b->stream));
+      HIPCHK(b, hipMemsetAsync(b->cont_mask.ptr, 0, kContMaskWords * c.n * sizeof(uint32_t), main_q(b)));
       if (c.layer == 0) {
         if (int rc = reserve_idle(b, b->cont_err, 16)) return rc;
-        HIPCHK(b, hipMemsetAsync(b->cont_err.ptr, 0, sizeof(uint32_t), b->stream));
+        HIPCHK(b, hipMemsetAsync(b->cont_err.ptr, 0, sizeof(uint32_t), main_q(b)));
       }
     }
   }
@@ -1803,7 +1852,7 @@
       DevBuf<HaloExitRecord> bigger;
       HIPCHK(b, bigger.reserve(need));
       if (b->exits_pending)
-        HIPCHK(b, hipMemcpyAsync(bigger.ptr, b->exits.ptr, b->exits_pending * sizeof(HaloExitRecord), hipMemcpyDeviceToDevice, b->stream));
+        HIPCHK(b, hipMemcpyAsync(bigger.ptr, b->exits.ptr, b->exits_pending * sizeof(HaloExitRecord), hipMemcpyDeviceToDevice, main_q(b)));
       if (int rc = sync_all(b)) return rc;
       b->exits.release();
       b->exits = bigger;
@@ -1814,11 +1863,11 @@
     if (int rc = join_aux(b)) return rc;
     if (int rc = reserve_idle(b, b->host_f, n * 7)) return rc;
     if (int rc = reserve_idle(b, b->host_u, n)) return rc;
-    HIPCHK(b, hipMemcpyAsync(b->host_f.ptr, rays->d, n * 3 * sizeof(float), hipMemcpyHostToDevice, b->stream));
-    HIPCHK(b, hipMemcpyAsync(b->host_f.ptr + n * 3, rays->p, n * 3 * sizeof(float), hipMemcpyHostToDevice, b->stream));
-    HIPCHK(b, hipMemcpyAsync(b->host_f.ptr + n * 6, rays->w, n * sizeof(float), hipMemcpyHostToDevice, b->stream));
-    HIPCHK(b, hipMemcpyAsync(b->host_u.ptr, rays->tf, n * sizeof(uint32_t), hipMemcpyHostToDevice, b->stream));
-    HIPCHK(b, hipStreamSynchronize(b->stream));
+    HIPCHK(b, hipMemcpyAsync(b->host_f.ptr, rays->d, n * 3 * sizeof(float), hipMemcpyHostToDevice, main_q(b)));
+    HIPCHK(b, hipMemcpyAsync(b->host_f.ptr + n * 3, rays->p, n * 3 * sizeof(float), hipMemcpyHostToDevice, main_q(b)));
+    HIPCHK(b, hipMemcpyAsync(b->host_f.ptr + n * 6, rays->w, n * sizeof(float), hipMemcpyHostToDevice, main_q(b)));
+    HIPCHK(b, hipMemcpyAsync(b->host_u.ptr, rays->tf, n * sizeof(uint32_t), hipMemcpyHostToDevice, main_q(b)));
+    HIPCHK(b, hipStreamSynchronize(main_q(b)));
   }
   EntryTables T;
   DispatchParams P{};
@@ -1849,8 +1898,8 @@
     HIPCHK(b, dev.reserve(n));
     std::vector<ShapePrism> recs(n);
     hipError_t ge = launch_shapegen(dev.ptr, true, n, b->seed, host::MakeRecipe(*crystal), first_index, b->stream, b->gen_serial != 0);
-    if (ge == hipSuccess) ge = hipMemcpyAsync(recs.data(), dev.ptr, static_cast<size_t>(n) * sizeof(ShapePrism), hipMemcpyDeviceToHost, b->stream);
-    if (ge == hipSuccess) ge = hipStreamSynchronize(b->stream);
+    if (ge == hipSuccess) ge = hipMemcpyAsync(recs.data(), dev.ptr, static_cast<size_t>(n) * sizeof(ShapePrism), hipMemcpyDeviceToHost, main_q(b));
+    if (ge == hipSuccess) ge = hipStreamSynchronize(main_q(b));
     dev.release();
     if (ge != hipSuccess) return hip_fail(b, ge, "halo_prismgen_team_kernel");
     for (uint32_t k = 0; k < n; k++) {
@@ -1871,8 +1920,8 @@
     DevBuf<ShapeDev> dev;
     HIPCHK(b, dev.reserve(n));
     hipError_t ge = launch_shapegen(dev.ptr, false, n, b->seed, host::MakeRecipe(*crystal), first_index, b->stream, b->gen_serial != 0);
-    if (ge == hipSuccess) ge = hipMemcpyAsync(pool.data(), dev.ptr, static_cast<size_t>(n) * sizeof(ShapeDev), hipMemcpyDeviceToHost, b->stream);
-    if (ge == hipSuccess) ge = hipStreamSynchronize(b->stream);
+    if (ge == hipSuccess) ge = hipMemcpyAsync(pool.data(), dev.ptr, static_cast<size_t>(n) * sizeof(ShapeDev), hipMemcpyDeviceToHost, main_q(b));
+    if (ge == hipSuccess) ge = hipStreamSynchronize(main_q(b));
     dev.release();
     if (ge != hipSuccess) return hip_fail(b, ge, "halo_shapegen_kernel");
   } else {
@@ -1909,10 +1958,10 @@
   if (int rc = join_aux(b)) return rc;
   const size_t n = static_cast<size_t>(class_count) * width * height;
   HIPCHK(b, b->lanes_stage.reserve(n));
-  hipError_t e = launch_lanes_drain(b->lanes.ptr, b->lanes_stage.ptr, n, b->cu_count * 8, b->stream);
+  hipError_t e = launch_lanes_drain(b->lanes.ptr, b->lanes_stage.ptr, n, b->cu_count * 8, main_q(b));
   if (e != hipSuccess) return hip_fail(b, e, "halo_lanes_drain_kernel launch");
-  HIPCHK(b, hipMemcpyAsync(lanes, b->lanes_stage.ptr, n * sizeof(float), hipMemcpyDeviceToHost, b->stream));
-  HIPCHK(b, hipStreamSynchronize(b->stream));
+  HIPCHK(b, hipMemcpyAsync(lanes, b->lanes_stage.ptr, n * sizeof(float), hipMemcpyDeviceToHost, main_q(b)));
+  HIPCHK(b, hipStreamSynchronize(main_q(b)));
   return HALO_OK;
 }
 
@@ -1965,9 +2014,9 @@
   if (rc != HALO_OK) return rc;
   const size_t n = static_cast<size_t>(b->acc_w) * static_cast<size_t>(b->acc_h) * 3 + 4;
   if (n > b->acc_floats) return fail(b, HALO_FATAL, "reduce_accumulator: the bound accumulator is smaller than width*height*3+4 floats");
-  const int nr = reduce(b->acc, b->acc, n, 7 , 0 , root, nccl_comm, b->stream);
+  const int nr = reduce(b->acc, b->acc, n, 7 , 0 , root, nccl_comm, main_q(b));
   if (nr != 0) return fail(b, HALO_FATAL, "ncclReduce failed with code " + std::to_string(nr));
-  if (this_rank != root) HIPCHK(b, hipMemsetAsync(b->acc, 0, n * sizeof(float), b->stream));
+  if (this_rank != root) HIPCHK(b, hipMemsetAsync(b->acc, 0, n * sizeof(float), main_q(b)));
   return HALO_OK;
 }
 
@@ -1975,7 +2024,7 @@
   if (!b || !out) return HALO_FATAL;
   HIPCHK(b, hipSetDevice(b->device));
   if (int rc = join_aux(b)) return rc;
-  HIPCHK(b, hipStreamSynchronize(b->stream));
+  HIPCHK(b, hipStreamSynchronize(main_q(b)));
   harvest_all(b);
   if (int rc = pull_tally(b)) return rc;
   add_stats(b->pending, b->layer_acc);
@@ -2014,11 +2063,11 @@
       if (int rc = reserve_idle(b, b->cont_tiles, std::max<uint64_t>(tiles, 1))) return rc;
       const hipError_t e = launch_cont_reorder(b->cont[src].ptr, b->cont_stride[src], b->cont_region[src], b->cont_cnt.ptr, b->cont_fill_max, b->cont_mask.ptr,
                                                static_cast<uint32_t>(b->cont_roots), b->cont_tiles.ptr, b->cont_base.ptr, b->cont[dst].ptr, static_cast<uint32_t>(stride),
-                                               static_cast<uint32_t>(n_cont), static_cast<uint32_t>(planes), b->cont_err.ptr, b->stream);
+                                               static_cast<uint32_t>(n_cont), static_cast<uint32_t>(planes), b->cont_err.ptr, main_q(b));
       if (e != hipSuccess) return hip_fail(b, e, "halo_cont_scatter_kernel launch");
       uint32_t err = 0;
-      HIPCHK(b, hipMemcpyAsync(&err, b->cont_err.ptr, sizeof(uint32_t), hipMemcpyDeviceToHost, b->stream));
-      HIPCHK(b, hipStreamSynchronize(b->stream));
+      HIPCHK(b, hipMemcpyAsync(&err, b->cont_err.ptr, sizeof(uint32_t), hipMemcpyDeviceToHost, main_q(b)));
+      HIPCHK(b, hipStreamSynchronize(main_q(b)));
       if (err != 0u) return cont_order_fail(b, err);
     }
     b->cont_stride[dst] = static_cast<uint32_t>(stride);
@@ -2041,7 +2090,7 @@
   if (!b) return HALO_FATAL;
   HIPCHK(b, hipSetDevice(b->device));
   if (int rc = join_aux(b)) return rc;
-  HIPCHK(b, hipStreamSynchronize(b->stream));
+  HIPCHK(b, hipStreamSynchronize(main_q(b)));
   const uint64_t n = b->exits_pending;
   if (!out) {
     if (count) *count = n;
@@ -2060,8 +2109,8 @@
   }
   b->exits_pending = left;
   const uint32_t left32 = static_cast<uint32_t>(left);
-  HIPCHK(b, hipMemcpyAsync(b->counters.ptr + kCntExit, &left32, sizeof(uint32_t), hipMemcpyHostToDevice, b->stream));
-  HIPCHK(b, hipStreamSynchronize(b->stream));
+  HIPCHK(b, hipMemcpyAsync(b->counters.ptr + kCntExit, &left32, sizeof(uint32_t), hipMemcpyHostToDevice, main_q(b)));
+  HIPCHK(b, hipStreamSynchronize(main_q(b)));
   return HALO_OK;
 }
 
@@ -2155,9 +2204,9 @@
   unsigned long long fix_now = 0ull;
   if (int rc = read_tally(b, now, &fix_now)) return rc;
   const uint32_t npix = static_cast<uint32_t>(b->acc_w) * static_cast<uint32_t>(b->acc_h);
-  hipError_t e = launch_export_fixed(b->fix.ptr, static_cast<unsigned long long*>(dev_words), npix, b->mono_s_log2, b->plane_cnt, fix_now - b->fix_landed_seen, b->stream);
+  hipError_t e = launch_export_fixed(b->fix.ptr, static_cast<unsigned long long*>(dev_words), npix, b->mono_s_log2, b->plane_cnt, fix_now - b->fix_landed_seen, main_q(b));
   if (e != hipSuccess) return hip_fail(b, e, "halo_export_fixed_kernel launch");
-  HIPCHK(b, hipStreamSynchronize(b->stream));
+  HIPCHK(b, hipStreamSynchronize(main_q(b)));
   b->fix_landed_seen = fix_now;
   b->landed_own = false;
   if (plane_cnt) *plane_cnt = b->plane_cnt;
@@ -2186,11 +2235,11 @@
   HIPCHK(b, hipSetDevice(b->device));
   if (int rc = join_aux(b)) return rc;
   const uint32_t npix = static_cast<uint32_t>(b->acc_w) * static_cast<uint32_t>(b->acc_h);
-  hipError_t e = launch_import_fixed(b->fix.ptr, static_cast<const unsigned long long*>(dev_words), npix, b->mono_s_log2, b->plane_cnt, b->stream);
+  hipError_t e = launch_import_fixed(b->fix.ptr, static_cast<const unsigned long long*>(dev_words), npix, b->mono_s_log2, b->plane_cnt, main_q(b));
   if (e != hipSuccess) return hip_fail(b, e, "halo_import_fixed_kernel launch");
   unsigned long long landed = 0ull;
-  HIPCHK(b, hipMemcpyAsync(&landed, static_cast<const unsigned long long*>(dev_words) + (n_words - 1u), sizeof(landed), hipMemcpyDeviceToHost, b->stream));
-  HIPCHK(b, hipStreamSynchronize(b->stream));
+  HIPCHK(b, hipMemcpyAsync(&landed, static_cast<const unsigned long long*>(dev_words) + (n_words - 1u), sizeof(landed), hipMemcpyDeviceToHost, main_q(b)));
+  HIPCHK(b, hipStreamSynchronize(main_q(b)));
   b->fix_landed_seen -= landed;
   b->fix_imported = !b->mono_dirty || b->fix_imported;
   b->fix_hits = held + rays;
@@ -2208,8 +2257,8 @@
     if (rc != HALO_OK) return rc;
   }
   const size_t n = static_cast<size_t>(width) * height * 3;
-  HIPCHK(b, hipMemcpyAsync(xyz, b->acc, n * sizeof(float), hipMemcpyDeviceToHost, b->stream));
-  HIPCHK(b, hipMemsetAsync(b->acc, 0, (n + 4) * sizeof(float), b->stream));
+  HIPCHK(b, hipMemcpyAsync(xyz, b->acc, n * sizeof(float), hipMemcpyDeviceToHost, main_q(b)));
+  HIPCHK(b, hipMemsetAsync(b->acc, 0, (n + 4) * sizeof(float), main_q(b)));
   double l = 0.0;
   if (int rc = take_landed_delta(b, &l)) return rc;
   if (landed) *landed = l;
@@ -2229,10 +2278,10 @@
   if (int rc = join_aux(b)) return rc;
   if (b->cons_sum.ptr) {
     const size_t n = static_cast<size_t>(b->cons_w) * b->cons_h * 3;
-    HIPCHK(b, hipMemsetAsync(b->cons_sum.ptr, 0, n * sizeof(float), b->stream));
-    HIPCHK(b, hipMemsetAsync(b->cons_comp.ptr, 0, n * sizeof(float), b->stream));
-  }
-  if (b->lanes.ptr) HIPCHK(b, hipMemsetAsync(b->lanes.ptr, 0, b->lanes.cap * sizeof(double), b->stream));
+    HIPCHK(b, hipMemsetAsync(b->cons_sum.ptr, 0, n * sizeof(float), main_q(b)));
+    HIPCHK(b, hipMemsetAsync(b->cons_comp.ptr, 0, n * sizeof(float), main_q(b)));
+  }
+  if (b->lanes.ptr) HIPCHK(b, hipMemsetAsync(b->lanes.ptr, 0, b->lanes.cap * sizeof(double), main_q(b)));
   b->total_intensity = 0.0;
   return HALO_OK;
 }
@@ -2249,11 +2298,11 @@
     HIPCHK(b, b->cons_comp.reserve(n));
     b->cons_w = b->acc_w;
     b->cons_h = b->acc_h;
-    HIPCHK(b, hipMemsetAsync(b->cons_sum.ptr, 0, n * sizeof(float), b->stream));
-    HIPCHK(b, hipMemsetAsync(b->cons_comp.ptr, 0, n * sizeof(float), b->stream));
+    HIPCHK(b, hipMemsetAsync(b->cons_sum.ptr, 0, n * sizeof(float), main_q(b)));
+    HIPCHK(b, hipMemsetAsync(b->cons_comp.ptr, 0, n * sizeof(float), main_q(b)));
     b->total_intensity = 0.0;
   }
-  hipError_t e = launch_consumer_fold(b->acc, b->cons_sum.ptr, b->cons_comp.ptr, static_cast<uint32_t>(n), b->cu_count * 8, b->stream);
+  hipError_t e = launch_consumer_fold(b->acc, b->cons_sum.ptr, b->cons_comp.ptr, static_cast<uint32_t>(n), b->cu_count * 8, main_q(b));
   if (e != hipSuccess) return hip_fail(b, e, "halo_consumer_fold_kernel launch");
   double landed = 0.0;
   if (int rc = take_landed_delta(b, &landed)) return rc;
@@ -2275,29 +2324,29 @@
     HIPCHK(b, b->cons_comp.reserve(n));
     b->cons_w = width;
     b->cons_h = height;
-    HIPCHK(b, hipMemsetAsync(b->cons_sum.ptr, 0, n * sizeof(float), b->stream));
-    HIPCHK(b, hipMemsetAsync(b->cons_comp.ptr, 0, n * sizeof(float), b->stream));
+    HIPCHK(b, hipMemsetAsync(b->cons_sum.ptr, 0, n * sizeof(float), main_q(b)));
+    HIPCHK(b, hipMemsetAsync(b->cons_comp.ptr, 0, n * sizeof(float), main_q(b)));
     b->total_intensity = 0.0;
   }
   HIPCHK(b, b->cons_stage.reserve(n));
-  HIPCHK(b, hipMemcpyAsync(b->cons_stage.ptr, xyz, n * sizeof(float), hipMemcpyHostToDevice, b->stream));
-  hipError_t e = launch_consumer_fold(b->cons_stage.ptr, b->cons_sum.ptr, b->cons_comp.ptr, static_cast<uint32_t>(n), b->cu_count * 8, b->stream);
+  HIPCHK(b, hipMemcpyAsync(b->cons_stage.ptr, xyz, n * sizeof(float), hipMemcpyHostToDevice, main_q(b)));
+  hipError_t e = launch_consumer_fold(b->cons_stage.ptr, b->cons_sum.ptr, b->cons_comp.ptr, static_cast<uint32_t>(n), b->cu_count * 8, main_q(b));
   if (e != hipSuccess) return hip_fail(b, e, "halo_consumer_fold_kernel launch");
   if (lanes != nullptr && class_count > 0) {
     if (class_count != static_cast<int>(b->color_classes.size())) return fail(b, HALO_FATAL, "consumer_consume: class count must equal halo_set_color's");
     const size_t nl = static_cast<size_t>(class_count) * width * height;
     if (!b->lanes.ptr || b->lanes_w != width || b->lanes_h != height) {
       HIPCHK(b, b->lanes.reserve(nl));
-      HIPCHK(b, hipMemsetAsync(b->lanes.ptr, 0, b->lanes.cap * sizeof(double), b->stream));
+      HIPCHK(b, hipMemsetAsync(b->lanes.ptr, 0, b->lanes.cap * sizeof(double), main_q(b)));
       b->lanes_w = width;
       b->lanes_h = height;
     }
     HIPCHK(b, b->lanes_stage.reserve(nl));
-    HIPCHK(b, hipMemcpyAsync(b->lanes_stage.ptr, lanes, nl * sizeof(float), hipMemcpyHostToDevice, b->stream));
-    e = launch_lanes_add(b->lanes_stage.ptr, b->lanes.ptr, nl, b->cu_count * 8, b->stream);
+    HIPCHK(b, hipMemcpyAsync(b->lanes_stage.ptr, lanes, nl * sizeof(float), hipMemcpyHostToDevice, main_q(b)));
+    e = launch_lanes_add(b->lanes_stage.ptr, b->lanes.ptr, nl, b->cu_count * 8, main_q(b));
     if (e != hipSuccess) return hip_fail(b, e, "halo_lanes_add_kernel launch");
   }
-  HIPCHK(b, hipStreamSynchronize(b->stream));
+  HIPCHK(b, hipStreamSynchronize(main_q(b)));
   b->total_intensity += static_cast<double>(landed);
   return HALO_OK;
 }
@@ -2314,11 +2363,11 @@
   if (xyz_out) HIPCHK(b, b->cons_xyz_out.reserve(n));
   hipError_t e = launch_post_snapshot(b->cons_sum.ptr, b->cons_comp.ptr, rgb_out ? b->cons_rgb.ptr : nullptr,
                                       xyz_out ? b->cons_xyz_out.ptr : nullptr, npix, scale, dsp->ray_color, dsp->background,
-                                      b->cu_count * 8, b->stream);
+                                      b->cu_count * 8, main_q(b));
   if (e != hipSuccess) return hip_fail(b, e, "halo_post_snapshot_kernel launch");
-  if (rgb_out) HIPCHK(b, hipMemcpyAsync(rgb_out, b->cons_rgb.ptr, n, hipMemcpyDeviceToHost, b->stream));
-  if (xyz_out) HIPCHK(b, hipMemcpyAsync(xyz_out, b->cons_xyz_out.ptr, n * sizeof(float), hipMemcpyDeviceToHost, b->stream));
-  HIPCHK(b, hipStreamSynchronize(b->stream));
+  if (rgb_out) HIPCHK(b, hipMemcpyAsync(rgb_out, b->cons_rgb.ptr, n, hipMemcpyDeviceToHost, main_q(b)));
+  if (xyz_out) HIPCHK(b, hipMemcpyAsync(xyz_out, b->cons_xyz_out.ptr, n * sizeof(float), hipMemcpyDeviceToHost, main_q(b)));
+  HIPCHK(b, hipStreamSynchronize(main_q(b)));
   if (rgb_out && scale == 0.0f) std::memset(rgb_out, 0, n);
   if (total_intensity) *total_intensity = b->total_intensity;
   return HALO_OK;
@@ -2349,14 +2398,14 @@
   constexpr size_t kRecWords = sizeof(AevRecord) / sizeof(uint32_t);
   HIPCHK(b, b->aev_ws.reserve(kRecWords + kAevHistWords));
   AevRecord* rec_dev = reinterpret_cast<AevRecord*>(b->aev_ws.ptr);
-  hipError_t e = launch_aev_values(b->cons_sum.ptr, b->cons_comp.ptr, w, h, f, wc, hc, b->aev_vals.ptr, b->cu_count * 8, b->stream);
+  hipError_t e = launch_aev_values(b->cons_sum.ptr, b->cons_comp.ptr, w, h, f, wc, hc, b->aev_vals.ptr, b->cu_count * 8, main_q(b));
   if (e != hipSuccess) return hip_fail(b, e, "halo_aev value kernel launch");
   const bool one_wg = b->aev_select < 0 ? n_vals <= kAevSmallMax : b->aev_select == 1;
-  e = launch_aev_select(b->aev_vals.ptr, n_vals, rec_dev, b->aev_ws.ptr + kRecWords, one_wg, b->aev_agg_hist != 0, b->cu_count, b->stream);
+  e = launch_aev_select(b->aev_vals.ptr, n_vals, rec_dev, b->aev_ws.ptr + kRecWords, one_wg, b->aev_agg_hist != 0, b->cu_count, main_q(b));
   if (e != hipSuccess) return hip_fail(b, e, "halo_aev select kernel launch");
   AevRecord rec{};
-  HIPCHK(b, hipMemcpyAsync(&rec, rec_dev, sizeof(rec), hipMemcpyDeviceToHost, b->stream));
-  HIPCHK(b, hipStreamSynchronize(b->stream));
+  HIPCHK(b, hipMemcpyAsync(&rec, rec_dev, sizeof(rec), hipMemcpyDeviceToHost, main_q(b)));
+  HIPCHK(b, hipStreamSynchronize(main_q(b)));
   float p99 = 0.0f;
   if (rec.count) std::memcpy(&p99, &rec.p99_bits, sizeof(float));
   if (coarse) p99 = p99 / (static_cast<float>(f) * static_cast<float>(f));
@@ -2392,10 +2441,10 @@
   b->lanes_w = width;
   b->lanes_h = height;
   HIPCHK(b, b->lanes_stage.reserve(n));
-  HIPCHK(b, hipMemcpyAsync(b->lanes_stage.ptr, lanes, n * sizeof(float), hipMemcpyHostToDevice, b->stream));
-  hipError_t e = launch_lanes_load(b->lanes_stage.ptr, b->lanes.ptr, n, b->cu_count * 8, b->stream);
+  HIPCHK(b, hipMemcpyAsync(b->lanes_stage.ptr, lanes, n * sizeof(float), hipMemcpyHostToDevice, main_q(b)));
+  hipError_t e = launch_lanes_load(b->lanes_stage.ptr, b->lanes.ptr, n, b->cu_count * 8, main_q(b));
   if (e != hipSuccess) return hip_fail(b, e, "halo_lanes_load_kernel launch");
-  HIPCHK(b, hipStreamSynchronize(b->stream));
+  HIPCHK(b, hipStreamSynchronize(main_q(b)));
   if (total_intensity >= 0.0) b->total_intensity = total_intensity;
   return HALO_OK;
 }
@@ -2446,11 +2495,11 @@
     bool empty = false;
     for (int pass = 0; pass < 3 && !empty; pass++) {
       const uint32_t nb = 1u << widths[pass];
-      HIPCHK(b, hipMemsetAsync(b->comp_hist.ptr, 0, nb * sizeof(uint32_t), b->stream));
-      hipError_t e = launch_lane_hist(b->lanes.ptr, npix, cd, shifts[pass], widths[pass], prefix, b->comp_hist.ptr, blocks, b->stream);
+      HIPCHK(b, hipMemsetAsync(b->comp_hist.ptr, 0, nb * sizeof(uint32_t), main_q(b)));
+      hipError_t e = launch_lane_hist(b->lanes.ptr, npix, cd, shifts[pass], widths[pass], prefix, b->comp_hist.ptr, blocks, main_q(b));
       if (e != hipSuccess) return hip_fail(b, e, "halo_lane_hist_kernel launch");
-      HIPCHK(b, hipMemcpyAsync(hist.data(), b->comp_hist.ptr, nb * sizeof(uint32_t), hipMemcpyDeviceToHost, b->stream));
-      HIPCHK(b, hipStreamSynchronize(b->stream));
+      HIPCHK(b, hipMemcpyAsync(hist.data(), b->comp_hist.ptr, nb * sizeof(uint32_t), hipMemcpyDeviceToHost, main_q(b)));
+      HIPCHK(b, hipStreamSynchronize(main_q(b)));
       if (pass == 0) {
         uint64_t count = 0;
         for (uint32_t i = 0; i < nb; i++) count += hist[i];
@@ -2490,11 +2539,11 @@
   if (linear_rgb_out) HIPCHK(b, b->comp_rgb.reserve(n3));
   if (srgb_out) HIPCHK(b, b->cons_rgb.reserve(n3));
   if (linear_rgb_out || srgb_out) {
-    hipError_t e = launch_composite(b->lanes.ptr, npix, cd, linear_rgb_out ? b->comp_rgb.ptr : nullptr, srgb_out ? b->cons_rgb.ptr : nullptr, blocks, b->stream);
+    hipError_t e = launch_composite(b->lanes.ptr, npix, cd, linear_rgb_out ? b->comp_rgb.ptr : nullptr, srgb_out ? b->cons_rgb.ptr : nullptr, blocks, main_q(b));
     if (e != hipSuccess) return hip_fail(b, e, "halo_composite_kernel launch");
-    if (linear_rgb_out) HIPCHK(b, hipMemcpyAsync(linear_rgb_out, b->comp_rgb.ptr, n3 * sizeof(float), hipMemcpyDeviceToHost, b->stream));
-    if (srgb_out) HIPCHK(b, hipMemcpyAsync(srgb_out, b->cons_rgb.ptr, n3, hipMemcpyDeviceToHost, b->stream));
-    HIPCHK(b, hipStreamSynchronize(b->stream));
+    if (linear_rgb_out) HIPCHK(b, hipMemcpyAsync(linear_rgb_out, b->comp_rgb.ptr, n3 * sizeof(float), hipMemcpyDeviceToHost, main_q(b)));
+    if (srgb_out) HIPCHK(b, hipMemcpyAsync(srgb_out, b->cons_rgb.ptr, n3, hipMemcpyDeviceToHost, main_q(b)));
+    HIPCHK(b, hipStreamSynchronize(main_q(b)));
   }
   *produced = 1;
   return HALO_OK;
diff --git a/ice_halo_sim_amd/csrc/halo_kernels.hip b/ice_halo_sim_amd/csrc/halo_kernels.hip
--- a/ice_halo_sim_amd/csrc/halo_kernels.hip
+++ b/ice_halo_sim_amd/csrc/halo_kernels.hip
@@ -524,7 +524,19 @@
   return hipMemsetAsync(ovf_flag, 0, sizeof(uint32_t), stream);
 }
 
-constexpr uint32_t kChunksInFlight = 16u, kLoads = 1u;
+#ifndef HALO_TILE_CHUNKS
+#define HALO_TILE_CHUNKS 8
+#endif
+#ifndef HALO_TILE_LOADS
+#define HALO_TILE_LOADS 1
+#endif
+#ifndef HALO_TILE_BATCH
+#define HALO_TILE_BATCH 32
+#endif
+constexpr uint32_t kChunksInFlight = HALO_TILE_CHUNKS, kLoads = HALO_TILE_LOADS;
+constexpr uint32_t kCloseBatch = HALO_TILE_BATCH;
+constexpr uint32_t kCloseKeep = 4u;
+static_assert(kCloseBatch % kChunksInFlight == 0u && kCloseBatch <= 64u, "a batch is whole groups of chunks, one count per lane");
 __global__ void __launch_bounds__(kBinBlock) halo_tile_close_kernel(const uint2* __restrict__ chunk, uint32_t cap, const uint32_t* __restrict__ cnt, uint32_t wgs,
                                                                     uint32_t tile_log2, uint32_t frac_bits, const CloseArgsOf<true> cl) {
   __shared__ __attribute__((aligned(16))) unsigned long long acc[1u << kBinTileLog2];
@@ -532,62 +544,85 @@
   const uint32_t tile = blockIdx.x;
   const uint32_t* tcnt = cnt + static_cast<size_t>(tile) * wgs;
   const bool take_twin = *cl.flag != 0u;
-  uint32_t any = 0u;
-  for (uint32_t c = threadIdx.x; c < wgs; c += kBinBlock) any |= tcnt[c];
+  const uint32_t lane = threadIdx.x & 63u, wave = threadIdx.x >> 6;
+  constexpr uint32_t kRound = (kBinBlock / 64u) * kCloseBatch;
+  auto count_at = [&](uint32_t r) -> uint32_t {
+    const uint32_t c = r * kRound + wave * kCloseBatch + lane;
+    return (lane < kCloseBatch && c < wgs) ? min(tcnt[c], cap) : 0u;
+  };
+  const uint32_t rounds = (wgs + kRound - 1u) / kRound;
+  uint32_t kept[kCloseKeep], any = rounds > kCloseKeep ? 1u : 0u;
+#pragma unroll
+  for (uint32_t r = 0; r < kCloseKeep; ++r) any |= kept[r] = count_at(r);
   if (!__syncthreads_or(static_cast<int>(any != 0u)) && !take_twin) return;
   const uint32_t slots = 1u << tile_log2, mask = slots - 1u;
   for (uint32_t j = threadIdx.x; j < slots; j += kBinBlock) acc[j] = 0ull;
   __syncthreads();
-  const uint32_t lane = threadIdx.x & 63u, wave = threadIdx.x >> 6, waves = kBinBlock / 64u;
   const uint2* tsrc = chunk + static_cast<size_t>(tile) * wgs * cap;
   auto add = [&](uint32_t slot, uint32_t w_bits) { atomicAdd(&acc[slot & mask], fq.fix(__uint_as_float(w_bits))); };
-  for (uint32_t c0 = wave * 64u; c0 < wgs; c0 += waves * 64u) {
-    const uint32_t mine = c0 + lane < wgs ? min(tcnt[c0 + lane], cap) : 0u;
-    if (__ballot(mine != 0u) == 0ull) continue;
-    for (uint32_t g = 0; g < 64u; g += kChunksInFlight) {
-      uint32_t n[kChunksInFlight], most = 0u;
+  auto batch = [&](uint32_t c0, uint32_t mine) {
+    if (__ballot(mine != 0u) == 0ull) return;
+    auto count_of = [&](uint32_t j) { return static_cast<uint32_t>(__builtin_amdgcn_readlane(static_cast<int>(mine), static_cast<int>(j))); };
+    auto steps_of = [&](uint32_t g) {
+      uint32_t most = 0u;
+#pragma unroll
+      for (uint32_t k = 0; k < kChunksInFlight; ++k) most = max(most, count_of(g + k));
+      return (most + 128u * kLoads - 1u) / (128u * kLoads);
+    };
+    uint32_t g = 0u, it = 0u, steps = 0u;
+    auto seek = [&]() {
+      while (g < kCloseBatch && (steps = steps_of(g)) == 0u) g += kChunksInFlight;
+      return g < kCloseBatch;
+    };
+    auto advance = [&]() {
+      if (++it < steps) return true;
+      it = 0u, g += kChunksInFlight;
+      return seek();
+    };
+    auto issue = [&](uint32_t sg, uint32_t si, uint4 (&h)[kChunksInFlight][kLoads]) {
 #pragma unroll
       for (uint32_t k = 0; k < kChunksInFlight; ++k) {
-        n[k] = static_cast<uint32_t>(__builtin_amdgcn_readlane(static_cast<int>(mine), static_cast<int>(g + k)));
-        most = max(most, n[k]);
-      }
-      if (most == 0u) continue;
-      uint4 h[kChunksInFlight][kLoads];
+        const uint32_t n = count_of(sg + k);
+        const uint4* src4 = reinterpret_cast<const uint4*>(tsrc + static_cast<size_t>(c0 + sg + k) * cap);
+#pragma unroll
+        for (uint32_t u = 0; u < kLoads; ++u) {
+          const uint32_t i = (si * kLoads + u) * 64u + lane;
+          if (2u * i < n) h[k][u] = load_list_u4<true>(&src4[i]);
+        }
+      }
+    };
+    auto take = [&](uint32_t sg, uint32_t si, const uint4 (&h)[kChunksInFlight][kLoads]) {
 #pragma unroll
       for (uint32_t k = 0; k < kChunksInFlight; ++k) {
-        const uint4* src4 = reinterpret_cast<const uint4*>(tsrc + static_cast<size_t>(c0 + g + k) * cap);
+        const uint32_t n = count_of(sg + k);
 #pragma unroll
         for (uint32_t u = 0; u < kLoads; ++u) {
-          const uint32_t i = lane + 64u * u;
-          h[k][u] = i < n[k] / 2u ? load_list_u4<true>(&src4[i]) : make_uint4(0u, 0u, 0u, 0u);
+          const uint32_t i = (si * kLoads + u) * 64u + lane;
+          if (2u * i < n) add(h[k][u].x, h[k][u].y);
+          if (2u * i + 1u < n) add(h[k][u].z, h[k][u].w);
         }
       }
-#pragma unroll
-      for (uint32_t k = 0; k < kChunksInFlight; ++k) {
-#pragma unroll
-        for (uint32_t u = 0; u < kLoads; ++u) {
-          if (lane + 64u * u < n[k] / 2u) {
-            add(h[k][u].x, h[k][u].y);
-            add(h[k][u].z, h[k][u].w);
-          }
-        }
-      }
-#pragma unroll
-      for (uint32_t k = 0; k < kChunksInFlight; ++k) {
-        const uint2* src = tsrc + static_cast<size_t>(c0 + g + k) * cap;
-        const uint4* src4 = reinterpret_cast<const uint4*>(src);
-        for (uint32_t i = lane + 64u * kLoads; i < n[k] / 2u; i += 64u) {
-          const uint4 q = load_list_u4<true>(&src4[i]);
-          add(q.x, q.y);
-          add(q.z, q.w);
-        }
-        if ((n[k] & 1u) != 0u && lane == 0u) {
-          const uint2 q = src[n[k] - 1u];
-          add(q.x, q.y);
-        }
-      }
-    }
-  }
+    };
+    if (!seek()) return;
+    uint4 ha[kChunksInFlight][kLoads], hb[kChunksInFlight][kLoads];
+    issue(g, it, ha);
+    for (;;) {
+      uint32_t tg = g, ti = it;
+      bool more = advance();
+      if (more) issue(g, it, hb);
+      take(tg, ti, ha);
+      if (!more) break;
+      tg = g, ti = it;
+      more = advance();
+      if (more) issue(g, it, ha);
+      take(tg, ti, hb);
+      if (!more) break;
+    }
+  };
+#pragma unroll
+  for (uint32_t r = 0; r < kCloseKeep; ++r)
+    if (r < rounds) batch(r * kRound + wave * kCloseBatch, kept[r]);
+  for (uint32_t r = kCloseKeep; r < rounds; ++r) batch(r * kRound + wave * kCloseBatch, count_at(r));
   __syncthreads();
   close_write_out(acc, fq, tile, tile_log2, slots, take_twin, cl);
 }
```

Result: faster. 29.14 billion, median of 6 (+5.1%).
